# microsoft/M3P

Measured on AMD Instinct MI355X. Metric: pre-train samples/sec (whole node), 12L/768d seq=128+36, higher is better.
Workload: dtype bf16; 1 GPU; cfg2: 12L/768d/12h, 36 regions + 128 tokens, V=250002, 19 MLM targets/seq + ITM BCE, dropout 0.10, adam_inverse_sqrt + clip 5; per_gpu_batch=256, global_batch=256, seq_len=164, parallelism=dp1, prewarm_steps=36

## Files before the change

### include/m3p_hip.h

```cpp
#ifndef M3P_HIP_H
#define M3P_HIP_H

#include <stddef.h>
#include <stdint.h>

#ifdef __cplusplus
extern "C" {
#endif

#define M3P_API __attribute__((visibility("default")))

#define M3P_OK 0
#define M3P_EINVAL (-1)
#define M3P_ENOTIMPL (-2)
#define M3P_ENOMEM (-3)

M3P_API const char* m3p_version(void);


enum {
  M3P_EPI_NONE = 0,
  M3P_EPI_BIAS = 1,
  M3P_EPI_BIAS_GELU = 2,
  M3P_EPI_BIAS_DROP_RES = 3,
  M3P_EPI_RES = 4,
  M3P_EPI_DGELU = 5,
  M3P_EPI_MUL = 6,
  M3P_EPI_MULQ = 7,
  M3P_EPI_BIAS_GELUQ = 8,
  M3P_EPI_BIAS_LSE = 9
};

typedef struct M3PEpilogue {
  const float* bias;
  const void* aux;
  void* out2;
  float* colsum;
  int32_t ld_aux;
  int32_t ld_out2;
  int32_t scale_cols;
  float scale;
  float alpha;
  uint32_t seed;
  uint32_t thresh24;
  float inv_keep;
  const float* descale_a;
  const float* descale_b;
  void* out8;
  const float* scale8;
  float* amax8;
  int32_t ld_out8;
  int32_t out8_bf8;
  const int32_t* rng_rows;
} M3PEpilogue;

M3P_API int m3p_gemm_nt_bf16(const void* A, int lda, const void* W, int ldw, void* C, int ldc,
                             int M, int N, int K, int epilogue, const M3PEpilogue* ep, void* stream);

M3P_API int m3p_gemm_nt_fp8(const void* A8, int lda, int a_is_bf8, const void* W8, int ldw, void* C, int ldc,
                            int M, int N, int K, int epilogue, const M3PEpilogue* ep, void* stream);

M3P_API int m3p_quant_fp8(const void* src, int ld_src, void* dst, int ld_dst, int rows, int cols, const float* scale,
                          float* amax, int bf8, void* stream);

M3P_API int m3p_quant_fp8_batch(const long long* desc, int n_desc, int blocks_per_matrix, void* stream);

M3P_API int m3p_gemm_nt_streamk_f32(const void* A, int lda, const void* W, int ldw, float* C, int ldc,
                                    int M, int N, int K, float alpha, void* stream);
M3P_API int m3p_gemm_nn_streamk_f32(const void* A, int lda, const void* W, int ldw, int k_valid, float* C,
                                    int ldc, int M, int N, int K, float alpha, void* stream);
M3P_API int m3p_gemm_nn_w4_f32(const void* A, int lda, const void* W, int ldw, float* C, int ldc, int M, int N, int K, float alpha,
                               void* workspace, size_t workspace_bytes, void* stream);

M3P_API size_t m3p_gemm_wgrad_workspace_bytes(void);
M3P_API int m3p_gemm_wgrad_bf16(const void* dY, int lddy, const void* X, int ldx, float* dW, int lddw,
                                int M, int N, int K, float alpha, void* workspace, size_t workspace_bytes,
                                void* stream);
M3P_API int m3p_gemm_wgrad_store_bf16(const void* dY, int lddy, const void* X, int ldx, float* dW, int lddw, int M, int N, int K,
                                      float alpha, void* workspace, size_t workspace_bytes, void* stream);
M3P_API int m3p_gemm_wgrad_pair_bf16(const void* dYa, int lddya, const void* Xa, int ldxa, float* dWa, int lddwa, int Na, int Ka,
                                     const void* dYb, int lddyb, const void* Xb, int ldxb, float* dWb, int lddwb, int Nb, int Kb,
                                     int M, float alpha, void* workspace, size_t workspace_bytes, void* stream);


M3P_API int m3p_layernorm_fwd(const void* x, const float* gamma, const float* beta, const uint8_t* rowmask,
                              void* y, float* mean, float* rstd, int rows, int d, float eps, void* stream);

M3P_API int m3p_layernorm_bwd(const void* dy_a, const void* dy_b, const void* x, const float* gamma,
                              const float* mean, const float* rstd, const uint8_t* rowmask,
                              void* dx, void* dx_drop, float* dgamma, float* dbeta, float* dbias_drop,
                              int rows, int d, uint32_t seed, uint32_t thresh24, float inv_keep, void* stream);
M3P_API int m3p_layernorm_bwd_rows(const void* dy_a, const void* dy_b, const void* x, const float* gamma,
                                   const float* mean, const float* rstd, const uint8_t* rowmask,
                                   void* dx, void* dx_drop, float* dgamma, float* dbeta, float* dbias_drop,
                                   int rows, int d, uint32_t seed, uint32_t thresh24, float inv_keep,
                                   const int32_t* rng_rows, void* stream);


M3P_API int m3p_attn_fwd(const void* qkv, const int32_t* keylen, void* ctx, float* lse, uint64_t* keepmask,
                         int B, int S, int H, int dh, uint32_t seed, uint32_t thresh24, float inv_keep,
                         void* stream);

M3P_API int m3p_attn_bwd(const void* qkv, const int32_t* keylen, const void* ctx, const void* dctx,
                         const float* lse, const uint64_t* keepmask, void* dqkv, float* dbias_qkv, int B, int S,
                         int H, int dh, float qscale, uint32_t seed, uint32_t thresh24, float inv_keep,
                         void* stream);

M3P_API int m3p_attn_query_fwd(const void* q, int ld_q, const void* kv, long long kv_bstride, int ld_kv,
                               const int32_t* klen, void* ctx, int B, int Tq, int H, int dh, int Lk, int causal,
                               int pos0, void* stream);

M3P_API int m3p_attn_rows_fwd(const void* q, int ld_q, const void* kv, long long kv_bstride, int ld_kv, const int32_t* klen,
                              void* ctx, float* lse, int B, int Tq, int H, int dh, int Lk, int causal, int pos0,
                              uint32_t seed, uint32_t thresh24, float inv_keep, void* stream);
M3P_API int m3p_attn_rows_bwd(const void* q, int ld_q, const void* kv, long long kv_bstride, int ld_kv, const int32_t* klen,
                              const void* dctx, const float* lse, void* dq, int ld_dq, float* dkv, int B, int Tq, int H,
                              int dh, int Lk, int causal, int pos0, float qscale, uint32_t seed, uint32_t thresh24,
                              float inv_keep, void* stream);


M3P_API int m3p_cast_f32_bf16(const float* src, void* dst, long long n, void* stream);

M3P_API int m3p_embed_assemble_fwd(const int64_t* tok, const void* emb_bf16, const float* pos,
                                   const void* img_proj, const float* loc, const float* w_loc,
                                   const float* b_loc, const float* g_img, const float* be_img,
                                   const float* g_emb, const float* be_emb, const int32_t* totlen,
                                   void* h, void* z, float* mean_emb, float* rstd_emb, void* e,
                                   float* mean_img, float* rstd_img, int B, int T, int R, int d,
                                   uint32_t seed_img, uint32_t seed_emb, uint32_t thresh24, float inv_keep,
                                   const void* img_rows, void* stream);

M3P_API int m3p_embed_image_rows_fwd(const void* img_proj, const float* loc, const float* w_loc, const float* b_loc,
                                     const float* g_img, const float* be_img, void* e, float* mean_img,
                                     float* rstd_img, void* img_rows, int B, int R, int d, uint32_t seed_img,
                                     uint32_t thresh24, float inv_keep, void* stream);

M3P_API int m3p_embed_assemble_bwd(const void* dh, const void* z, const float* mean_emb, const float* rstd_emb,
                                   const float* g_emb, const void* e, const float* mean_img,
                                   const float* rstd_img, const float* g_img, const int64_t* tok,
                                   const int32_t* totlen, const float* loc, void* dz_scratch, void* de,
                                   float* d_g_emb, float* d_be_emb, float* d_pos, float* d_emb,
                                   void* d_tok_rows, float* d_g_img, float* d_be_img, float* d_b_img, float* d_b_loc,
                                   float* d_w_loc, int B, int T, int R, int d, int pad_index,
                                   uint32_t seed_img, uint32_t seed_emb, uint32_t thresh24, float inv_keep,
                                   int phase, void* stream);


M3P_API int m3p_gather_rows(const void* src, const int32_t* idx, void* dst, int n, int d, void* stream);
M3P_API int m3p_place_rows(const void* src, const int32_t* inv, void* dst, int rows, int d, int n, uint32_t fill_bits,
                           void* stream);
M3P_API int m3p_scatter_add_rows(const void* src, const int32_t* idx, void* dst, int n, int d, void* stream);
M3P_API int m3p_scatter_add_token_rows(const void* rows, int ld_rows, const int64_t* ids, float* dst, int n, int d,
                                       int pad_index, void* stream);

M3P_API int m3p_itm_score_fwd(const void* pre, const float* w2, const float* b2, float* pooled, float* scores, int B,
                              int d, void* stream);
M3P_API int m3p_itm_score_bwd(const float* dscores, const float* pooled, const float* w2, void* dpre16, void* dpreT16,
                              int ldt, float* db1, float* dw2, float* db2, int B, int d, void* stream);

M3P_API int m3p_ce_fwd_bwd(void* logits, int ld, int n_rows, int V, const int64_t* target, float* row_loss,
                           float* loss_sum, float loss_scale, float grad_scale, void* stream);

M3P_API int m3p_ce_lse_from_blocks(const void* stats, int n_blocks, int n_rows, const void* logits, int ld, const int64_t* target,
                                   float* row_loss, float* row_lse, void* scratch, void* stream);
M3P_API int m3p_ce_bwd_colsum(void* logits, int ld, int n_rows, int V, const int64_t* target, const float* row_lse,
                              float grad_scale, float* colsum, void* workspace, size_t workspace_bytes, void* stream);
M3P_API size_t m3p_ce_colsum_workspace_bytes(int ld, int n_rows);
M3P_API int m3p_ce_fwd_bwd_colsum(void* logits, int ld, int n_rows, int V, const int64_t* target, float* row_loss,
                                  float* row_lse, float grad_scale, float* colsum, void* workspace,
                                  size_t workspace_bytes, void* stream);

M3P_API int m3p_ce_eval(const void* logits, int ld, int n_rows, int V, const int64_t* target, float* row_loss,
                        int32_t* row_argmax, void* stream);

M3P_API int m3p_colsum_bf16(const void* x, int ld, int n, int ncols, float* out, const float* scale_ptr,
                            void* stream);


M3P_API int m3p_sumsq_f32(const float* g, long long n, double* out, void* stream);

M3P_API int m3p_sumsq_ranges_f32(const float* base, const long long* starts, const long long* counts, int n_ranges, double* out,
                                 void* stream);

M3P_API int m3p_adam_step(float* p, float* g, float* m, float* v, void* w16, long long n, float lr, float beta1,
                          float beta2, float eps, float weight_decay, float step_size, const double* gnorm_sq,
                          float max_norm, float grad_scale, int zero_grad, void* stream);
M3P_API int m3p_adam_step_ranges(float* p, float* g, float* m, float* v, void* w16, const long long* starts,
                                 const long long* counts, const float* step_sizes, const int* zero_grad, int n_ranges,
                                 float lr, float beta1, float beta2, float eps, float weight_decay, const double* gnorm_sq,
                                 float max_norm, float grad_scale, void* stream);

M3P_API int m3p_gelu_fwd(const void* u, void* h, void* dh, long long n, void* stream);
M3P_API int m3p_gelu_fwd_gq(const void* u, void* h, void* gq, int M, int N, void* stream);
M3P_API int m3p_gelu_fwd_q8(const void* u, void* h, void* h8, long long n, const float* scale, float* amax, void* stream);

M3P_API int m3p_gelu_bwd(const void* dy, const void* u, void* du, long long n, void* stream);

M3P_API int m3p_mse_fwd_bwd(const void* pred, int ld_pred, const float* tgt, int ld_tgt, void* dpred, float* row_sq,
                            int rows, int cols, float grad_scale, void* stream);


M3P_API int m3p_dropout_rows(const void* x, int ldx, const void* res, int ldres, void* y, int ldy, int rows, int cols,
                             uint32_t rng_ld, uint32_t rng_col0, uint32_t seed, uint32_t thresh24, float inv_keep,
                             void* stream);

M3P_API int m3p_glu_fwd(const void* ab, int ld_ab, void* y, int rows, int d, void* stream);
M3P_API int m3p_glu_bwd(const void* ab, int ld_ab, const void* dy, void* dab, int rows, int d, void* stream);

M3P_API int m3p_transpose_batch_bf16(const long long* desc, int n_desc, int max_tiles, void* stream);

M3P_API int m3p_transpose_bf16(const void* src, void* dst, int rows, int cols, int ld_src, int ld_dst,
                               void* stream);

M3P_API int m3p_set_persistent_grid(int workgroups);
M3P_API int m3p_set_tile_queue(int32_t* counters, int n_slots);

enum {
  M3P_KERN_NT_SKINNY = 1,
  M3P_KERN_NT_W8 = 2,
  M3P_KERN_NT_W8_QUEUE = 3,
  M3P_KERN_NT_W4 = 4,
  M3P_KERN_NT_RING = 5,
  M3P_KERN_NT_128 = 6,
  M3P_KERN_WGRAD_W4_CHUNKS = 10,
  M3P_KERN_WGRAD_W4_TILES = 11,
  M3P_KERN_WGRAD_RING = 12,
  M3P_KERN_WGRAD_128 = 13
};
M3P_API int m3p_gemm_nt_plan(int M, int N, int K, int epilogue);
M3P_API int m3p_gemm_wgrad_plan(int M, int N, int K);

M3P_API void m3p_debug_set_variant(int v);
M3P_API void m3p_debug_attn_variant(int v);

M3P_API int m3p_seq_masks(const int64_t* lengths, const int64_t* lengths_b, int B, int S, int32_t* totlen,
                          uint8_t* rowmask, void* stream);
M3P_API int m3p_mask_to_rows(const uint8_t* mask, int n_mask, int inner, long long s0, long long s1, long long soff,
                             int d, int32_t* rows, int n_rows, void* stream);
M3P_API int m3p_cast_rows_f32_bf16(const float* in, long long s0, long long s1, int n0, int n1, int cols, void* out,
                                   void* stream);
M3P_API int m3p_scale_bf16_dev(const void* in, int in_is_f32, const float* g, void* out, long long n, void* stream);
M3P_API int m3p_axpy_dev_f32(float* dst, const float* src, const float* g, long long n, void* stream);
M3P_API int m3p_itm_loss_fwd_bwd(const float* scores, const int64_t* pos, int n_groups, int sample_n, float w_ce,
                                 float w_bce, float* loss, float* dscores, void* stream);

M3P_API int m3p_probe_mfma_16x16x32(const void* a_rowmajor_16x32, const void* b_colmajor_32x16,
                                    float* d_16x16, int* d_rowcol, void* stream);
M3P_API int m3p_probe_mfma_fp8_16x16x128(const void* a_16x128, const void* w_16x128, float* d_16x16, int a_is_bf8,
                                         void* stream);
M3P_API int m3p_probe_tr16(const void* tile_bf16_64x16, void* out_64x4, void* stream);
M3P_API int m3p_probe_permlane16_swap(void* out_2x64_u32, void* stream);

#ifdef __cplusplus
}
#endif
#endif
```

### m3p_amd/csrc/gemm.hip

```cpp
#include <mutex>
#include <type_traits>
#include "common.hpp"
#include "../../include/m3p_hip.h"
#include <hip/amd_detail/amd_hip_unsafe_atomics.h>

static int g_variant = 1;
extern "C" void m3p_debug_set_variant(int v) { g_variant = (v == 2 || v == 6) ? v : 1; }

namespace {

constexpr int BK = 64;
constexpr int ROWB = BK * 2;

template <int EPI>
__device__ __forceinline__ void epilogue_store(const M3PEpilogue& ep, bf16* __restrict__ C, int ldc,
                                               int M, int N, int m, int n, f32x4 acc, f32x4& csum) {
  if (m >= M || n >= N) return;
  const bool full = (n + 3 < N);
  float v[4] = {acc[0], acc[1], acc[2], acc[3]};
  const float alpha = (ep.alpha == 0.f) ? 1.f : ep.alpha;
  if (EPI == M3P_EPI_NONE || EPI == M3P_EPI_BIAS || EPI == M3P_EPI_RES) {
#pragma unroll
    for (int r = 0; r < 4; ++r) v[r] *= alpha;
  }
// ... 440 lines not shown
        {
          typedef unsigned int u32x2 __attribute__((ext_vector_type(2)));
          const u32x2 raw = __builtin_bit_cast(u32x2, a);
#pragma unroll
          for (int r = 0; r < 4; ++r) {
            const uint32_t sign = (raw[r >> 1] << (16 * (1 - (r & 1)))) & 0x80000000u;
            const uint32_t tb = __builtin_bit_cast(uint32_t, tv[j][r]);
            v[r] *= 0.5f + __builtin_bit_cast(float, (tb & 0x7FFFFFFFu) | sign);
          }
        }
      } else {
#pragma unroll
        for (int r = 0; r < 4; ++r) v[r] *= gelu_erf_grad_f((float)a[r]);
      }
    } else {
      v *= f32x4{(float)a[0], (float)a[1], (float)a[2], (float)a[3]};
    }
    const bf16x4 ob = bf16x4{(bf16)v[0], (bf16)v[1], (bf16)v[2], (bf16)v[3]};
    *reinterpret_cast<bf16x4*>(r1 + ep_off8<true>(fr, (j * 16 + fg * 4) * 2)) = ob;
    csum[j] += f32x4{(float)ob[0], (float)ob[1], (float)ob[2], (float)ob[3]};
  }
  bf16* Cp = C + (size_t)mrow0 * ldc + nw + sch * 8;
#pragma unroll
  for (int it = 0; it < 2; ++it) {
    const int row = it * 8 + srow;
    st16(Cp + (size_t)row * ldc, flip_halves(*reinterpret_cast<const u32x4*>(r1 + ep_off<true>(row, sch * 16)), it & 1));
  }
}


template <bool BF8>
__device__ __forceinline__ uint32_t pack8(const f32x4& v, float scale, float& amax) {
  constexpr float kMax = BF8 ? 57344.f : 448.f;
  float f[4];
#pragma unroll
  for (int r = 0; r < 4; ++r) {
    amax = fmaxf(amax, fabsf(v[r]));
    f[r] = __builtin_amdgcn_fmed3f(v[r] * scale, -kMax, kMax);
  }
  int w = 0;
  if (BF8) { w = __builtin_amdgcn_cvt_pk_bf8_f32(f[0], f[1], w, false); w = __builtin_amdgcn_cvt_pk_bf8_f32(f[2], f[3], w, true); }
  else { w = __builtin_amdgcn_cvt_pk_fp8_f32(f[0], f[1], w, false); w = __builtin_amdgcn_cvt_pk_fp8_f32(f[2], f[3], w, true); }
  return (uint32_t)w;
}
__device__ __forceinline__ void lds_w32(uint32_t a, uint32_t v) { asm volatile("ds_write_b32 %0, %1" :: "v"(a), "v"(v)); }
__device__ __forceinline__ void piece8_write(char* r8, const uint32_t (&w8)[4], int lane) {
  const int fr = lane & 15, fg = lane >> 4;
  const uint32_t la = lds_addr(r8);
  asm volatile("" ::: "memory");
#pragma unroll
  for (int j = 0; j < 4; ++j) lds_w32(la + fr * 64 + ((j ^ ((fr >> 1) & 3)) << 4) + fg * 4, w8[j]);
}
__device__ __forceinline__ void piece8_store(uint8_t* __restrict__ o8, int ld8, int mrow0, int nw, char* r8, int lane) {
  const uint32_t la = lds_addr(r8);
  const int row = lane >> 2, c = lane & 3;
  u32x4_lds R;
  lds_r128(la + row * 64 + (c << 4), R);
  asm volatile("s_waitcnt lgkmcnt(0)" : "+v"(R) :: "memory");
  st16p<true>(o8 + (size_t)(mrow0 + row) * ld8 + nw + ((c ^ ((row >> 1) & 3)) << 4), u32x4{R[0], R[1], R[2], R[3]});
}
__device__ __forceinline__ void piece8_flush(uint8_t* __restrict__ o8, int ld8, int mrow0, int nw, char* r1, const uint32_t (&w8)[4], int lane) {
  piece8_write(r1, w8, lane);
  piece8_store(o8, ld8, mrow0, nw, r1, lane);
}
template <int O8 = 0>
__device__ __forceinline__ void epilogue_pieceq(bf16* __restrict__ C, int ldc, int mrow0, int nw, char* r1, const f32x4 (&rows)[4],
                                                const u32x4& q, int lane, f32x4 (&csum)[4], uint8_t* __restrict__ o8 = nullptr, int ld8 = 0,
                                                float scale8 = 1.f, float* amax = nullptr, char* r8 = nullptr) {
  const int fr = lane & 15, fg = lane >> 4;
  const int srow = lane >> 3, sch = lane & 7;
  uint32_t w8[4];
#pragma unroll
  for (int j = 0; j < 4; ++j) {
    const uint32_t w = q[j];
    f32x4 g = f32x4{(float)(w & 0xFFu), (float)((w >> 8) & 0xFFu), (float)((w >> 16) & 0xFFu), (float)(w >> 24)};
    g = g * GQ_STEP - GQ_OFF;
    const f32x4 v = rows[j] * g;
    const bf16x4 ob = bf16x4{(bf16)v[0], (bf16)v[1], (bf16)v[2], (bf16)v[3]};
    if (O8) lds_w64(lds_addr(r1) + ep_off8<true>(fr, (j * 16 + fg * 4) * 2), ob);
    else *reinterpret_cast<bf16x4*>(r1 + ep_off8<true>(fr, (j * 16 + fg * 4) * 2)) = ob;
    csum[j] += v;
    if (O8) w8[j] = (O8 == 2) ? pack8<true>(v, scale8, *amax) : pack8<false>(v, scale8, *amax);
  }
  if (O8) piece8_write(r8, w8, lane);
  bf16* Cp = C + (size_t)mrow0 * ldc + nw + sch * 8;
  if (O8) {
    const uint32_t la = lds_addr(r1), l8 = lds_addr(r8);
    const int row8 = lane >> 2, c8 = lane & 3;
    u32x4_lds Ra, Rb, R8;
    lds_r128(la + ep_off<true>(srow, sch * 16), Ra);
    lds_r128(la + ep_off<true>(8 + srow, sch * 16), Rb);
    lds_r128(l8 + row8 * 64 + (c8 << 4), R8);
    asm volatile("s_waitcnt lgkmcnt(0)" : "+v"(Ra), "+v"(Rb), "+v"(R8));
    st16p<true>(Cp + (size_t)srow * ldc, u32x4{Ra[0], Ra[1], Ra[2], Ra[3]});
    st16p<true>(Cp + (size_t)(8 + srow) * ldc, u32x4{Rb[2], Rb[3], Rb[0], Rb[1]});
    st16p<true>(o8 + (size_t)(mrow0 + row8) * ld8 + nw + ((c8 ^ ((row8 >> 1) & 3)) << 4), u32x4{R8[0], R8[1], R8[2], R8[3]});
    return;
  }
  u32x4 R2[2];
#pragma unroll
  for (int it = 0; it < 2; ++it) {
    const int row = it * 8 + srow;
    R2[it] = flip_halves(*reinterpret_cast<const u32x4*>(r1 + ep_off<true>(row, sch * 16)), it & 1);
  }
#pragma unroll
  for (int it = 0; it < 2; ++it) st16p<true>(Cp + (size_t)(it * 8 + srow) * ldc, R2[it]);
  if (O8) piece8_store(o8, ld8, mrow0, nw, r8, lane);
}

__device__ __forceinline__ void epilogue_half_lse(bf16* __restrict__ C, int ldc, float2* __restrict__ stats, int V, int mrow0, int nw,
                                                  char* r1, const f32x4 (&rows0)[4], const f32x4 (&rows1)[4],
                                                  const f32x4 (&biasv)[4], int lane, bool edge) {
  constexpr float kLog2e = 1.4426950408889634f;
  const int fr = lane & 15, fg = lane >> 4;
  const int srow = lane >> 3, sch = lane & 7;
#pragma unroll
  for (int ii = 0; ii < 2; ++ii) {
    f32x4 x[4];
#pragma unroll
    for (int j = 0; j < 4; ++j) {
      x[j] = (ii ? rows1[j] : rows0[j]) + biasv[j];
      const bf16x4 xb = bf16x4{(bf16)x[j][0], (bf16)x[j][1], (bf16)x[j][2], (bf16)x[j][3]};
      *reinterpret_cast<bf16x4*>(r1 + ep_off8<true>(ii * 16 + fr, (j * 16 + fg * 4) * 2)) = xb;
#pragma unroll
      for (int r = 0; r < 4; ++r) x[j][r] = (float)xb[r];
    }
    if (edge) {
#pragma unroll
      for (int j = 0; j < 4; ++j)
#pragma unroll
        for (int r = 0; r < 4; ++r)
          if (nw + j * 16 + fg * 4 + r >= V) x[j][r] = -INFINITY;
    }
    f32x4 m4 = x[0];
#pragma unroll
    for (int j = 1; j < 4; ++j)
#pragma unroll
      for (int r = 0; r < 4; ++r) m4[r] = fmaxf(m4[r], x[j][r]);
    float m = fmaxf(fmaxf(m4[0], m4[1]), fmaxf(m4[2], m4[3]));
    m = fmaxf(m, __shfl_xor(m, 16, 64));
    m = fmaxf(m, __shfl_xor(m, 32, 64));
    const float mb = (m == -INFINITY) ? 0.f : m * kLog2e;
    f32x4 s4 = f32x4{0.f, 0.f, 0.f, 0.f};
#pragma unroll
    for (int j = 0; j < 4; ++j) {
      const f32x4 a = x[j] * kLog2e - mb;
#pragma unroll
      for (int r = 0; r < 4; ++r) s4[r] += __builtin_amdgcn_exp2f(a[r]);
    }
    float sm = (s4[0] + s4[1]) + (s4[2] + s4[3]);
    sm += __shfl_xor(sm, 16, 64);
    sm += __shfl_xor(sm, 32, 64);
    if (fg == 0) stats[mrow0 + ii * 16 + fr] = float2{m, sm};
  }
  bf16* Cp = C + (size_t)mrow0 * ldc + nw + sch * 8;
#pragma unroll
  for (int it = 0; it < 4; ++it) {
    const int row = it * 8 + srow;
    st16p<true>(Cp + (size_t)row * ldc, flip_halves(*reinterpret_cast<const u32x4*>(r1 + ep_off<true>(row, sch * 16)), it & 1));
  }
}

constexpr int GQ_TAB_LO = 0x3A00, GQ_TAB_HI = 0x4100, GQ_TAB_N = GQ_TAB_HI - GQ_TAB_LO;
constexpr int GQ_TAB_BYTES = GQ_TAB_N * 4;
__device__ __forceinline__ void geluq_table_fill(uint32_t* tab, int tid, int nthreads) {
  for (int i = tid; i < GQ_TAB_N; i += nthreads) {
    const float xm = __builtin_bit_cast(float, ((uint32_t)(GQ_TAB_LO + i) << 16) | 0x8000u);
    const float tail = 0.5f * erfcf(xm * 0.70710678118654752440f);
    const float gd = (1.0f - tail) + xm * 0.39894228040143267794f * __expf(-0.5f * xm * xm);
    tab[i] = (__builtin_bit_cast(uint32_t, tail) & 0xFFFFFF00u) | gelu_grad_code(gd);
  }
}
__device__ __forceinline__ void lds_r32(uint32_t a, uint32_t& v) { asm volatile("ds_read_b32 %0, %1" : "=v"(v) : "v"(a)); }
template <int O8 = 0>
__device__ __forceinline__ void epilogue_piece_geluq_lut(bf16* __restrict__ C, int ldc, uint8_t* __restrict__ qout, int mrow0, int nw,
                                                         char* r1, const f32x4 (&rows)[4], int lane, uint32_t tab_off,
                                                         uint8_t* __restrict__ o8 = nullptr, int ld8 = 0, float scale8 = 1.f, float* amax = nullptr,
                                                         char* r8 = nullptr) {
  const int fr = lane & 15, fg = lane >> 4;
  const int srow = lane >> 3, sch = lane & 7;
  uint32_t w8[4];
  uint32_t w[4][4];
#pragma unroll
  for (int j = 0; j < 4; ++j)
#pragma unroll
    for (int r = 0; r < 4; ++r) {
      const float xf = rows[j][r];
      const uint32_t xb = __builtin_bit_cast(uint32_t, xf);
      const uint32_t mag = __builtin_amdgcn_ubfe(xb, 16, 15);
      const uint32_t idx = min(max(mag, (uint32_t)GQ_TAB_LO), (uint32_t)(GQ_TAB_HI - 1));
      lds_r32((idx << 2) + tab_off, w[j][r]);
    }
  asm volatile("s_waitcnt lgkmcnt(0)" : "+v"(w[0][0]), "+v"(w[0][1]), "+v"(w[0][2]), "+v"(w[0][3]), "+v"(w[1][0]), "+v"(w[1][1]), "+v"(w[1][2]), "+v"(w[1][3]),
                                        "+v"(w[2][0]), "+v"(w[2][1]), "+v"(w[2][2]), "+v"(w[2][3]), "+v"(w[3][0]), "+v"(w[3][1]), "+v"(w[3][2]), "+v"(w[3][3]));
  const uint32_t la = lds_addr(r1);
  u32x4 code;
#pragma unroll
  for (int j = 0; j < 4; ++j) {
    f32x4 hv;
    float xs[4];
#pragma unroll
    for (int r = 0; r < 4; ++r) {
      xs[r] = rows[j][r];
      float mx;
      asm("v_max_f32 %0, 0, %1" : "=v"(mx) : "v"(xs[r]));
      asm("v_fma_f32 %0, -|%1|, %2, %3" : "=v"(hv[r]) : "v"(xs[r]), "v"(w[j][r]), "v"(mx));
    }
    const uint32_t x0 = __builtin_bit_cast(uint32_t, xs[0]), x1 = __builtin_bit_cast(uint32_t, xs[1]);
    const uint32_t x2 = __builtin_bit_cast(uint32_t, xs[2]), x3 = __builtin_bit_cast(uint32_t, xs[3]);
    const uint32_t blo = __builtin_amdgcn_perm(w[j][1], w[j][0], 0x0c0c0400u), bhi = __builtin_amdgcn_perm(w[j][3], w[j][2], 0x04000c0cu);
    const uint32_t slo = __builtin_amdgcn_perm(x1, x0, 0x0c0c0b09u), shi = __builtin_amdgcn_perm(x3, x2, 0x0b090c0cu);
    code[j] = (blo | bhi) ^ (slo | shi);
    lds_w64(la + ep_off8<true>(fr, (j * 16 + fg * 4) * 2), bf16x4{(bf16)hv[0], (bf16)hv[1], (bf16)hv[2], (bf16)hv[3]});
    if (O8) w8[j] = pack8<false>(hv, scale8, *amax);
  }
  st16p<true>(qout + lane * 16, code);
  if (O8) piece8_write(r8, w8, lane);
  u32x4 R[2];
  u32x4_lds R8;
  lds_r128(la + ep_off<true>(srow, sch * 16), R[0]);
  lds_r128(la + ep_off<true>(8 + srow, sch * 16), R[1]);
  const int row8 = lane >> 2, c8 = lane & 3;
  if (O8) {
    lds_r128(lds_addr(r8) + row8 * 64 + (c8 << 4), R8);
    asm volatile("s_waitcnt lgkmcnt(0)" : "+v"(R[0]), "+v"(R[1]), "+v"(R8));
  } else {
    asm volatile("s_waitcnt lgkmcnt(0)" : "+v"(R[0]), "+v"(R[1]));
  }
  bf16* Cp = C + (size_t)mrow0 * ldc + nw + sch * 8;
  st16p<true>(Cp + (size_t)srow * ldc, R[0]);
  st16p<true>(Cp + (size_t)(8 + srow) * ldc, flip_halves(R[1], true));
  if (O8) st16p<true>(o8 + (size_t)(mrow0 + row8) * ld8 + nw + ((c8 ^ ((row8 >> 1) & 3)) << 4), u32x4{R8[0], R8[1], R8[2], R8[3]});
}


template <int EPI>
__global__ __launch_bounds__(512)
void gemm_nt_ring_kernel(const bf16* __restrict__ A, int lda, const bf16* __restrict__ W, int ldw,
                         bf16* __restrict__ C, int ldc, int M, int N, int K, M3PEpilogue ep,
                         int tiles_m, int tiles_n) {
  constexpr int BM = 256, BN = 128, NWAVES = 8;
  constexpr int A_BYTES = BM * ROWB, B_BYTES = BN * ROWB, STAGE = A_BYTES + B_BYTES;
  extern __shared__ __attribute__((aligned(16))) char smem[];

  const int tid = threadIdx.x, lane = tid & 63;
  const int wid = __builtin_amdgcn_readfirstlane(tid >> 6);
  const int ntiles = tiles_m * tiles_n;
  const int n_strips = (tiles_n >= 24) ? (tiles_n + 7) / 8 : 1;
  const int strip_w = (tiles_n + n_strips - 1) / n_strips;
  auto split_tile = [&](int t, int& tm, int& tn) {
    const int strip = t / (tiles_m * strip_w);
    const int rem = t - strip * tiles_m * strip_w;
    const int bn = min(strip_w, tiles_n - strip * strip_w);
    tm = rem / bn;
    tn = strip * strip_w + (rem - tm * bn);
  };
  const int nwg = gridDim.x;
  const int per_xcd = nwg >> 3;
  const int slot = (blockIdx.x & 7) * per_xcd + (blockIdx.x >> 3);
  auto tile_of = [&](int q) { return q * nwg + slot; };
  const int my_tiles = (ntiles > slot) ? (ntiles - slot + nwg - 1) / nwg : 0;
  if (my_tiles == 0) return;
  float* gtab = (EPI == M3P_EPI_DGELU) ? reinterpret_cast<float*>(smem + 3 * STAGE) : nullptr;
  if (EPI == M3P_EPI_DGELU) gelu_grad_table_fill(gtab, tid, 512);
  const int nk = K / BK;
  const int total = my_tiles * nk;

  const int sr = lane >> 3, sc = (lane & 7) ^ sr;
  const bf16* a_src[4];
  const bf16* w_src[2];
  int l_q = 0, l_kt = 0;
  auto set_load_tile = [&](int q) {
    const int t = tile_of(q);
    int tm, tn;
    split_tile(t, tm, tn);
#pragma unroll
    for (int i = 0; i < 4; ++i) a_src[i] = A + (size_t)min(tm * BM + (wid + i * NWAVES) * 8 + sr, M - 1) * lda + sc * 8;
#pragma unroll
    for (int i = 0; i < 2; ++i) w_src[i] = W + (size_t)min(tn * BN + (wid + i * NWAVES) * 8 + sr, N - 1) * ldw + sc * 8;
  };
  auto issue_load = [&](int s, int piece) {
    char* sa = smem + s * STAGE;
    const int k0 = l_kt * BK;
    if (piece < 4)
      __builtin_amdgcn_global_load_lds(GLB_PTR(a_src[piece] + k0), LDS_PTR(sa + (wid + piece * NWAVES) * 1024), 16, 0, 0);
    else
      __builtin_amdgcn_global_load_lds(GLB_PTR(w_src[piece - 4] + k0), LDS_PTR(sa + A_BYTES + (wid + (piece - 4) * NWAVES) * 1024), 16, 0, 0);
  };
  auto load_done = [&]() {
    if (++l_kt == nk) { l_kt = 0; ++l_q; if (l_q < my_tiles) set_load_tile(l_q); }
  };
  auto stage_next = [&](int s) {
#pragma unroll
    for (int pc = 0; pc < 6; ++pc) issue_load(s, pc);
    load_done();
  };

  const int wm = wid >> 1, wn = wid & 1;
  const int fr = lane & 15, fg = lane >> 4;
  const uint32_t lds0 = (uint32_t)(uintptr_t)(__attribute__((address_space(3))) char*)smem;
  uint32_t a_addr[2], b_addr[2];
#pragma unroll
  for (int ks = 0; ks < 2; ++ks) {
    const int ch = ((fg + 4 * ks) ^ (fr & 7)) * 16;
    a_addr[ks] = lds0 + (wm * 64 + fr) * ROWB + ch;
    b_addr[ks] = lds0 + A_BYTES + (wn * 64 + fr) * ROWB + ch;
// ... 243 lines not shown
    a_addr[ks] = lds0 + (wm * 128 + fr) * ROWB + ch;
    b_addr[ks] = lds0 + A_BYTES + (wn * 64 + fr) * ROWB + ch;
  }
#define W8_DSR(dst, addr, off) asm volatile("ds_read_b128 %0, %1 offset:" #off : "=v"(dst) : "v"(addr))
  auto read_w = [&](uint32_t ba, bf16x8 (&wf)[4]) {
    W8_DSR(wf[0], ba, 0); W8_DSR(wf[1], ba, 2048); W8_DSR(wf[2], ba, 4096); W8_DSR(wf[3], ba, 6144);
  };
  auto read_a_lo = [&](uint32_t aa, bf16x8 (&af)[4]) {
    W8_DSR(af[0], aa, 0); W8_DSR(af[1], aa, 2048); W8_DSR(af[2], aa, 4096); W8_DSR(af[3], aa, 6144);
  };
  auto read_a_hi = [&](uint32_t aa, bf16x8 (&af)[4]) {
    W8_DSR(af[0], aa, 8192); W8_DSR(af[1], aa, 10240); W8_DSR(af[2], aa, 12288); W8_DSR(af[3], aa, 14336);
  };
#define W8_LGKM0() do { __builtin_amdgcn_sched_barrier(0); asm volatile("s_waitcnt lgkmcnt(0)" ::: "memory"); __builtin_amdgcn_sched_barrier(0); } while (0)

  f32x4 acc[8][4];
#pragma unroll
  for (int i = 0; i < 8; ++i)
#pragma unroll
    for (int j = 0; j < 4; ++j) acc[i][j] = f32x4{0.f, 0.f, 0.f, 0.f};
  if constexpr (kGqLut) {
    int tm0, tn0;
    split_tile(slot, tm0, tn0);
    const float* bp = ep.bias + tn0 * BN + wn * 64 + fg * 4;
#pragma unroll
    for (int j = 0; j < 4; ++j) {
      const f32x4 b = *reinterpret_cast<const f32x4*>(bp + j * 16);
#pragma unroll
      for (int i = 0; i < 8; ++i) acc[i][j] = b;
    }
  }
  auto mfma_q = [&](auto half_c, const bf16x8 (&af)[4], const bf16x8 (&wf)[4]) {
    constexpr int I0 = 4 * decltype(half_c)::value;
    __builtin_amdgcn_s_setprio(1);
#pragma unroll
    for (int i = 0; i < 4; ++i)
#pragma unroll
      for (int j = 0; j < 4; ++j)
        acc[I0 + i][j] = __builtin_amdgcn_mfma_f32_16x16x32_bf16(wf[j], af[i], acc[I0 + i][j], 0, 0, 0);
    __builtin_amdgcn_s_setprio(0);
  };
  using H0 = std::integral_constant<int, 0>;
  using H1 = std::integral_constant<int, 1>;

  set_load_tile(slot);
  stage_next(0);
#define W8_H1 (dyn ? h1d : (step + 1 < total))
#define W8_MORE2 (dyn ? l_alive : more2)
  bool h1d = l_alive;
  if (dyn ? h1d : (total > 1)) {
    stage_next(1);
    asm volatile("s_waitcnt vmcnt(8)" ::: "memory");
  } else {
    asm volatile("s_waitcnt vmcnt(0)" ::: "memory");
  }
  __builtin_amdgcn_s_barrier();
  asm volatile("" ::: "memory");

  bf16x8 fa0[4], fa1[4], fw0[4], fw1[4];
  read_w(b_addr[0], fw0);
  read_a_lo(a_addr[0], fa0);
  W8_LGKM0();
  int c_kt = 0, c_q = 0;
  const bool io_aligned = ((ldc & 7) == 0) && (((uintptr_t)C & 15) == 0) &&
                          (!(EPI == M3P_EPI_BIAS_GELU) || (((ep.ld_out2 & 7) == 0) && (((uintptr_t)ep.out2 & 15) == 0))) &&
                          (!ep.bias || (((uintptr_t)ep.bias & 15) == 0)) &&
                          (!ep.aux || (((ep.ld_aux & 7) == 0) && (((uintptr_t)ep.aux & 15) == 0)));
  f32x4 csum[4];
#pragma unroll
  for (int j = 0; j < 4; ++j) csum[j] = f32x4{0.f, 0.f, 0.f, 0.f};
  int csum_nw = -1;
  auto flush_csum = [&]() {
#pragma unroll
    for (int j = 0; j < 4; ++j)
#pragma unroll
      for (int r = 0; r < 4; ++r) {
        float sfl = csum[j][r];
        sfl += __shfl_xor(sfl, 1, 64); sfl += __shfl_xor(sfl, 2, 64);
        sfl += __shfl_xor(sfl, 4, 64); sfl += __shfl_xor(sfl, 8, 64);
        const int n = csum_nw + j * 16 + fg * 4 + r;
        if (fr == 0 && n < N) unsafeAtomicAdd(ep.colsum + n, sfl);
        csum[j][r] = 0.f;
      }
  };
  float amax_run = 0.f;
  if constexpr (O8 && EPI == M3P_EPI_MULQ) reinterpret_cast<float*>(smem + 2 * STAGE + 8 * 2048)[tid] = 0.f;
  bool spread_pending = false;
  for (int step = 0; dyn || step < total; ++step) {
    const int cur = step & 1, nxt = cur ^ 1;
    const bool last_kt = (c_kt + 1 == nk);
    const bool more2 = dyn ? false : (step + 2 < total);
    const uint32_t so = cur * STAGE;
    const bool pend = spread_pending;
    if (pend) { issue_load(nxt, 3); issue_load(nxt, 4); issue_load(nxt, 5); }
    read_a_hi(a_addr[0] + so, fa1);
    __builtin_amdgcn_sched_barrier(0);
    mfma_q(H0{}, fa0, fw0);
    W8_LGKM0();
    if (pend) { issue_load(nxt, 6); issue_load(nxt, 7); }
    read_w(b_addr[1] + so, fw1);
    read_a_lo(a_addr[1] + so, fa0);
    __builtin_amdgcn_sched_barrier(0);
    mfma_q(H1{}, fa1, fw0);
    if (pend) { load_done(); spread_pending = false; }
    W8_LGKM0();
    read_a_hi(a_addr[1] + so, fa1);
    __builtin_amdgcn_sched_barrier(0);
    mfma_q(H0{}, fa0, fw1);
    W8_LGKM0();
    asm volatile("s_waitcnt vmcnt(0)" ::: "memory");
    __builtin_amdgcn_s_barrier();
    asm volatile("" ::: "memory");
    __builtin_amdgcn_sched_barrier(0);
    if (dyn && pop_state) {
      if (pop_state == 1) {
        if (wid == 0 && lane == 0) {
          const int p = per_xcd + (int)popped, q = p / per_xcd;
          const int t = q * nwg + xcd * per_xcd + (p - q * per_xcd);
          *mbox = (t < ntiles) ? t : -1;
        }
        pop_state = 2;
      } else {
        t_next = __builtin_amdgcn_readfirstlane(*mbox);
        pop_state = 0;
      }
      __builtin_amdgcn_sched_barrier(0);
    }
    const bool req = W8_MORE2 && (!last_kt || !kAuxE);
    if (req) {
      issue_load(cur, 0); issue_load(cur, 1); issue_load(cur, 2);
      spread_pending = true;
    }
    if (W8_H1 && !last_kt) {
      read_w(b_addr[0] + nxt * STAGE, fw0);
      read_a_lo(a_addr[0] + nxt * STAGE, fa0);
    }
    __builtin_amdgcn_sched_barrier(0);
    mfma_q(H1{}, fa1, fw1);
    W8_LGKM0();

    if (++c_kt == nk) {
      c_kt = 0;
      const int t = dyn ? t_cmp : tile_of(c_q);
      if (dyn) t_cmp = t_ld; else ++c_q;
      int tm, tn;
      split_tile(t, tm, tn);
      const int m0 = tm * BM, n0 = tn * BN;
      const int mw = m0 + wm * 128, nw = n0 + wn * 64;
      if (kMulE && ep.colsum && csum_nw != nw) {
        if (csum_nw >= 0) flush_csum();
        csum_nw = nw;
      }
      const bool fast = io_aligned && (m0 + BM <= M) && (n0 + BN <= N);
      if constexpr (EPI == M3P_EPI_BIAS_LSE) {
        if (fast) {
          char* r1 = smem + 2 * STAGE + wid * 4096;
          f32x4 biasv[4];
#pragma unroll
          for (int j = 0; j < 4; ++j) biasv[j] = *reinterpret_cast<const f32x4*>(ep.bias + nw + j * 16 + (lane >> 4) * 4);
          const int V = ep.ld_out2;
          float2* st = reinterpret_cast<float2*>(ep.out2) + (size_t)(tn * 4 + wn) * M;
          const bool edge = (nw + 64 > V);
#pragma unroll
          for (int hf = 0; hf < 4; ++hf) {
            epilogue_half_lse(C, ldc, st, V, mw + 32 * hf, nw, r1, acc[2 * hf], acc[2 * hf + 1], biasv, lane, edge);
            __builtin_amdgcn_sched_barrier(0);
          }
        }
      } else if constexpr (kGqLut) {
        f32x4 bnext[4];
        {
          const bool more_tiles = dyn ? (t_cmp >= 0) : (c_q < my_tiles);
          int tm2 = tm, tn2 = tn;
          if (more_tiles) split_tile(dyn ? t_cmp : tile_of(c_q), tm2, tn2);
          const float* bp = ep.bias + tn2 * BN + wn * 64 + fg * 4;
#pragma unroll
          for (int j = 0; j < 4; ++j) bnext[j] = *reinterpret_cast<const f32x4*>(bp + j * 16);
        }
        {
          char* r1 = smem + 2 * STAGE + kTabBytes + wid * 2048;
          const uint32_t tab_off = lds0 + 2 * STAGE - 4 * GQ_TAB_LO;
          uint8_t* qo = reinterpret_cast<uint8_t*>(ep.out2) + gq_block_offset(tm, tn, tiles_n, wid, 0);
          if constexpr (O8) {
            const float sc8 = ep.scale8 ? *ep.scale8 : 1.f;
#pragma unroll
            for (int hp = 0; hp < 8; ++hp) {
              epilogue_piece_geluq_lut<1>(C, ldc, qo + 1024 * hp, mw + 16 * hp, nw, r1, acc[hp], lane, tab_off,
                                          reinterpret_cast<uint8_t*>(ep.out8), ep.ld_out8, sc8, &amax_run,
                                          smem + 2 * STAGE + kTabBytes + 8 * 2048 + wid * 1024);
              __builtin_amdgcn_sched_barrier(0);
            }
          } else {
#pragma unroll
            for (int hp = 0; hp < 8; ++hp) {
              epilogue_piece_geluq_lut(C, ldc, qo + 1024 * hp, mw + 16 * hp, nw, r1, acc[hp], lane, tab_off);
              __builtin_amdgcn_sched_barrier(0);
            }
          }
        }
#pragma unroll
        for (int i = 0; i < 8; ++i)
#pragma unroll
          for (int j = 0; j < 4; ++j) acc[i][j] = bnext[j];
      } else if constexpr (EPI == M3P_EPI_MULQ) {
        if (fast) {
          const uint8_t* qp = reinterpret_cast<const uint8_t*>(ep.aux) + gq_block_offset(tm, tn, tiles_n, wid, 0) + lane * 16;
          char* r1 = smem + 2 * STAGE + wid * 2048;
#define MQ_LD(off) (*reinterpret_cast<const u32x4*>(qp + (off)))
          u32x4 qa = MQ_LD(0), qb = MQ_LD(1024);
          __builtin_amdgcn_sched_barrier(0);
          if (W8_MORE2) { issue_load(cur, 0); issue_load(cur, 1); issue_load(cur, 2); spread_pending = true; }
          __builtin_amdgcn_sched_barrier(0);
          if constexpr (O8) {
            const float sc8 = ep.scale8 ? *ep.scale8 : 1.f;
            uint8_t* o8 = reinterpret_cast<uint8_t*>(ep.out8);
            float* amax_slot = reinterpret_cast<float*>(smem + 2 * STAGE + 8 * 2048) + tid;
            float amax_t = *amax_slot;
#pragma unroll
            for (int hp = 0; hp < 8; ++hp) {
              u32x4 qc = qb;
              if (hp + 2 < 8) qc = MQ_LD((hp + 2) * 1024);
              char* r8 = smem + 2 * STAGE + 8 * 2048 + 2048 + wid * 1024;
              epilogue_pieceq<2>(C, ldc, mw + 16 * hp, nw, r1, acc[hp], qa, lane, csum, o8, ep.ld_out8, sc8, &amax_t, r8);
              __builtin_amdgcn_sched_barrier(0);
              qa = qb; qb = qc;
            }
            *amax_slot = amax_t;
          } else {
#pragma unroll
          for (int hp = 0; hp < 8; hp += 2) {
            u32x4 qc = qa, qd = qb;
            if (hp + 2 < 8) qc = MQ_LD((hp + 2) * 1024);
            epilogue_pieceq(C, ldc, mw + 16 * hp, nw, r1, acc[hp], qa, lane, csum);
            __builtin_amdgcn_sched_barrier(0);
            if (hp + 3 < 8) qd = MQ_LD((hp + 3) * 1024);
            epilogue_pieceq(C, ldc, mw + 16 * (hp + 1), nw, r1, acc[hp + 1], qb, lane, csum);
            __builtin_amdgcn_sched_barrier(0);
            qa = qc; qb = qd;
          }
          }
#undef MQ_LD
        }
      } else if (fast && kMulE) {
        char* r1 = smem + 2 * STAGE + kTabBytes + wid * 2048;
        u32x4 ta[2], tb[2];
        aux16_issue(ep, mw, nw, lane, ta);
        __builtin_amdgcn_sched_barrier(0);
        if (W8_MORE2) { issue_load(cur, 0); issue_load(cur, 1); issue_load(cur, 2); spread_pending = true; }
        __builtin_amdgcn_sched_barrier(0);
#pragma unroll
        for (int hp = 0; hp < 8; hp += 2) {
          aux16_issue(ep, mw + 16 * (hp + 1), nw, lane, tb);
          epilogue_piece16<EPI>(ep, C, ldc, mw + 16 * hp, nw, r1, acc[hp], ta, lane, csum, gtab);
          __builtin_amdgcn_sched_barrier(0);
          if (hp + 2 < 8) aux16_issue(ep, mw + 16 * (hp + 2), nw, lane, ta);
          epilogue_piece16<EPI>(ep, C, ldc, mw + 16 * (hp + 1), nw, r1, acc[hp + 1], tb, lane, csum, gtab);
          __builtin_amdgcn_sched_barrier(0);
        }
      } else if (fast) {
        char* r1 = smem + 2 * STAGE + wid * 4096;
        f32x4 biasv[4];
        load_bias4<EPI>(ep, nw, lane, biasv);
        u32x4 aux0[4];
        if (kAuxE) {
          load_aux_rows_issue<EPI>(ep, mw, nw, lane, aux0);
          __builtin_amdgcn_sched_barrier(0);
          if (W8_MORE2) { issue_load(cur, 0); issue_load(cur, 1); issue_load(cur, 2); spread_pending = true; }
          __builtin_amdgcn_sched_barrier(0);
        }
#pragma unroll
        for (int hf = 0; hf < 4; ++hf) {
          f32x4 rows[2][4];
#pragma unroll
          for (int ii = 0; ii < 2; ++ii)
#pragma unroll
            for (int j = 0; j < 4; ++j) rows[ii][j] = acc[2 * hf + ii][j];
          bf16x4 auxv[2][4];
          if (kAuxE && hf == 0) load_aux_rows_finish<EPI, true>(lane, r1, aux0, auxv);
          else load_aux_rows<EPI, true>(ep, mw + 32 * hf, nw, lane, r1, auxv);
          epilogue_half<EPI, true>(ep, C, ldc, N, mw + 32 * hf, nw, r1, rows, biasv, auxv, lane, csum, gtab);
          __builtin_amdgcn_sched_barrier(0);
        }
      } else {
        if (kAuxE && W8_MORE2) { issue_load(cur, 0); issue_load(cur, 1); issue_load(cur, 2); spread_pending = true; }
#pragma unroll
        for (int i = 0; i < 8; ++i)
#pragma unroll
          for (int j = 0; j < 4; ++j)
            epilogue_store<EPI>(ep, C, ldc, M, N, mw + i * 16 + fr, nw + j * 16 + fg * 4, acc[i][j], csum[j]);
      }
      if constexpr (!kGqLut) {
#pragma unroll
        for (int i = 0; i < 8; ++i)
#pragma unroll
          for (int j = 0; j < 4; ++j) acc[i][j] = f32x4{0.f, 0.f, 0.f, 0.f};
      }
      if (W8_H1) {
        read_w(b_addr[0] + nxt * STAGE, fw0);
        read_a_lo(a_addr[0] + nxt * STAGE, fa0);
        W8_LGKM0();
      }
    }
    if (dyn) {
      if (!h1d) break;
      h1d = l_alive;
    }
  }
  if (kMulE && ep.colsum && csum_nw >= 0) flush_csum();
  if constexpr (O8 && (EPI == M3P_EPI_BIAS_GELUQ || EPI == M3P_EPI_MULQ)) {
    if (ep.amax8) {
      float* wmax = reinterpret_cast<float*>(smem + 2 * STAGE + kTabBytes);
      if constexpr (EPI == M3P_EPI_MULQ) amax_run = reinterpret_cast<float*>(smem + 2 * STAGE + 8 * 2048)[tid];
      const float mxw = wave_max(amax_run);
      __syncthreads();
      if (lane == 0) wmax[wid] = mxw;
      __syncthreads();
      if (tid == 0) {
        float mx = wmax[0];
#pragma unroll
// ... 951 lines not shown
  *err = hipSuccess;
  std::lock_guard<std::mutex> lk(g_tq_mu);
  if (!g_tq_pool) return nullptr;
  if (!g_tq_bound) { g_tq_stream = st; g_tq_bound = true; }
  if (st != g_tq_stream) return nullptr;
  if (g_tq_next == g_tq_slots) {
    *err = hipMemsetAsync(g_tq_pool, 0, (size_t)g_tq_slots * 8 * sizeof(int), st);
    if (*err != hipSuccess) return nullptr;
    g_tq_next = 0;
  }
  return g_tq_pool + 8 * g_tq_next++;
}

constexpr int W4_MIN_K = 2048;
static bool tq_enabled() {
  std::lock_guard<std::mutex> lk(g_tq_mu);
  return g_tq_pool != nullptr;
}

static int nt_plan(int epi, int M, int N, int K, int* queue) {
  if (queue) *queue = 0;
  const bool whole = M >= 1024 && (M % 256) == 0 && (N % 256) == 0 && N >= 512 && (K % 64) == 0;
  if (epi == M3P_EPI_MULQ || epi == M3P_EPI_BIAS_GELUQ || epi == M3P_EPI_BIAS_LSE) return whole ? M3P_KERN_NT_W8 : M3P_EINVAL;
  const bool mul_epi = epi == M3P_EPI_DGELU || epi == M3P_EPI_MUL;
  if (M <= 128 && (K % 128) == 0 && !mul_epi) return M3P_KERN_NT_SKINNY;
  const bool deep = N >= 512 && 2LL * N * K <= (64LL << 20) && epi != M3P_EPI_DGELU;
  const bool armed = tq_enabled();
  const bool w4_first = g_variant == 1 && deep && K >= W4_MIN_K && epi != M3P_EPI_MUL && !armed;
  if (whole && g_variant != 2 && !w4_first) {
    int grid = num_cus();
    const int ntiles = (M / 256) * (N / 256);
    if (ntiles < grid) grid = (ntiles + 7) / 8 * 8;
    if (queue) *queue = (!mul_epi && armed && ntiles > grid && K >= 8 * BK) ? 1 : 0;
    return M3P_KERN_NT_W8;
  }
  if (M >= 1024 && (M % 256) == 0 && (N % 256) == 0 && (g_variant == 2 || (g_variant == 1 && deep)))
    return M3P_KERN_NT_W4;
  if (M >= 1024) return M3P_KERN_NT_RING;
  return M3P_KERN_NT_128;
}

template <int EPI>
int launch_nt(const bf16* A, int lda, const bf16* W, int ldw, bf16* C, int ldc, int M, int N, int K,
              const M3PEpilogue& ep, hipStream_t st) {
  int want_queue = 0;
  const int plan = nt_plan(EPI, M, N, K, &want_queue);
  if (plan == M3P_KERN_NT_SKINNY) {
    if constexpr (EPI != M3P_EPI_DGELU && EPI != M3P_EPI_MUL) {
      if (M <= 16) return launch_nt_skinny<EPI, 1>(A, lda, W, ldw, C, ldc, M, N, K, ep, st);
      if (M <= 32) return launch_nt_skinny<EPI, 2>(A, lda, W, ldw, C, ldc, M, N, K, ep, st);
      if (M <= 64) return launch_nt_skinny<EPI, 4>(A, lda, W, ldw, C, ldc, M, N, K, ep, st);
      return launch_nt_skinny<EPI, 8>(A, lda, W, ldw, C, ldc, M, N, K, ep, st);
    }
  }
  if (plan == M3P_KERN_NT_W8) {
    const int tiles_m = M / 256, tiles_n = N / 256;
    const size_t lds = 2 * 512 * ROWB + (EPI == M3P_EPI_DGELU ? GELU_TAB_N * sizeof(float) : 0) +
                       ((EPI == M3P_EPI_DGELU || EPI == M3P_EPI_MUL) ? 8 * 2048 : 8 * 4096);
    auto kern = gemm_nt_w8_kernel<EPI>;
    static bool attr_set8 = false;
    if (!attr_set8) {
      hipError_t e = hipFuncSetAttribute((const void*)kern, hipFuncAttributeMaxDynamicSharedMemorySize, (int)lds);
      if (e != hipSuccess) return (int)e;
      attr_set8 = true;
    }
    int grid = num_cus();
    const int ntiles = tiles_m * tiles_n;
    if (ntiles < grid) grid = (ntiles + 7) / 8 * 8;
    constexpr bool kQueueOk = !(EPI == M3P_EPI_DGELU || EPI == M3P_EPI_MUL);
    int* ctr = nullptr;
    if (kQueueOk && want_queue) {
      hipError_t e;
      ctr = tq_acquire(st, &e);
      if (e != hipSuccess) return (int)e;
    }
    if constexpr (kQueueOk) if (ctr) {
      auto kern_d = gemm_nt_w8_kernel<EPI, true>;
      static bool attr_set8d = false;
      if (!attr_set8d) {
        hipError_t e = hipFuncSetAttribute((const void*)kern_d, hipFuncAttributeMaxDynamicSharedMemorySize, (int)lds);
        if (e != hipSuccess) return (int)e;
        attr_set8d = true;
      }
      hipLaunchKernelGGL(kern_d, dim3(grid), dim3(512), lds, st, A, lda, W, ldw, C, ldc, M, N, K, ep, tiles_m, tiles_n, ctr);
      M3P_CHECK_LAUNCH();
      return M3P_OK;
    }
    hipLaunchKernelGGL(kern, dim3(grid), dim3(512), lds, st, A, lda, W, ldw, C, ldc, M, N, K, ep, tiles_m, tiles_n, ctr);
    M3P_CHECK_LAUNCH();
    return M3P_OK;
  }
  if (plan == M3P_KERN_NT_W4) {
    constexpr int BM = 256, BN = 256;
    const int tiles_m = (M + BM - 1) / BM, tiles_n = (N + BN - 1) / BN;
    const size_t lds = 2 * (BM + BN) * 128 + 4 * EP_HALF;
    const bool rows = (EPI == M3P_EPI_BIAS_DROP_RES && ep.rng_rows != nullptr);
    auto kern = rows ? gemm_nt_w4_kernel<(EPI == M3P_EPI_BIAS_DROP_RES ? M3P_EPI_DROP_RES_ROWS : EPI)> : gemm_nt_w4_kernel<EPI>;
    static bool attr_set_both[2] = {false, false};
    bool& attr_set = attr_set_both[rows ? 1 : 0];
    if (!attr_set) {
      hipError_t e = hipFuncSetAttribute((const void*)kern, hipFuncAttributeMaxDynamicSharedMemorySize, (int)lds);
      if (e != hipSuccess) return (int)e;
      attr_set = true;
    }
    int grid = num_cus();
    const int ntiles = tiles_m * tiles_n;
    if (ntiles < grid) grid = (ntiles + 7) / 8 * 8;
    const long long wbytes = 2LL * N * K, abytes = 2LL * M * K;
    const int m_fast = (wbytes > (64LL << 20) && abytes < wbytes) ? 1 : 0;
    hipLaunchKernelGGL(kern, dim3(grid), dim3(256), lds, st, A, lda, W, ldw, C, ldc, M, N, K, ep, tiles_m, tiles_n, m_fast);
    M3P_CHECK_LAUNCH();
    return M3P_OK;
  }
  if (plan == M3P_KERN_NT_RING) {
    constexpr int BM = 256, BN = 128;
    const int tiles_m = (M + BM - 1) / BM, tiles_n = (N + BN - 1) / BN;
    const size_t lds = 3 * (BM + BN) * ROWB + (EPI == M3P_EPI_DGELU ? GELU_TAB_N * sizeof(float) : 0);
    auto kern = gemm_nt_ring_kernel<EPI>;
    static bool attr_set = false;
    if (!attr_set) {
      hipError_t e = hipFuncSetAttribute((const void*)kern, hipFuncAttributeMaxDynamicSharedMemorySize, (int)lds);
      if (e != hipSuccess) return (int)e;
      attr_set = true;
    }
    int grid = num_cus();
    const int ntiles = tiles_m * tiles_n;
    if (ntiles < grid) grid = (ntiles + 7) / 8 * 8;
    hipLaunchKernelGGL(kern, dim3(grid), dim3(512), lds, st, A, lda, W, ldw, C, ldc, M, N, K, ep, tiles_m, tiles_n);
    M3P_CHECK_LAUNCH();
    return M3P_OK;
  }
  constexpr int BM = 128, BN = 128;
  const int tiles_m = (M + BM - 1) / BM, tiles_n = (N + BN - 1) / BN;
  const size_t lds = 2 * (BM + BN) * ROWB;
  auto kern = gemm_nt_kernel<BM, BN, EPI>;
  static bool attr_set = false;
  if (!attr_set) {
    hipError_t e = hipFuncSetAttribute((const void*)kern, hipFuncAttributeMaxDynamicSharedMemorySize, (int)lds);
    if (e != hipSuccess) return (int)e;
    attr_set = true;
  }
  hipLaunchKernelGGL(kern, dim3(tiles_m * tiles_n), dim3(256), lds, st, A, lda, W, ldw, C, ldc, M, N, K, ep,
                     tiles_m, tiles_n);
  M3P_CHECK_LAUNCH();
  return M3P_OK;
}

template <int EPI>
static int launch_nt_gq(const bf16* A, int lda, const bf16* W, int ldw, bf16* C, int ldc, int M, int N, int K,
                        const M3PEpilogue& ep, hipStream_t st) {
  if (M < 1024 || (M % 256) || (N % 256) || N < 512 || (K % 64) || (lda % 8) || (ldw % 8) || (ldc % 8) || ((uintptr_t)C & 15))
    return M3P_EINVAL;
  if (EPI == M3P_EPI_MULQ && (!ep.aux || ((uintptr_t)ep.aux & 15))) return M3P_EINVAL;
  if ((EPI == M3P_EPI_BIAS_GELUQ || EPI == M3P_EPI_BIAS_LSE) && (!ep.out2 || ((uintptr_t)ep.out2 & 15) || !ep.bias || ((uintptr_t)ep.bias & 15)))
    return M3P_EINVAL;
  if (EPI == M3P_EPI_BIAS_LSE && (ep.ld_out2 <= 0 || ep.ld_out2 > N)) return M3P_EINVAL;
  const int tiles_m = M / 256, tiles_n = N / 256;
  const size_t lds = 2 * 512 * ROWB + ((EPI == M3P_EPI_BIAS_GELUQ) ? GQ_TAB_BYTES + 8 * 2048 + 8 * 1024 : 8 * (EPI != M3P_EPI_MULQ ? 4096 : 2048)) +
                     (EPI == M3P_EPI_MULQ ? 2048 + 8 * 1024 : 0);
  int grid = num_cus();
  const int ntiles = tiles_m * tiles_n;
  if (ntiles < grid) grid = (ntiles + 7) / 8 * 8;
  if constexpr (EPI == M3P_EPI_BIAS_GELUQ || EPI == M3P_EPI_MULQ) {
    if (ep.out8) {
      if (((uintptr_t)ep.out8 & 15) || (ep.ld_out8 & 15) || ep.ld_out8 < N || !ep.scale8 || !ep.amax8) return M3P_EINVAL;
      if ((EPI == M3P_EPI_MULQ) != (ep.out8_bf8 != 0)) return M3P_EINVAL;
      auto kern8 = gemm_nt_w8_kernel<EPI, false, true>;
      static bool attr_set8 = false;
      if (!attr_set8) {
        hipError_t e = hipFuncSetAttribute((const void*)kern8, hipFuncAttributeMaxDynamicSharedMemorySize, (int)lds);
        if (e != hipSuccess) return (int)e;
        attr_set8 = true;
      }
      hipLaunchKernelGGL(kern8, dim3(grid), dim3(512), lds, st, A, lda, W, ldw, C, ldc, M, N, K, ep, tiles_m, tiles_n, (int*)nullptr);
      M3P_CHECK_LAUNCH();
      return M3P_OK;
    }
  }
  auto kern = gemm_nt_w8_kernel<EPI>;
  static bool attr_set = false;
  if (!attr_set) {
    hipError_t e = hipFuncSetAttribute((const void*)kern, hipFuncAttributeMaxDynamicSharedMemorySize, (int)lds);
    if (e != hipSuccess) return (int)e;
    attr_set = true;
  }
  hipLaunchKernelGGL(kern, dim3(grid), dim3(512), lds, st, A, lda, W, ldw, C, ldc, M, N, K, ep, tiles_m, tiles_n, (int*)nullptr);
  M3P_CHECK_LAUNCH();
  return M3P_OK;
}

constexpr int WG_T = 128;
constexpr int WG_ROWB = WG_T * 2;
constexpr int WG_TILE_BYTES = BK * WG_ROWB;

__device__ __forceinline__ bf16x4 lds_tr16(const char* p) {
  s16x4 v = __builtin_amdgcn_ds_read_tr16_b64_v4i16((__attribute__((address_space(3))) s16x4*)(p));
  return __builtin_bit_cast(bf16x4, v);
}

__global__ __launch_bounds__(256)
void gemm_wgrad_kernel(const bf16* __restrict__ dY, int lddy, const bf16* __restrict__ X, int ldx,
                       float* __restrict__ dW, int lddw, int M, int N, int K, float alpha,
                       int tiles_i, int tiles_j, int m_chunk) {
  extern __shared__ __attribute__((aligned(16))) char smem[];
  const int tid = threadIdx.x, lane = tid & 63;
  const int wid = __builtin_amdgcn_readfirstlane(tid >> 6);
  const int ntile = tiles_i * tiles_j;
  const int id = xcd_remap(blockIdx.x, gridDim.x);
  const int split = id / ntile, tile = id - split * ntile;
  const int ti = tile / tiles_j, tj = tile - ti * tiles_j;
  const int i0 = ti * WG_T, j0 = tj * WG_T;
  const int m_begin = split * m_chunk;
  const int m_end = min(M, m_begin + m_chunk);
  if (m_begin >= m_end) return;

  const int sr = lane >> 4, sc = lane & 15;
  const int n_chunks = (N + 7) / 8, k_chunks = (K + 7) / 8;
  int ycol[4], xcol[4];
#pragma unroll
  for (int i = 0; i < 4; ++i) {
    const int rb = wid + i * 4;
    const int f = sr | (((rb >> 1) & 1) << 2);
    const int gc = sc ^ (f << 1);
    ycol[i] = min(i0 / 8 + gc, n_chunks - 1) * 8;
    xcol[i] = min(j0 / 8 + gc, k_chunks - 1) * 8;
  }

  auto stage = [&](int mt, int s) {
    char* sy = smem + s * 2 * WG_TILE_BYTES;
    char* sx = sy + WG_TILE_BYTES;
    const int mbase = m_begin + mt * BK;
    const bool fullt = (mbase + BK <= m_end);
#pragma unroll
    for (int i = 0; i < 4; ++i) {
      const int rb = wid + i * 4;
      const int m = mbase + rb * 4 + sr;
      if (fullt) {
        __builtin_amdgcn_global_load_lds(GLB_PTR(dY + (size_t)m * lddy + ycol[i]), LDS_PTR(sy + rb * 1024), 16, 0, 0);
        __builtin_amdgcn_global_load_lds(GLB_PTR(X + (size_t)m * ldx + xcol[i]), LDS_PTR(sx + rb * 1024), 16, 0, 0);
      } else {
        uint4 vy = make_uint4(0, 0, 0, 0), vx = make_uint4(0, 0, 0, 0);
        if (m < m_end) {
          vy = *reinterpret_cast<const uint4*>(dY + (size_t)m * lddy + ycol[i]);
          vx = *reinterpret_cast<const uint4*>(X + (size_t)m * ldx + xcol[i]);
        }
        *reinterpret_cast<uint4*>(sy + rb * 1024 + lane * 16) = vy;
        *reinterpret_cast<uint4*>(sx + rb * 1024 + lane * 16) = vx;
      }
    }
  };

  const int wi = wid >> 1, wj = wid & 1;
  const int ft = lane & 15, fg = lane >> 4;
  const int frow = (fg * 8 + (ft >> 2)) * WG_ROWB;
  const int fsw = ((ft >> 2) | ((fg & 1) << 2)) << 1;
  int y_off[4], x_off[4];
#pragma unroll
  for (int c = 0; c < 4; ++c) {
    const int qy = wi * 8 + 2 * c + ((ft & 3) >> 1), qx = wj * 8 + 2 * c + ((ft & 3) >> 1);
    y_off[c] = frow + ((qy ^ fsw) << 4) + ((ft & 1) << 3);
    x_off[c] = WG_TILE_BYTES + frow + ((qx ^ fsw) << 4) + ((ft & 1) << 3);
  }

  f32x4 acc[4][4];
#pragma unroll
  for (int a = 0; a < 4; ++a)
#pragma unroll
    for (int b = 0; b < 4; ++b) acc[a][b] = f32x4{0.f, 0.f, 0.f, 0.f};

  const int nmt = (m_end - m_begin + BK - 1) / BK;
  stage(0, 0);
  __syncthreads();
  for (int mt = 0; mt < nmt; ++mt) {
    const int cur = mt & 1;
    if (mt + 1 < nmt) stage(mt + 1, cur ^ 1);
    const char* sbase = smem + cur * 2 * WG_TILE_BYTES;
#pragma unroll
    for (int ks = 0; ks < 2; ++ks) {
      bf16x8 yf[4], xf[4];
#pragma unroll
      for (int c = 0; c < 4; ++c) {
        const char* py = sbase + y_off[c] + ks * 32 * WG_ROWB;
        const char* px = sbase + x_off[c] + ks * 32 * WG_ROWB;
        bf16x4 y0 = lds_tr16(py), y1 = lds_tr16(py + 4 * WG_ROWB);
        bf16x4 x0 = lds_tr16(px), x1 = lds_tr16(px + 4 * WG_ROWB);
        yf[c] = bf16x8{y0[0], y0[1], y0[2], y0[3], y1[0], y1[1], y1[2], y1[3]};
        xf[c] = bf16x8{x0[0], x0[1], x0[2], x0[3], x1[0], x1[1], x1[2], x1[3]};
      }
#pragma unroll
      for (int a = 0; a < 4; ++a)
#pragma unroll
        for (int b = 0; b < 4; ++b)
          acc[a][b] = __builtin_amdgcn_mfma_f32_16x16x32_bf16(yf[a], xf[b], acc[a][b], 0, 0, 0);
    }
    __syncthreads();
  }

#pragma unroll
  for (int a = 0; a < 4; ++a)
#pragma unroll
    for (int b = 0; b < 4; ++b) {
      const int j = j0 + wj * 64 + b * 16 + ft;
#pragma unroll
      for (int r = 0; r < 4; ++r) {
        const int i = i0 + wi * 64 + a * 16 + fg * 4 + r;
        if (i < N && j < K) unsafeAtomicAdd(dW + (size_t)i * lddw + j, alpha * acc[a][b][r]);
      }
    }
}
// ... 532 lines not shown
  const int frow = fg * 8 + (ft >> 2);
  const int fsw = ((ft >> 2) | ((fg & 1) << 2)) << 1;
  uint32_t y_addr[4], x_addr[4];
#pragma unroll
  for (int c = 0; c < 4; ++c) {
    const int qy = wi * 8 + 2 * c + ((ft & 3) >> 1), qx = wj * 8 + 2 * c + ((ft & 3) >> 1);
    y_addr[c] = lds0 + frow * WR_YROW + ((qy ^ fsw) << 4) + ((ft & 1) << 3);
    x_addr[c] = lds0 + WR_YB + frow * WR_XROW + ((qx ^ fsw) << 4) + ((ft & 1) << 3);
  }
#define M3P_TR(dst, addr, off) asm volatile("ds_read_b64_tr_b16 %0, %1 offset:" #off : "=v"(dst) : "v"(addr))
  auto read_set0 = [&](uint32_t so, s16x4 (&y)[4][2], s16x4 (&x)[4][2]) {
#pragma unroll
    for (int c = 0; c < 4; ++c) {
      M3P_TR(y[c][0], y_addr[c] + so, 0); M3P_TR(y[c][1], y_addr[c] + so, 2048);
      M3P_TR(x[c][0], x_addr[c] + so, 0); M3P_TR(x[c][1], x_addr[c] + so, 1024);
    }
  };
  auto read_set1 = [&](uint32_t so, s16x4 (&y)[4][2], s16x4 (&x)[4][2]) {
#pragma unroll
    for (int c = 0; c < 4; ++c) {
      M3P_TR(y[c][0], y_addr[c] + so, 16384); M3P_TR(y[c][1], y_addr[c] + so, 18432);
      M3P_TR(x[c][0], x_addr[c] + so, 8192); M3P_TR(x[c][1], x_addr[c] + so, 9216);
    }
  };
#define M3P_LGKM0() do { __builtin_amdgcn_sched_barrier(0); asm volatile("s_waitcnt lgkmcnt(0)" ::: "memory"); __builtin_amdgcn_sched_barrier(0); } while (0)

  f32x4 acc[4][4];
#pragma unroll
  for (int a = 0; a < 4; ++a)
#pragma unroll
    for (int b = 0; b < 4; ++b) acc[a][b] = f32x4{0.f, 0.f, 0.f, 0.f};
  auto frag = [](const s16x4 (&h)[2]) {
    return __builtin_bit_cast(bf16x8, __builtin_shufflevector(h[0], h[1], 0, 1, 2, 3, 4, 5, 6, 7));
  };
  auto mfma_batch = [&](const s16x4 (&y)[4][2], const s16x4 (&x)[4][2]) {
    bf16x8 yf[4], xf[4];
#pragma unroll
    for (int c = 0; c < 4; ++c) { yf[c] = frag(y[c]); xf[c] = frag(x[c]); }
#pragma unroll
    for (int a = 0; a < 4; ++a)
#pragma unroll
      for (int b = 0; b < 4; ++b)
        acc[a][b] = __builtin_amdgcn_mfma_f32_16x16x32_bf16(yf[a], xf[b], acc[a][b], 0, 0, 0);
  };

  stage_next(0);
  if (total > 1) {
    stage_next(1);
    asm volatile("s_waitcnt vmcnt(6)" ::: "memory");
  } else {
    asm volatile("s_waitcnt vmcnt(0)" ::: "memory");
  }
  __builtin_amdgcn_s_barrier();
  asm volatile("" ::: "memory");

  s16x4 y0[4][2], x0[4][2], y1[4][2], x1[4][2];
  read_set0(0, y0, x0);
  M3P_LGKM0();
  WgCursor cc = locate(g0);
  int cur = 0;
  for (int step = 0; step < total; ++step) {
    const int nxt = (cur == 2) ? 0 : cur + 1;
    const int nx2 = (nxt == 2) ? 0 : nxt + 1;
    const bool more2 = (step + 2 < total);
    if (more2) stage_next(nx2);
    read_set1(cur * WR_STAGE, y1, x1);
    __builtin_amdgcn_sched_barrier(0);
    mfma_batch(y0, x0);
    M3P_LGKM0();
    if (more2) asm volatile("s_waitcnt vmcnt(6)" ::: "memory");
    else asm volatile("s_waitcnt vmcnt(0)" ::: "memory");
    __builtin_amdgcn_s_barrier();
    asm volatile("" ::: "memory");
    __builtin_amdgcn_sched_barrier(0);
    read_set0(nxt * WR_STAGE, y0, x0);
    __builtin_amdgcn_sched_barrier(0);
    mfma_batch(y1, x1);
    M3P_LGKM0();

    const bool last_of_tile = (cc.mt + 1 == cc.len) || (step + 1 == total);
    if (last_of_tile) {
      const int ti = cc.t / tiles_j, tj = cc.t - ti * tiles_j;
#pragma unroll
      for (int a = 0; a < 4; ++a)
#pragma unroll
        for (int b = 0; b < 4; ++b) {
          const int j = tj * WR_J + wj * 64 + b * 16 + ft;
#pragma unroll
          for (int r = 0; r < 4; ++r) {
            const int i = ti * WR_I + wi * 64 + a * 16 + fg * 4 + r;
            if (i < N && j < K) unsafeAtomicAdd(dW + (size_t)i * lddw + j, alpha * acc[a][b][r]);
            acc[a][b][r] = 0.f;
          }
        }
    }
    advance(cc);
    cur = nxt;
  }
#undef M3P_TR
#undef M3P_LGKM0
}

}

namespace {
template <int EPI, bool A_BF8>
int launch_nt_fp8(const uint8_t* A, int lda, const uint8_t* W, int ldw, bf16* C, int ldc, int M, int N, int K,
                         const M3PEpilogue& ep, hipStream_t st) {
  const int tiles_m = M / 256, tiles_n = N / 256;
  const size_t lds = 2 * 512 * ROWB + (EPI == M3P_EPI_DGELU ? GELU_TAB_N * sizeof(float) : 0) +
                     ((EPI == M3P_EPI_DGELU || EPI == M3P_EPI_MUL) ? 8 * 2048 : 8 * 4096);
  auto kern = gemm_nt_w8f8_kernel<EPI, A_BF8>;
  static bool attr_set = false;
  if (!attr_set) {
    hipError_t e = hipFuncSetAttribute((const void*)kern, hipFuncAttributeMaxDynamicSharedMemorySize, (int)lds);
    if (e != hipSuccess) return (int)e;
    attr_set = true;
  }
  int grid = num_cus();
  const int ntiles = tiles_m * tiles_n;
  if (ntiles < grid) grid = (ntiles + 7) / 8 * 8;
  hipLaunchKernelGGL(kern, dim3(grid), dim3(512), lds, st, A, lda, W, ldw, C, ldc, M, N, K, ep, tiles_m, tiles_n);
  M3P_CHECK_LAUNCH();
  return M3P_OK;
}

}

extern "C" {

int m3p_gemm_nt_bf16(const void* A, int lda, const void* W, int ldw, void* C, int ldc, int M, int N, int K,
                     int epilogue, const M3PEpilogue* ep_in, void* stream) {
  if (M <= 0 || N <= 0 || K <= 0 || (K % BK) != 0 || (lda % 8) != 0 || (ldw % 8) != 0 || (ldc % 4) != 0)
    return M3P_EINVAL;
  if (((uintptr_t)A & 15) || ((uintptr_t)W & 15) || ((uintptr_t)C & 7)) return M3P_EINVAL;
  M3PEpilogue ep = {};
  if (ep_in) ep = *ep_in;
  if ((epilogue == M3P_EPI_BIAS_DROP_RES || epilogue == M3P_EPI_RES || epilogue == M3P_EPI_DGELU || epilogue == M3P_EPI_MUL) &&
      (!ep.aux || (ep.ld_aux % 4) != 0))
    return M3P_EINVAL;
  if (epilogue == M3P_EPI_BIAS_GELU && (!ep.out2 || (ep.ld_out2 % 4) != 0)) return M3P_EINVAL;
  hipStream_t st = (hipStream_t)stream;
  const bf16* a = (const bf16*)A; const bf16* w = (const bf16*)W; bf16* c = (bf16*)C;
  switch (epilogue) {
    case M3P_EPI_NONE: return launch_nt<M3P_EPI_NONE>(a, lda, w, ldw, c, ldc, M, N, K, ep, st);
    case M3P_EPI_BIAS: return launch_nt<M3P_EPI_BIAS>(a, lda, w, ldw, c, ldc, M, N, K, ep, st);
    case M3P_EPI_BIAS_GELU: return launch_nt<M3P_EPI_BIAS_GELU>(a, lda, w, ldw, c, ldc, M, N, K, ep, st);
    case M3P_EPI_BIAS_DROP_RES: return launch_nt<M3P_EPI_BIAS_DROP_RES>(a, lda, w, ldw, c, ldc, M, N, K, ep, st);
    case M3P_EPI_RES: return launch_nt<M3P_EPI_RES>(a, lda, w, ldw, c, ldc, M, N, K, ep, st);
    case M3P_EPI_DGELU: return launch_nt<M3P_EPI_DGELU>(a, lda, w, ldw, c, ldc, M, N, K, ep, st);
    case M3P_EPI_MUL: return launch_nt<M3P_EPI_MUL>(a, lda, w, ldw, c, ldc, M, N, K, ep, st);
    case M3P_EPI_MULQ: return launch_nt_gq<M3P_EPI_MULQ>(a, lda, w, ldw, c, ldc, M, N, K, ep, st);
    case M3P_EPI_BIAS_GELUQ: return launch_nt_gq<M3P_EPI_BIAS_GELUQ>(a, lda, w, ldw, c, ldc, M, N, K, ep, st);
    case M3P_EPI_BIAS_LSE: return launch_nt_gq<M3P_EPI_BIAS_LSE>(a, lda, w, ldw, c, ldc, M, N, K, ep, st);
    default: return M3P_EINVAL;
  }
}

int m3p_gemm_nt_fp8(const void* A, int lda, int a_is_bf8, const void* W, int ldw, void* C, int ldc, int M, int N, int K,
                    int epilogue, const M3PEpilogue* ep_in, void* stream) {
  if (M <= 0 || N <= 0 || K <= 0 || (K % 128) != 0 || (lda % 16) != 0 || (ldw % 16) != 0 || (ldc % 8) != 0) return M3P_EINVAL;
  if ((M % 256) != 0 || (N % 256) != 0) return M3P_EINVAL;
  if (((uintptr_t)A & 15) || ((uintptr_t)W & 15) || ((uintptr_t)C & 15)) return M3P_EINVAL;
  M3PEpilogue ep = {};
  if (ep_in) ep = *ep_in;
  if ((epilogue == M3P_EPI_BIAS_DROP_RES || epilogue == M3P_EPI_RES || epilogue == M3P_EPI_DGELU || epilogue == M3P_EPI_MUL) &&
      (!ep.aux || (ep.ld_aux % 8) != 0))
    return M3P_EINVAL;
  hipStream_t st = (hipStream_t)stream;
  const uint8_t* a = (const uint8_t*)A; const uint8_t* w = (const uint8_t*)W; bf16* c = (bf16*)C;
#define M3P_F8_CASE(E)                                                                                        \
  case E: return a_is_bf8 ? launch_nt_fp8<E, true>(a, lda, w, ldw, c, ldc, M, N, K, ep, st)                    \
                          : launch_nt_fp8<E, false>(a, lda, w, ldw, c, ldc, M, N, K, ep, st)
  switch (epilogue) {
    M3P_F8_CASE(M3P_EPI_NONE);
    M3P_F8_CASE(M3P_EPI_BIAS);
    M3P_F8_CASE(M3P_EPI_BIAS_DROP_RES);
    M3P_F8_CASE(M3P_EPI_RES);
    M3P_F8_CASE(M3P_EPI_DGELU);
    M3P_F8_CASE(M3P_EPI_MUL);
    default: return M3P_ENOTIMPL;
  }
#undef M3P_F8_CASE
}

static int launch_streamk(const void* A, int lda, const void* W, int ldw, float* C, int ldc, int M, int N, int K, float alpha,
                          bool w_kn, int k_valid, void* stream) {
  if (M <= 0 || N <= 0 || K <= 0 || (K % BK) != 0 || (lda % 8) != 0 || (ldw % 8) != 0) return M3P_EINVAL;
  if (((uintptr_t)A & 15) || ((uintptr_t)W & 15)) return M3P_EINVAL;
  if (w_kn && (k_valid <= 0 || k_valid > K)) return M3P_EINVAL;
  const int tiles_m_all = (M + 255) / 256, tiles_n = (N + 127) / 128;
  const size_t lds = 3 * (256 + 128) * ROWB;
  auto kern = w_kn ? gemm_nt_streamk_kernel<true> : gemm_nt_streamk_kernel<false>;
  hipError_t e = hipFuncSetAttribute((const void*)kern, hipFuncAttributeMaxDynamicSharedMemorySize, (int)lds);
  if (e != hipSuccess) return (int)e;
  const int grid = num_cus();
  const int nk = K / BK;
  const int n_launch = (tiles_m_all * tiles_n + grid - 1) / grid;
  const int rows_per = ((tiles_m_all + n_launch - 1) / n_launch) * 256;
  for (int m0 = 0; m0 < M; m0 += rows_per) {
    const int m = (M - m0 < rows_per) ? M - m0 : rows_per;
    const int tiles_m = (m + 255) / 256;
    long long share = ((long long)tiles_m * tiles_n * nk + grid - 1) / grid;
    const int chunk = (int)(share < nk ? (share < 1 ? 1 : share) : nk);
    hipLaunchKernelGGL(kern, dim3(grid), dim3(512), lds, (hipStream_t)stream, (const bf16*)A + (size_t)m0 * lda, lda,
                       (const bf16*)W, ldw, C + (size_t)m0 * ldc, ldc, m, N, K, alpha, tiles_m, tiles_n, chunk, k_valid);
    M3P_CHECK_LAUNCH();
  }
  return M3P_OK;
}

int m3p_gemm_nt_streamk_f32(const void* A, int lda, const void* W, int ldw, float* C, int ldc, int M, int N, int K,
                            float alpha, void* stream) {
  return launch_streamk(A, lda, W, ldw, C, ldc, M, N, K, alpha, false, K, stream);
}

int m3p_gemm_nn_streamk_f32(const void* A, int lda, const void* W, int ldw, int k_valid, float* C, int ldc, int M, int N,
                            int K, float alpha, void* stream) {
  return launch_streamk(A, lda, W, ldw, C, ldc, M, N, K, alpha, true, k_valid, stream);
}

int m3p_set_persistent_grid(int workgroups) {
  if (workgroups < 0 || (workgroups % 8) != 0) return M3P_EINVAL;
  g_persistent_grid = workgroups;
  return M3P_OK;
}

int m3p_set_tile_queue(int32_t* counters, int n_slots) {
  if (counters && (n_slots <= 0 || ((uintptr_t)counters & 3))) return M3P_EINVAL;
  std::lock_guard<std::mutex> lk(g_tq_mu);
  g_tq_pool = counters;
  g_tq_slots = counters ? n_slots : 0;
  g_tq_next = 0;
  g_tq_bound = false;
  return M3P_OK;
}

size_t m3p_gemm_wgrad_workspace_bytes(void) {
  const size_t grid = (size_t)hw_cus();
  return grid * (65536 + 272) * sizeof(float) + grid * sizeof(int);
}

static bool wgrad_w4_ok(int M, int N, int K, int lddy, int ldx, const void* dY, const void* X) {
  return (M % 64) == 0 && M >= 4096 && (N % 256) == 0 && (K % 256) == 0 &&
         (lddy % 8) == 0 && (ldx % 8) == 0 && !((uintptr_t)dY & 15) && !((uintptr_t)X & 15);
}
extern "C++" {
template <bool YROWS = false>
static int launch_wgrad_w4(const void* dY, int lddy, const void* X, int ldx, float* dW, int lddw, int M, int N, int K,
                           float alpha, void* workspace, size_t workspace_bytes, void* stream, const WgradProblem* pb_in,
                           bool store = false) {
  const int ti = N / 256, tj = K / 256;
  WgradProblem pb = {};
  if (pb_in) pb = *pb_in;
  const int ntile = ti * tj + pb.tiles_i * pb.tiles_j;
  const size_t lds = 2 * 65536;
  static bool attr_set_w = false;
  if (!attr_set_w) {
    hipError_t e = hipFuncSetAttribute((const void*)gemm_wgrad_w4_kernel<YROWS>, hipFuncAttributeMaxDynamicSharedMemorySize, (int)lds);
    if (e != hipSuccess) return (int)e;
    attr_set_w = true;
  }
  const int grid = num_cus();
  const int nmt = M / 64;
  long long share = ((long long)ntile * nmt + grid - 1) / grid;
  int chunk = (int)(share < nmt ? (share < 1 ? 1 : share) : nmt);
  if ((long long)ntile >= 4LL * grid) chunk = 0;
  if (pb_in && chunk == 0) return M3P_EINVAL;
  if (store && chunk != 0) return M3P_ENOTIMPL;
  float* ws = nullptr;
  if (workspace && workspace_bytes >= m3p_gemm_wgrad_workspace_bytes() && (((uintptr_t)workspace & 15) == 0) && chunk != 0 &&
      (lddw % 4) == 0 && (((uintptr_t)dW & 15) == 0) && (!pb_in || ((pb.lddw % 4) == 0 && (((uintptr_t)pb.dW & 15) == 0))))
    ws = (float*)workspace;
  int* ws_tile = ws ? (int*)(ws + (size_t)grid * (65536 + 272)) : nullptr;
  hipLaunchKernelGGL(gemm_wgrad_w4_kernel<YROWS>, dim3(grid), dim3(256), lds, (hipStream_t)stream, (const bf16*)dY, lddy,
                     (const bf16*)X, ldx, dW, lddw, M, N, K, alpha, ti, tj, chunk, ws, ws_tile, store ? 1 : 0, pb);
  M3P_CHECK_LAUNCH();
  if (ws) {
    hipLaunchKernelGGL(wgrad_reduce_kernel, dim3(16, ntile), dim3(256), 0, (hipStream_t)stream, (const float*)ws,
                       (const int*)ws_tile, grid, dW, lddw, tj, alpha, ti * tj, pb);
    M3P_CHECK_LAUNCH();
  }
  return M3P_OK;
}
}

static int wgrad_plan(int M, int N, int K, bool aligned) {
  if (aligned && (M % 64) == 0 && M >= 4096 && (N % 256) == 0 && (K % 256) == 0 && (N / 256) * (K / 256) >= 9)
    return ((long long)(N / 256) * (K / 256) >= 4LL * num_cus()) ? M3P_KERN_WGRAD_W4_TILES : M3P_KERN_WGRAD_W4_CHUNKS;
  if ((M % BK) == 0 && M >= 4096) return M3P_KERN_WGRAD_RING;
  return M3P_KERN_WGRAD_128;
}

int m3p_gemm_nt_plan(int M, int N, int K, int epilogue) {
  if (M <= 0 || N <= 0 || K <= 0 || (K % BK) != 0 || epilogue < 0 || epilogue > M3P_EPI_BIAS_LSE) return M3P_EINVAL;
  int queue = 0;
  const int plan = nt_plan(epilogue, M, N, K, &queue);
  return (plan == M3P_KERN_NT_W8 && queue) ? M3P_KERN_NT_W8_QUEUE : plan;
}

int m3p_gemm_wgrad_plan(int M, int N, int K) {
  if (M <= 0 || N <= 0 || K <= 0) return M3P_EINVAL;
  return wgrad_plan(M, N, K, true);
}

int m3p_gemm_nn_w4_f32(const void* A, int lda, const void* W, int ldw, float* C, int ldc, int M, int N, int K, float alpha,
                       void* workspace, size_t workspace_bytes, void* stream) {
// ... 85 lines not shown
```

### m3p_amd/csrc/heads.hip

```cpp
#include "common.hpp"
#include <hip/amd_detail/amd_hip_unsafe_atomics.h>

namespace {

__global__ __launch_bounds__(256) void gather_rows_kernel(const bf16* __restrict__ src, const int32_t* __restrict__ idx,
                                                          bf16* __restrict__ dst, int n, int d) {
  const int nchunk = d >> 2;
  const size_t total = (size_t)n * nchunk;
  for (size_t i = (size_t)blockIdx.x * blockDim.x + threadIdx.x; i < total; i += (size_t)gridDim.x * blockDim.x) {
    const int r = (int)(i / nchunk), c = (int)(i - (size_t)r * nchunk);
    *reinterpret_cast<bf16x4*>(dst + (size_t)r * d + 4 * c) =
        *reinterpret_cast<const bf16x4*>(src + (size_t)idx[r] * d + 4 * c);
  }
}
__global__ __launch_bounds__(256) void place_rows_kernel(const bf16* __restrict__ src, const int32_t* __restrict__ inv,
                                                         bf16* __restrict__ dst, int rows, int d, int n, uint32_t fill2) {
  typedef unsigned int u32x4 __attribute__((ext_vector_type(4)));
  const int nchunk = d >> 3;
  const size_t total = (size_t)rows * nchunk;
  const u32x4 fv = u32x4{fill2, fill2, fill2, fill2};
  for (size_t i = (size_t)blockIdx.x * blockDim.x + threadIdx.x; i < total; i += (size_t)gridDim.x * blockDim.x) {
    const int r = (int)(i / nchunk), c = (int)(i - (size_t)r * nchunk);
    const int j = inv[r];
    u32x4 v = fv;
// ... 160 lines not shown
  const int nchunk = ld >> 3;
  float m = -INFINITY, s = 0.f;
  int bi = CE_NO_COL;
  for (int c = tid; c < nchunk; c += 1024) {
    const bf16x8 v = *reinterpret_cast<const bf16x8*>(lr + 8 * c);
    float x[8];
    float gm = -INFINITY;
#pragma unroll
    for (int j = 0; j < 8; ++j) {
      x[j] = (8 * c + j < V) ? (float)v[j] : -INFINITY;
      gm = fmaxf(gm, x[j]);
    }
    if (gm > m) {
      int jj = 7;
#pragma unroll
      for (int j = 6; j >= 0; --j) jj = (x[j] == gm) ? j : jj;
      bi = 8 * c + jj;
      s *= __builtin_amdgcn_exp2f((m - gm) * kLog2e);
      m = gm;
    }
    const float mb = m * kLog2e;
#pragma unroll
    for (int j = 0; j < 8; ++j) s += __builtin_amdgcn_exp2f(__builtin_fmaf(x[j], kLog2e, -mb));
  }
#pragma unroll
  for (int o = 32; o > 0; o >>= 1) {
    const float m2 = __shfl_xor(m, o, 64), s2 = __shfl_xor(s, o, 64);
    const int i2 = __shfl_xor(bi, o, 64);
    argmax_fold(m, bi, m2, i2);
    lse_fold(m, s, m2, s2);
  }
  if (lane == 0) { s_m[wib] = m; s_s[wib] = s; s_i[wib] = bi; }
  __syncthreads();
  if (tid == 0) {
    float M = s_m[0], Ssum = s_s[0];
    int I = s_i[0];
    for (int w = 1; w < 16; ++w) {
      argmax_fold(M, I, s_m[w], s_i[w]);
      lse_fold(M, Ssum, s_m[w], s_s[w]);
    }
    row_loss[row] = M + __logf(Ssum) - (float)lr[target[row]];
    row_argmax[row] = (I == CE_NO_COL) ? 0 : I;
  }
}

__global__ __launch_bounds__(256) void ce_lse_partial_kernel(const float2* __restrict__ stats, int n_blocks, int n_rows,
                                                             float2* __restrict__ part) {
  __shared__ float2 sh[4][64];
  const int r = threadIdx.x & 63, q = threadIdx.x >> 6;
  const int row = blockIdx.x * 64 + r;
  const int per = (n_blocks + CE_LSE_SPLIT - 1) / CE_LSE_SPLIT;
  const int b0 = blockIdx.y * per, b1 = min(n_blocks, b0 + per);
  float m = -INFINITY, s = 0.f;
  int b = b0 + q;
  for (; b + 12 < b1; b += 16) {
    float2 v[4];
#pragma unroll
    for (int k = 0; k < 4; ++k) v[k] = stats[(size_t)(b + 4 * k) * n_rows + row];
#pragma unroll
    for (int k = 0; k < 4; ++k) lse_fold(m, s, v[k].x, v[k].y);
  }
  for (; b < b1; b += 4) {
    const float2 v = stats[(size_t)b * n_rows + row];
    lse_fold(m, s, v.x, v.y);
  }
  sh[q][r] = float2{m, s};
  __syncthreads();
  if (q == 0) {
#pragma unroll
    for (int k = 1; k < 4; ++k) lse_fold(m, s, sh[k][r].x, sh[k][r].y);
    part[(size_t)blockIdx.y * n_rows + row] = float2{m, s};
  }
}
__global__ __launch_bounds__(256) void ce_lse_final_kernel(const float2* __restrict__ part, int n_rows, const bf16* __restrict__ logits,
                                                           int ld, const int64_t* __restrict__ target, float* __restrict__ row_loss,
                                                           float* __restrict__ row_lse) {
  const int row = blockIdx.x * 256 + threadIdx.x;
  if (row >= n_rows) return;
  float m = -INFINITY, s = 0.f;
  for (int k = 0; k < CE_LSE_SPLIT; ++k) {
    const float2 v = part[(size_t)k * n_rows + row];
    lse_fold(m, s, v.x, v.y);
  }
  const float lse = m + __logf(s);
  row_lse[row] = lse;
  row_loss[row] = lse - (float)logits[(size_t)row * ld + target[row]];
}

__global__ __launch_bounds__(256) void ce_grad_tile_kernel(bf16* __restrict__ logits, int ld, int n_rows, int V,
                                                           const int64_t* __restrict__ target, const float* __restrict__ row_lse,
                                                           float gscale, float* __restrict__ part) {
  constexpr float kLog2e = 1.4426950408889634f;
  const int col0 = blockIdx.x * CE_CB + threadIdx.x * 8;
  if (col0 >= ld) return;
  const int r0 = blockIdx.y * CE_RB, r1 = min(n_rows, r0 + CE_RB);
  float cs[8] = {0.f, 0.f, 0.f, 0.f, 0.f, 0.f, 0.f, 0.f};
  constexpr int U = 4;
  for (int rb = r0; rb < r1; rb += U) {
    bf16x8 v[U];
    float lb[U];
    int tc[U];
#pragma unroll
    for (int u = 0; u < U; ++u) {
      const int r = min(rb + u, r1 - 1);
      v[u] = __builtin_nontemporal_load(reinterpret_cast<const bf16x8*>(logits + (size_t)r * ld + col0));
      lb[u] = row_lse[r] * kLog2e;
      tc[u] = (int)(target[r] - col0);
    }
#pragma unroll
    for (int u = 0; u < U; ++u) {
      if (rb + u < r1) {
        bf16x8 g;
#pragma unroll
        for (int j = 0; j < 8; ++j) {
          float q = (col0 + j < V) ? __builtin_amdgcn_exp2f(__builtin_fmaf((float)v[u][j], kLog2e, -lb[u])) : 0.f;
          if (j == tc[u]) q -= 1.f;
          g[j] = (bf16)(q * gscale);
          cs[j] += (float)g[j];
        }
        *reinterpret_cast<bf16x8*>(logits + (size_t)(rb + u) * ld + col0) = g;
      }
    }
  }
  float* out = part + (size_t)blockIdx.y * ld + col0;
  *reinterpret_cast<f32x4*>(out) = f32x4{cs[0], cs[1], cs[2], cs[3]};
  *reinterpret_cast<f32x4*>(out + 4) = f32x4{cs[4], cs[5], cs[6], cs[7]};
}

__global__ __launch_bounds__(256) void ce_colsum_reduce_kernel(const float* __restrict__ part, int ld, int n_groups, float* __restrict__ out) {
  const int c = (blockIdx.x * 256 + threadIdx.x) * 4;
  if (c >= ld) return;
  const int per = (n_groups + gridDim.y - 1) / gridDim.y;
  const int g0 = blockIdx.y * per, g1 = min(n_groups, g0 + per);
  f32x4 acc = {0.f, 0.f, 0.f, 0.f};
  for (int g = g0; g < g1; ++g) acc += *reinterpret_cast<const f32x4*>(part + (size_t)g * ld + c);
#pragma unroll
  for (int j = 0; j < 4; ++j) unsafeAtomicAdd(out + c + j, acc[j]);
}

__global__ __launch_bounds__(256) void colsum_kernel(const bf16* __restrict__ x, int ld, int n, int ncols,
                                                     float* __restrict__ out, const float* __restrict__ scale_ptr) {
  const int c4 = blockIdx.x * blockDim.x + threadIdx.x;
  if (4 * c4 >= ncols) return;
  const int rows_per = (n + gridDim.y - 1) / gridDim.y;
  const int r0 = blockIdx.y * rows_per, r1 = min(n, r0 + rows_per);
  f32x4 acc = {0.f, 0.f, 0.f, 0.f};
  for (int r = r0; r < r1; ++r) acc += Vec4<bf16>::load(x + (size_t)r * ld + 4 * c4);
  const float sc = scale_ptr ? *scale_ptr : 1.f;
#pragma unroll
  for (int j = 0; j < 4; ++j)
    if (4 * c4 + j < ncols) unsafeAtomicAdd(out + 4 * c4 + j, acc[j] * sc);
}

}

extern "C" {

size_t m3p_ce_colsum_workspace_bytes(int ld, int n_rows) {
  return (size_t)((n_rows + CE_RB - 1) / CE_RB) * (size_t)ld * sizeof(float);
}

int m3p_ce_fwd_bwd_colsum(void* logits, int ld, int n_rows, int V, const int64_t* target, float* row_loss, float* row_lse,
                          float grad_scale, float* colsum, void* workspace, size_t workspace_bytes, void* stream) {
  if (n_rows <= 0 || V <= 0 || ld < V || (ld % 8) != 0 || ((uintptr_t)logits & 15) || ((uintptr_t)colsum & 15) ||
      ((uintptr_t)workspace & 15))
    return M3P_EINVAL;
  if (workspace_bytes < m3p_ce_colsum_workspace_bytes(ld, n_rows)) return M3P_EINVAL;
  hipLaunchKernelGGL(ce_stats_kernel, dim3(n_rows), dim3(1024), 0, (hipStream_t)stream, (const bf16*)logits, ld, V, target, row_loss, row_lse);
  return m3p_ce_bwd_colsum(logits, ld, n_rows, V, target, row_lse, grad_scale, colsum, workspace, workspace_bytes, stream);
}

int m3p_ce_lse_from_blocks(const void* stats, int n_blocks, int n_rows, const void* logits, int ld, const int64_t* target,
                           float* row_loss, float* row_lse, void* scratch, void* stream) {
  if (n_blocks <= 0 || n_rows <= 0 || (n_rows % 64) != 0 || !stats || !logits || !target || !row_loss || !row_lse || !scratch ||
      ((uintptr_t)stats & 7) || ((uintptr_t)scratch & 7))
    return M3P_EINVAL;
  hipStream_t st = (hipStream_t)stream;
  hipLaunchKernelGGL(ce_lse_partial_kernel, dim3(n_rows / 64, CE_LSE_SPLIT), dim3(256), 0, st, (const float2*)stats, n_blocks, n_rows,
                     (float2*)scratch);
  hipLaunchKernelGGL(ce_lse_final_kernel, dim3((n_rows + 255) / 256), dim3(256), 0, st, (const float2*)scratch, n_rows,
                     (const bf16*)logits, ld, target, row_loss, row_lse);
  M3P_CHECK_LAUNCH();
  return M3P_OK;
}

int m3p_ce_bwd_colsum(void* logits, int ld, int n_rows, int V, const int64_t* target, const float* row_lse,
                      float grad_scale, float* colsum, void* workspace, size_t workspace_bytes, void* stream) {
  if (n_rows <= 0 || V <= 0 || ld < V || (ld % 8) != 0 || ((uintptr_t)logits & 15) || ((uintptr_t)colsum & 15) ||
      ((uintptr_t)workspace & 15) || !row_lse)
    return M3P_EINVAL;
  if (workspace_bytes < m3p_ce_colsum_workspace_bytes(ld, n_rows)) return M3P_EINVAL;
  hipStream_t st = (hipStream_t)stream;
  const int groups = (n_rows + CE_RB - 1) / CE_RB;
  hipLaunchKernelGGL(ce_grad_tile_kernel, dim3((ld + CE_CB - 1) / CE_CB, groups), dim3(256), 0, st, (bf16*)logits, ld, n_rows, V,
                     target, (const float*)row_lse, grad_scale, (float*)workspace);
  if (hipMemsetAsync(colsum, 0, (size_t)ld * sizeof(float), st) != hipSuccess) return M3P_EINVAL;
  hipLaunchKernelGGL(ce_colsum_reduce_kernel, dim3((ld / 4 + 255) / 256, groups >= 16 ? 8 : 1), dim3(256), 0, st,
                     (const float*)workspace, ld, groups, colsum);
  M3P_CHECK_LAUNCH();
  return M3P_OK;
}

int m3p_colsum_bf16(const void* x, int ld, int n, int ncols, float* out, const float* scale_ptr, void* stream) {
  if (n <= 0 || ncols <= 0 || (ld % 4) != 0 || ld < ((ncols + 3) / 4) * 4) return M3P_EINVAL;
  const int c4 = (ncols + 3) / 4;
  int ysplit = 1;
  while (ysplit < 64 && ((c4 + 255) / 256) * ysplit < 1024 && n / (ysplit * 2) >= 16) ysplit *= 2;
  hipLaunchKernelGGL(colsum_kernel, dim3((c4 + 255) / 256, ysplit), dim3(256), 0, (hipStream_t)stream, (const bf16*)x, ld,
                     n, ncols, out, scale_ptr);
  M3P_CHECK_LAUNCH();
  return M3P_OK;
}

int m3p_gather_rows(const void* src, const int32_t* idx, void* dst, int n, int d, void* stream) {
  if (n <= 0) return M3P_OK;
  if ((d % 4) != 0) return M3P_EINVAL;
  const size_t total = (size_t)n * (d / 4);
  const int blocks = (int)((total + 255) / 256 < 2048 ? (total + 255) / 256 : 2048);
  hipLaunchKernelGGL(gather_rows_kernel, dim3(blocks), dim3(256), 0, (hipStream_t)stream, (const bf16*)src, idx, (bf16*)dst, n, d);
  M3P_CHECK_LAUNCH();
  return M3P_OK;
}

int m3p_place_rows(const void* src, const int32_t* inv, void* dst, int rows, int d, int n, uint32_t fill_bits, void* stream) {
  if (rows <= 0) return M3P_OK;
  if (d <= 0 || (d % 8) != 0 || n < 0 || !inv || !dst || (n > 0 && !src) || ((uintptr_t)src & 15) || ((uintptr_t)dst & 15))
    return M3P_EINVAL;
  const size_t total = (size_t)rows * (d / 8);
  const int blocks = (int)((total + 255) / 256 < 8192 ? (total + 255) / 256 : 8192);
  const uint32_t f = fill_bits & 0xFFFFu;
  hipLaunchKernelGGL(place_rows_kernel, dim3(blocks), dim3(256), 0, (hipStream_t)stream, (const bf16*)src, inv, (bf16*)dst, rows, d, n,
                     f | (f << 16));
  M3P_CHECK_LAUNCH();
  return M3P_OK;
}

int m3p_scatter_add_rows(const void* src, const int32_t* idx, void* dst, int n, int d, void* stream) {
  if (n <= 0) return M3P_OK;
  if ((d % 4) != 0) return M3P_EINVAL;
  const size_t total = (size_t)n * (d / 4);
  const int blocks = (int)((total + 255) / 256 < 2048 ? (total + 255) / 256 : 2048);
  hipLaunchKernelGGL(scatter_add_rows_kernel, dim3(blocks), dim3(256), 0, (hipStream_t)stream, (const bf16*)src, idx, (bf16*)dst, n, d);
  M3P_CHECK_LAUNCH();
  return M3P_OK;
}

int m3p_scatter_add_token_rows(const void* rows, int ld_rows, const int64_t* ids, float* dst, int n, int d, int pad_index, void* stream) {
  if (n <= 0) return M3P_OK;
  if (d <= 0 || ld_rows < d) return M3P_EINVAL;
  const int blocks = (n + 3) / 4 < 4096 ? (n + 3) / 4 : 4096;
  hipLaunchKernelGGL(scatter_add_token_rows_kernel, dim3(blocks), dim3(256), 0, (hipStream_t)stream, (const bf16*)rows, ld_rows, ids,
                     dst, n, d, pad_index);
  M3P_CHECK_LAUNCH();
  return M3P_OK;
}

int m3p_ce_fwd_bwd(void* logits, int ld, int n_rows, int V, const int64_t* target, float* row_loss, float* loss_sum,
                   float loss_scale, float grad_scale, void* stream) {
  if (n_rows <= 0 || V <= 0 || ld < V || (ld % 8) != 0 || ((uintptr_t)logits & 15)) return M3P_EINVAL;
  hipLaunchKernelGGL(ce_fwd_bwd_kernel, dim3(n_rows), dim3(1024), 0, (hipStream_t)stream, (bf16*)logits, ld, V, target,
                     row_loss, loss_sum, loss_scale, grad_scale);
  M3P_CHECK_LAUNCH();
  return M3P_OK;
}

int m3p_ce_eval(const void* logits, int ld, int n_rows, int V, const int64_t* target, float* row_loss, int32_t* row_argmax, void* stream) {
  if (n_rows <= 0 || V <= 0 || ld < V || (ld % 8) != 0 || !logits || ((uintptr_t)logits & 15) || !target || !row_loss || !row_argmax)
    return M3P_EINVAL;
  hipLaunchKernelGGL(ce_eval_kernel, dim3(n_rows), dim3(1024), 0, (hipStream_t)stream, (const bf16*)logits, ld, V, target, row_loss,
                     row_argmax);
  M3P_CHECK_LAUNCH();
  return M3P_OK;
}

}
```

### m3p_amd/functional.py

```python
import math
import os
from collections import OrderedDict

import torch

from . import lib as L
from . import fp8 as fp8mod
from . import ops
from . import rng

BF16 = torch.bfloat16
ALIGN = 64
BUCKET_ALIGN = 64 * 8


def _round_up(n, a):
    return (n + a - 1) // a * a


_VOCAB_FULL_TILES = os.environ.get('M3P_VOCAB_FULL_TILES', '1') != '0'
_GELU_GRAD_IN_FWD = os.environ.get('M3P_GELU_GRAD_IN_FWD', '0') != '0'
_GELU_BYTE_GRAD = int(os.environ.get('M3P_GELU_BYTE_GRAD', '2'))
_CE_FUSED_LSE = os.environ.get('M3P_CE_FUSED_LSE', '1') != '0'
_VOCAB_DGRAD_W4 = os.environ.get('M3P_VOCAB_DGRAD_W4', '1') != '0'
# ... 919 lines not shown
                xf, mean15, rstd15 = ops.layernorm_fwd(pre15, ar.p('layer_norm15.%d.weight' % i), ar.p('layer_norm15.%d.bias' % i))
                cross = (q2, kvc, ctx2, lse2, pre15, mean15, rstd15)
            u = torch.empty((M, 4 * d), dtype=BF16, device=dev)
            hact = ops.gemm_nt(xf, ar.w(f + 'lin1.weight'), L.EPI_BIAS_GELU, bias=ar.p(f + 'lin1.bias'), out2=u)
            pre2 = ops.gemm_nt(hact, ar.w(f + 'lin2.weight'), L.EPI_BIAS_DROP_RES, bias=ar.p(f + 'lin2.bias'), aux=xf,
                               seed=dseed(4, i), p_drop=p_drop)
            h_next, mean2, rstd2 = ops.layernorm_fwd(pre2, ar.p('layer_norm2.%d.weight' % i), ar.p('layer_norm2.%d.bias' % i),
                                                     rowmask)
            saved.append((h, qkv, ctxt, lse, pre1, mean1, rstd1, x1, cross, xf, u, hact, pre2, mean2, rstd2))
            h = h_next
        ctx.model = model
        ctx.dims = (B, T, S, d, H, dh, nL)
        ctx.drop = (p_drop, p_attn, seed_step)
        ctx.saved = (x, totlen, rowmask, emb_saved, saved, src16, src_klen, langs, positions)
        ctx.text_meta = (text_embed.dtype, text_embed.device, text_embed.requires_grad) if text_embed is not None else None
        ctx.src_meta = (src_enc.dtype, src_enc.requires_grad) if has_src else None
        hook = model.ddp_hook
        ctx.track = hook is not None
        ctx.tok_rows_max = hook.encoder_forward(T * B) if ctx.track else None
        ctx.set_materialize_grads(False)
        return h

    @staticmethod
    def backward(ctx, dout):
        model = ctx.model
        ar = model.arena()
        B, T, S, d, H, dh, nL = ctx.dims
        p_drop, p_attn, seed_step = ctx.drop
        x, totlen, rowmask, emb_saved, saved, src16, src_klen, langs, positions = ctx.saved
        ctx.saved = None
        dseed = lambda k, i=0: rng.stream_seed(model.base_seed, seed_step, _DEC_SITE0 + 8 * i + k)
        hook = model.ddp_hook if ctx.track else None
        if dout is None:
            if hook is not None:
                hook.encoder_backward_end()
            return (None,) * N_DEC_ARGS
        dh_ = dout.contiguous()
        if dh_.dtype != BF16:
            dh_ = dh_.to(BF16)
        last = hook.encoder_backward_begin() if hook is not None else True
        qscale = 1.0 / math.sqrt(dh)
        has_src = src16 is not None
        d_src = None
        for i in reversed(range(nL)):
            a, f, e = 'attentions.%d.' % i, 'ffns.%d.' % i, 'encoder_attn.%d.' % i
            (h_in, qkv, ctxt, lse, pre1, mean1, rstd1, x1, cross, xf, u, hact, pre2, mean2, rstd2) = saved[i]
            saved[i] = None
            dpre2, dY2 = ops.layernorm_bwd(dh_, None, pre2, ar.p('layer_norm2.%d.weight' % i), mean2, rstd2, rowmask,
                                           ar.g('layer_norm2.%d.weight' % i), ar.g('layer_norm2.%d.bias' % i),
                                           dbias_drop=ar.g(f + 'lin2.bias'), want_drop=p_drop > 0, seed=dseed(4, i), p_drop=p_drop)
            if dY2 is None:
                dY2 = dpre2
            ops.gemm_wgrad(dY2, hact, ar.g(f + 'lin2.weight'))
            dU = ops.gemm_nt(dY2, ar.wt[('lin2', i)], L.EPI_DGELU, aux=u, colsum=ar.g(f + 'lin1.bias'))
            ops.gemm_wgrad(dU, xf, ar.g(f + 'lin1.weight'))
            dxf = ops.gemm_nt(dU, ar.wt[('lin1', i)], L.EPI_RES, aux=dpre2)
            if has_src:
                q2, kvc, ctx2, lse2, pre15, mean15, rstd15 = cross
                dpre15, dAO2 = ops.layernorm_bwd(dxf, None, pre15, ar.p('layer_norm15.%d.weight' % i), mean15, rstd15, None,
                                                 ar.g('layer_norm15.%d.weight' % i), ar.g('layer_norm15.%d.bias' % i),
                                                 dbias_drop=ar.g(e + 'out_lin.bias'), want_drop=p_drop > 0, seed=dseed(3, i),
                                                 p_drop=p_drop)
                if dAO2 is None:
                    dAO2 = dpre15
                ops.gemm_wgrad(dAO2, ctx2, ar.g(e + 'out_lin.weight'))
                dctx2 = ops.gemm_nt(dAO2, ar.wt[('xout', i)], L.EPI_NONE)
                dq2, dkvc = ops.attn_rows_bwd(q2, kvc, src_klen, dctx2, lse2, B, T, H, dh, S, qscale, seed=dseed(2, i), p_drop=p_attn)
                dkvc = dkvc.to(BF16).view(B * S, 2 * d)
                ops.gemm_wgrad(dq2, x1, ar.xattn(i, 'q', grad=True))
                ops.colsum(dq2, d, ar.xattn(i, 'bq', grad=True))
                ops.gemm_wgrad(dkvc, src16, ar.xattn(i, 'kv', grad=True))
                ops.colsum(dkvc, 2 * d, ar.xattn(i, 'bkv', grad=True))
                d_src = ops.gemm_nt(dkvc, ar.wt[('xkv', i)], L.EPI_NONE if d_src is None else L.EPI_RES, aux=d_src)
                dx1 = ops.gemm_nt(dq2, ar.wt[('xq', i)], L.EPI_RES, aux=dpre15)
            else:
                dx1 = dxf
            dpre1, dAO = ops.layernorm_bwd(dx1, None, pre1, ar.p('layer_norm1.%d.weight' % i), mean1, rstd1, None,
                                           ar.g('layer_norm1.%d.weight' % i), ar.g('layer_norm1.%d.bias' % i),
                                           dbias_drop=ar.g(a + 'out_lin.bias'), want_drop=p_drop > 0, seed=dseed(1, i), p_drop=p_drop)
            if dAO is None:
                dAO = dpre1
            ops.gemm_wgrad(dAO, ctxt, ar.g(a + 'out_lin.weight'))
            dctx = ops.gemm_nt(dAO, ar.wt[('out', i)], L.EPI_NONE)
            dqkv = torch.empty_like(qkv)
            _, dkv = ops.attn_rows_bwd(qkv, qkv.view(B, T, 3 * d)[:, :, d:], None, dctx, lse, B, T, H, dh, T, qscale, causal=True,
                                       seed=dseed(0, i), p_drop=p_attn, dq_out=dqkv)
            dqkv.view(B, T, 3 * d)[:, :, d:] = dkv
            ops.colsum(dqkv, 3 * d, ar.qkv_bias(i, grad=True))
            ops.gemm_wgrad(dqkv, h_in, ar.qkv_wgrad(i))
            dh_ = ops.gemm_nt(dqkv, ar.wt[('qkv', i)], L.EPI_RES, aux=dpre1)
            ar.touch_layer(i, cross=has_src)
            if hook is not None:
                hook.layer_done(i, last)
        tok_rows = None
        own_rows = langs is not None or positions is not None or ctx.text_meta is not None
        g_text = None
        if own_rows or (hook is not None and hook.active):
            tok_rows = torch.empty((T * B, d), dtype=BF16, device=dh_.device)
        grads = dict(
            d_g_emb=ar.g('layer_norm_emb.weight'), d_be_emb=ar.g('layer_norm_emb.bias'),
            d_pos=ar.g('position_embeddings.weight'), d_emb=ar.g('embeddings.weight'),
            d_g_img=ar.g('image_embeddings.LayerNorm.weight'), d_be_img=ar.g('image_embeddings.LayerNorm.bias'),
            d_b_img=ar.g('image_embeddings.image_embeddings.bias'),
            d_b_loc=ar.g('image_embeddings.image_location_embeddings.bias'),
            d_w_loc=ar.g('image_embeddings.image_location_embeddings.weight'))
        ops.embed_assemble_bwd(dh_, emb_saved, ar.p('layer_norm_emb.weight'), ar.p('image_embeddings.LayerNorm.weight'), x,
                               totlen, None, grads, B, T, 0, d, model.pad_index, seed_img=0, seed_emb=dseed(7), p_drop=p_drop,
                               tok_rows=tok_rows)
        ar.touch('layer_norm_emb.weight', 'layer_norm_emb.bias', 'position_embeddings.weight', 'embeddings.weight')
        if own_rows:
            if langs is not None:
                npad = (model.n_langs + 7) // 8 * 8
                onehot = torch.zeros((T * B, npad), dtype=BF16, device=tok_rows.device)
                onehot.scatter_(1, langs.view(-1, 1), 1.0)
                dl = torch.zeros((npad, d), dtype=torch.float32, device=tok_rows.device)
                ops.gemm_wgrad(onehot, tok_rows, dl)
                ar.g('cross_lang_embeddings.weight').add_(dl[:model.n_langs])
                ar.touch('cross_lang_embeddings.weight')
            if positions is not None:
                gpos = ar.g('position_embeddings.weight')
                rows32 = tok_rows.float()
                gpos.index_add_(0, positions.reshape(-1), rows32)
                gpos[:T].sub_(rows32.view(T, B, d).sum(dim=1))
            if ctx.text_meta is not None:
                assert hook is None or not hook.active, 'text_embed on the decoder is single-GPU (no token-row exchange for it)'
                if ctx.text_meta[2]:
                    g_text = tok_rows.view(T, B, d).transpose(0, 1).to(device=ctx.text_meta[1], dtype=ctx.text_meta[0])
                tok_rows = None
            elif hook is None or not hook.active:
                ops.scatter_add_token_rows(tok_rows, x.contiguous().view(-1), ar.g('embeddings.weight'), model.pad_index)
                tok_rows = None
        if hook is not None:
            hook.embed_done(last, ids=x if tok_rows is not None else None, rows=tok_rows, n_max=ctx.tok_rows_max)
        g_src = None
        if has_src and ctx.src_meta[1]:
            g_src = d_src.view(B, S, d).to(ctx.src_meta[0])
        return (None, None, None, None, g_src, None, None, None, None, None, None, g_text)


class MLMHeadFn(torch.autograd.Function):

    @staticmethod
    def forward(ctx, tensor, model, base, row_idx, y, scores_out, sink=None):
        ar = model.arena()
        ar.refresh()
        d, V = model.dim, model.n_words
        n = int(y.shape[0])
        ctx.sink = sink
        hsel = ops.gather_rows(base, row_idx, n, d)
        logits = torch.empty((n, ar.V_pad), dtype=BF16, device=hsel.device)
        full_tiles = _VOCAB_FULL_TILES and n >= 1024 and n % 256 == 0
        n_cols = ar.V_pad if full_tiles else V
        fused_lse = _CE_FUSED_LSE and full_tiles
        stats = None
        if fused_lse:
            o = ar.offsets['pred_layer.proj.bias'][0]
            stats = torch.empty((ar.V_pad // 64, n, 2), dtype=torch.float32, device=hsel.device)
            ops.gemm_nt(hsel, ar.w('embeddings.weight'), L.EPI_BIAS_LSE, bias=ar.master[o:o + ar.V_pad], out=logits, n=n_cols,
                        out2=stats, scale_cols=V)
        else:
            ops.gemm_nt(hsel, ar.w('embeddings.weight'), L.EPI_BIAS, bias=ar.p('pred_layer.proj.bias'), out=logits, n=n_cols)
        if scores_out is not None:
            scores_out.append(logits[:, :V].float())
        dbias = None
        if fused_lse:
            loss_sum, _, dbias = ops.ce_from_block_stats(logits, V, y, stats, 1.0 / n, 1.0 / n)
        elif _VOCAB_FULL_TILES and n >= 1024:
            loss_sum, _, dbias = ops.ce_fwd_bwd_colsum(logits, V, y, 1.0 / n, 1.0 / n)
        else:
            loss_sum, _ = ops.ce_fwd_bwd(logits, V, y, 1.0 / n, 1.0 / n)
        ctx.model = model
        ctx.saved = (hsel, logits, row_idx, tuple(tensor.shape), tuple(tensor.stride()), tensor.storage_offset(), base, dbias)
        return loss_sum[0].clone()

    @staticmethod
    def backward(ctx, gloss):
        model = ctx.model
        ar = model.arena()
        fresh = ar.range_untouched(ar.offsets['embeddings.weight'][0], ar.V_pad * model.dim)
        ar.touch('embeddings.weight', 'pred_layer.proj.bias')
        ar.vocab_stored = False
        d, V = model.dim, model.n_words
        hsel, dlogits, row_idx, shape, stride, soff, base, dbias = ctx.saved
        ctx.saved = None
        n = hsel.shape[0]
        g = gloss.reshape(1).float()
        hs = ops.scale_bf16_dev(hsel, g)
        if _VOCAB_FULL_TILES and n >= 4096 and n % 64 == 0:
            o = ar.offsets['embeddings.weight'][0]
            will_store = fresh and L.load().m3p_gemm_wgrad_plan(n, ar.V_pad, d) == L.KERN_WGRAD_W4_TILES
            lazy = will_store and ar.stale == ar.vocab_range()
            if not lazy:
                ar.ensure_zero()
            ar.vocab_stored = ops.gemm_wgrad(dlogits, hs, ar.grad[o:o + ar.V_pad * d].view(ar.V_pad, d), n=ar.V_pad, k=d,
                                             dw_is_zero=fresh, report_store=True, must_store=lazy)
            if lazy:
                ar.stale = None
            if will_store and not ar.vocab_stored:
                raise RuntimeError('the dispatch table promised a stored vocabulary weight gradient, the launcher accumulated')
        else:
            ops.gemm_wgrad(dlogits, hs, ar.g('embeddings.weight'), n=V, k=d)
        if dbias is not None:
            ops.axpy_dev(ar.g('pred_layer.proj.bias'), dbias[:V], g)
        else:
            ops.colsum(dlogits, V, ar.g('pred_layer.proj.bias'), scale=g)
        dH32 = torch.zeros((n, d), dtype=torch.float32, device=dlogits.device)
        ops.gemm_nn(dlogits, ar.w('embeddings.weight'), dH32, k_rows_readable=ar.V_pad if _VOCAB_DGRAD_W4 else None)
        dH = ops.scale_bf16_dev(dH32, g)
        dtensor = _scatter_rows_grad(dH, row_idx, base, shape, stride, soff, ctx.sink)
        if model.ddp_hook is not None:
            model.ddp_hook.mlm_head_done()
        return dtensor, None, None, None, None, None, None


def _as_row_buffer(tensor, d):
    strides, soff = tensor.stride(), tensor.storage_offset()
    with torch.no_grad():
        ok = strides[-1] == 1 and all(st % d == 0 for st in strides[:-1]) and soff % d == 0
        base = torch.as_strided(tensor, (tensor.untyped_storage().nbytes() // 2 // d, d), (d, 1), 0) if ok else None
    if base is None:
        tensor = tensor.contiguous()
        with torch.no_grad():
            base = tensor.view(-1, d)
        strides, soff = tensor.stride(), 0
    return tensor, base, strides, soff


def _scatter_rows_grad(dH, row_idx, base, shape, stride, soff, sink=None):
    if sink is not None:
        ops.scatter_add_rows(dH, row_idx, sink.rows(base), dH.shape[0], dH.shape[1])
        return None
    dbase = torch.zeros_like(base)
    ops.scatter_add_rows(dH, row_idx, dbase, dH.shape[0], dH.shape[1])
    return torch.as_strided(dbase, shape, stride, soff)


class ObjHeadFn(torch.autograd.Function):

    @staticmethod
    def forward(ctx, tensor, model, base, row_idx, y, sink=None):
        ar = model.arena()
        ar.refresh()
        d = model.dim
        n = int(y.shape[0])
        ctx.sink = sink
        hsel = ops.gather_rows(base, row_idx, n, d)
        u = torch.empty((n, d), dtype=BF16, device=hsel.device)
        t = ops.gemm_nt(hsel, ar.w('transformer_obj.dense.weight'), L.EPI_BIAS_GELU, bias=ar.p('transformer_obj.dense.bias'), out2=u)
        x1, mean, rstd = ops.layernorm_fwd(t, ar.p('transformer_obj.LayerNorm.weight'), ar.p('transformer_obj.LayerNorm.bias'))
        logits = ops.gemm_nt(x1, ar.w('pred_obj_layer.proj.weight'), L.EPI_BIAS, bias=ar.p('pred_obj_layer.proj.bias'))
        loss_sum, _ = ops.ce_fwd_bwd(logits, logits.shape[1], y, 1.0 / n, 1.0 / n)
        ctx.model = model
        ctx.saved = (hsel, u, t, mean, rstd, x1, logits, row_idx, tuple(tensor.shape), tuple(tensor.stride()),
                     tensor.storage_offset(), base)
        return loss_sum[0].clone()

    @staticmethod
    def backward(ctx, gloss):
        model = ctx.model
        ar = model.arena()
        hsel, u, t, mean, rstd, x1, dlogits, row_idx, shape, stride, soff, base = ctx.saved
        ctx.saved = None
        n, d = hsel.shape
        g = gloss.reshape(1).float()
        dev = hsel.device
        ar.touch('transformer_obj.dense.weight', 'transformer_obj.dense.bias', 'transformer_obj.LayerNorm.weight',
                 'transformer_obj.LayerNorm.bias', 'pred_obj_layer.proj.weight', 'pred_obj_layer.proj.bias')
        nobj = dlogits.shape[1]
        ops.gemm_wgrad(dlogits, (x1.float() * g).to(BF16), ar.g('pred_obj_layer.proj.weight'))
        ops.colsum(dlogits, nobj, ar.g('pred_obj_layer.proj.bias'), scale=g)
        dx1 = torch.zeros((n, d), dtype=torch.float32, device=dev)
        ops.gemm_nn_streamk(dlogits, ar.w('pred_obj_layer.proj.weight'), dx1)
        dx1 = (dx1 * g).to(BF16)
        dt, _ = ops.layernorm_bwd(dx1, None, t, ar.p('transformer_obj.LayerNorm.weight'), mean, rstd, None,
                                  ar.g('transformer_obj.LayerNorm.weight'), ar.g('transformer_obj.LayerNorm.bias'))
        du = ops.gelu_bwd(dt, u)
        ops.gemm_wgrad(du, hsel, ar.g('transformer_obj.dense.weight'))
        ops.colsum(du, d, ar.g('transformer_obj.dense.bias'))
        dH = torch.zeros((n, d), dtype=torch.float32, device=dev)
        ops.gemm_nn_streamk(du, ar.w('transformer_obj.dense.weight'), dH)
        return _scatter_rows_grad(dH.to(BF16), row_idx, base, shape, stride, soff, ctx.sink), None, None, None, None, None


class MrfrHeadFn(torch.autograd.Function):

    @staticmethod
    def forward(ctx, tensor, model, base, row_idx, target, sink=None):
        ar = model.arena()
        ar.refresh()
        d = model.dim
        n = int(target.shape[0])
        ctx.sink = sink
        hsel = ops.gather_rows(base, row_idx, n, d)
        reg = ops.gemm_nt(hsel, ar.w('mrfr_dense.weight'), L.EPI_BIAS, bias=ar.p('mrfr_dense.bias'))
        sq, dreg = ops.mse_fwd_bwd(reg, target, 1.0 / (n * reg.shape[1]))
        ctx.model = model
        ctx.saved = (hsel, dreg, row_idx, tuple(tensor.shape), tuple(tensor.stride()), tensor.storage_offset(), base)
        return (sq[0] / (n * reg.shape[1])).clone()

    @staticmethod
    def backward(ctx, gloss):
        model = ctx.model
        ar = model.arena()
        hsel, dreg, row_idx, shape, stride, soff, base = ctx.saved
        ctx.saved = None
        n, d = hsel.shape
        g = gloss.reshape(1).float()
        ar.touch('mrfr_dense.weight', 'mrfr_dense.bias')
        ops.gemm_wgrad(dreg, ops.scale_bf16_dev(hsel, g), ar.g('mrfr_dense.weight'))
        ops.colsum(dreg, dreg.shape[1], ar.g('mrfr_dense.bias'), scale=g)
        dH = torch.zeros((n, d), dtype=torch.float32, device=hsel.device)
        ops.gemm_nn_streamk(dreg, ar.w('mrfr_dense.weight'), dH)
        return _scatter_rows_grad(ops.scale_bf16_dev(dH, g), row_idx, base, shape, stride, soff, ctx.sink), None, None, None, None, None


class DenseRowsFn(torch.autograd.Function):

    @staticmethod
    def forward(ctx, x, model, wname, bname):
        ar = model.arena()
        ar.refresh()
        ctx.model, ctx.names = model, (wname, bname)
        ctx.save_for_backward(x)
        return ops.gemm_nt(x, ar.w(wname), L.EPI_BIAS, bias=ar.p(bname))

    @staticmethod
    def backward(ctx, dy):
        model = ctx.model
        ar = model.arena()
        wname, bname = ctx.names
        x, = ctx.saved_tensors
        dy = dy.contiguous()
        if dy.dtype != BF16:
            dy = dy.to(BF16)
        ar.touch(wname, bname)
        ops.colsum(dy, dy.shape[1], ar.g(bname))
        ops.gemm_wgrad(dy, x, ar.g(wname))
        dx = ops.gemm_nt(dy, _transposed(ar.w(wname)), L.EPI_NONE)
        return dx, None, None, None


def mrfr_dense_rows(model, tensor):
    d = model.dim
    assert tensor.shape[-1] == d
    x = tensor.to(BF16).contiguous().view(-1, d)
    return DenseRowsFn.apply(x, model, 'mrfr_dense.weight', 'mrfr_dense.bias').view(*tensor.shape[:-1], -1)


def _masked_region_rows(tensor, labels, d):
    assert tensor.dim() == 3 and tensor.shape[-1] == d and tensor.dtype == BF16
    B, R, _ = tensor.shape
    tensor, base, strides, soff = _as_row_buffer(tensor, d)
    lab = labels.reshape(-1)
    pos = torch.nonzero(lab.cpu() != -1).view(-1)
    b_idx, r_idx = pos // R, pos % R
    row_idx = ((soff + b_idx * strides[0] + r_idx * strides[1]) // d).to(torch.int32).to(tensor.device)
    return tensor, base, row_idx, pos


def mrm_head(model, tensor, y_all):
    tensor, base, row_idx, pos = _masked_region_rows(tensor, y_all, model.dim)
# ... 140 lines not shown
```

### m3p_amd/lib.py

```python
import ctypes as C
import os

import torch

_HERE = os.path.dirname(os.path.abspath(__file__))
LIB_PATH = os.environ.get('M3P_HIP_LIB') or os.path.join(_HERE, 'libm3p_hip.so')

EPI_NONE, EPI_BIAS, EPI_BIAS_GELU, EPI_BIAS_DROP_RES, EPI_RES, EPI_DGELU, EPI_MUL, EPI_MULQ, EPI_BIAS_GELUQ, EPI_BIAS_LSE = range(10)
KERN_NT_SKINNY, KERN_NT_W8, KERN_NT_W8_QUEUE, KERN_NT_W4, KERN_NT_RING, KERN_NT_128 = range(1, 7)
KERN_WGRAD_W4_CHUNKS, KERN_WGRAD_W4_TILES, KERN_WGRAD_RING, KERN_WGRAD_128 = range(10, 14)


class M3PError(RuntimeError):
    pass


class Epilogue(C.Structure):
    _fields_ = [
        ('bias', C.c_void_p), ('aux', C.c_void_p), ('out2', C.c_void_p), ('colsum', C.c_void_p),
        ('ld_aux', C.c_int32), ('ld_out2', C.c_int32), ('scale_cols', C.c_int32), ('scale', C.c_float),
        ('alpha', C.c_float), ('seed', C.c_uint32), ('thresh24', C.c_uint32), ('inv_keep', C.c_float),
        ('descale_a', C.c_void_p), ('descale_b', C.c_void_p),
        ('out8', C.c_void_p), ('scale8', C.c_void_p), ('amax8', C.c_void_p), ('ld_out8', C.c_int32), ('out8_bf8', C.c_int32),
        ('rng_rows', C.c_void_p),
    ]


_p, _i, _f, _u32 = C.c_void_p, C.c_int, C.c_float, C.c_uint32

SIGNATURES = {
    'm3p_version': (C.c_char_p, []),
    'm3p_gemm_nt_bf16': (_i, [_p, _i, _p, _i, _p, _i, _i, _i, _i, _i, C.POINTER(Epilogue), _p]),
    'm3p_gemm_nt_fp8': (_i, [_p, _i, _i, _p, _i, _p, _i, _i, _i, _i, _i, C.POINTER(Epilogue), _p]),
    'm3p_quant_fp8': (_i, [_p, _i, _p, _i, _i, _i, _p, _p, _i, _p]),
    'm3p_quant_fp8_batch': (_i, [_p, _i, _i, _p]),
    'm3p_gemm_nt_streamk_f32': (_i, [_p, _i, _p, _i, _p, _i, _i, _i, _i, _f, _p]),
    'm3p_gemm_nn_streamk_f32': (_i, [_p, _i, _p, _i, _i, _p, _i, _i, _i, _i, _f, _p]),
    'm3p_gemm_nn_w4_f32': (_i, [_p, _i, _p, _i, _p, _i, _i, _i, _i, _f, _p, C.c_size_t, _p]),
    'm3p_gemm_wgrad_workspace_bytes': (C.c_size_t, []),
    'm3p_gemm_wgrad_bf16': (_i, [_p, _i, _p, _i, _p, _i, _i, _i, _i, _f, _p, C.c_size_t, _p]),
    'm3p_gemm_wgrad_store_bf16': (_i, [_p, _i, _p, _i, _p, _i, _i, _i, _i, _f, _p, C.c_size_t, _p]),
    'm3p_gemm_wgrad_pair_bf16': (_i, [_p, _i, _p, _i, _p, _i, _i, _i, _p, _i, _p, _i, _p, _i, _i, _i, _i, _f, _p, C.c_size_t, _p]),
    'm3p_layernorm_fwd': (_i, [_p, _p, _p, _p, _p, _p, _p, _i, _i, _f, _p]),
    'm3p_layernorm_bwd': (_i, [_p, _p, _p, _p, _p, _p, _p, _p, _p, _p, _p, _p, _i, _i, _u32, _u32, _f, _p]),
    'm3p_layernorm_bwd_rows': (_i, [_p, _p, _p, _p, _p, _p, _p, _p, _p, _p, _p, _p, _i, _i, _u32, _u32, _f, _p, _p]),
    'm3p_attn_fwd': (_i, [_p, _p, _p, _p, _p, _i, _i, _i, _i, _u32, _u32, _f, _p]),
    'm3p_attn_bwd': (_i, [_p, _p, _p, _p, _p, _p, _p, _p, _i, _i, _i, _i, _f, _u32, _u32, _f, _p]),
    'm3p_attn_query_fwd': (_i, [_p, _i, _p, C.c_longlong, _i, _p, _p, _i, _i, _i, _i, _i, _i, _i, _p]),
    'm3p_attn_rows_fwd': (_i, [_p, _i, _p, C.c_longlong, _i, _p, _p, _p, _i, _i, _i, _i, _i, _i, _i, _u32, _u32, _f, _p]),
    'm3p_attn_rows_bwd': (_i, [_p, _i, _p, C.c_longlong, _i, _p, _p, _p, _p, _i, _p, _i, _i, _i, _i, _i, _i, _i, _f, _u32, _u32, _f, _p]),
    'm3p_cast_f32_bf16': (_i, [_p, _p, C.c_longlong, _p]),
    'm3p_embed_assemble_fwd': (_i, [_p] * 19 + [_i, _i, _i, _i, _u32, _u32, _u32, _f, _p, _p]),
    'm3p_embed_image_rows_fwd': (_i, [_p] * 10 + [_i, _i, _i, _u32, _u32, _f, _p]),
    'm3p_embed_assemble_bwd': (_i, [_p] * 24 + [_i, _i, _i, _i, _i, _u32, _u32, _u32, _f, _i, _p]),
    'm3p_dropout_rows': (_i, [_p, _i, _p, _i, _p, _i, _i, _i, _u32, _u32, _u32, _u32, _f, _p]),
    'm3p_glu_fwd': (_i, [_p, _i, _p, _i, _i, _p]),
    'm3p_glu_bwd': (_i, [_p, _i, _p, _p, _i, _i, _p]),
    'm3p_gather_rows': (_i, [_p, _p, _p, _i, _i, _p]),
    'm3p_place_rows': (_i, [_p, _p, _p, _i, _i, _i, _u32, _p]),
    'm3p_scatter_add_rows': (_i, [_p, _p, _p, _i, _i, _p]),
    'm3p_scatter_add_token_rows': (_i, [_p, _i, _p, _p, _i, _i, _i, _p]),
    'm3p_ce_fwd_bwd': (_i, [_p, _i, _i, _i, _p, _p, _p, _f, _f, _p]),
    'm3p_ce_colsum_workspace_bytes': (C.c_size_t, [_i, _i]),
    'm3p_ce_fwd_bwd_colsum': (_i, [_p, _i, _i, _i, _p, _p, _p, _f, _p, _p, C.c_size_t, _p]),
    'm3p_ce_lse_from_blocks': (_i, [_p, _i, _i, _p, _i, _p, _p, _p, _p, _p]),
    'm3p_ce_bwd_colsum': (_i, [_p, _i, _i, _i, _p, _p, _f, _p, _p, C.c_size_t, _p]),
    'm3p_ce_eval': (_i, [_p, _i, _i, _i, _p, _p, _p, _p]),
    'm3p_colsum_bf16': (_i, [_p, _i, _i, _i, _p, _p, _p]),
    'm3p_sumsq_f32': (_i, [_p, C.c_longlong, _p, _p]),
    'm3p_sumsq_ranges_f32': (_i, [_p, _p, _p, _i, _p, _p]),
    'm3p_adam_step': (_i, [_p, _p, _p, _p, _p, C.c_longlong, _f, _f, _f, _f, _f, _f, _p, _f, _f, _i, _p]),
    'm3p_adam_step_ranges': (_i, [_p, _p, _p, _p, _p, _p, _p, _p, _p, _i, _f, _f, _f, _f, _f, _p, _f, _f, _p]),
    'm3p_itm_score_fwd': (_i, [_p, _p, _p, _p, _p, _i, _i, _p]),
    'm3p_itm_score_bwd': (_i, [_p, _p, _p, _p, _p, _i, _p, _p, _p, _i, _i, _p]),
    'm3p_gelu_bwd': (_i, [_p, _p, _p, C.c_longlong, _p]),
    'm3p_mse_fwd_bwd': (_i, [_p, _i, _p, _i, _p, _p, _i, _i, _f, _p]),
    'm3p_gelu_fwd': (_i, [_p, _p, _p, C.c_longlong, _p]),
    'm3p_gelu_fwd_gq': (_i, [_p, _p, _p, _i, _i, _p]),
    'm3p_gelu_fwd_q8': (_i, [_p, _p, _p, C.c_longlong, _p, _p, _p]),
    'm3p_transpose_batch_bf16': (_i, [_p, _i, _i, _p]),
    'm3p_transpose_bf16': (_i, [_p, _p, _i, _i, _i, _i, _p]),
    'm3p_set_persistent_grid': (_i, [_i]),
    'm3p_set_tile_queue': (_i, [_p, _i]),
    'm3p_gemm_nt_plan': (_i, [_i, _i, _i, _i]),
    'm3p_gemm_wgrad_plan': (_i, [_i, _i, _i]),
    'm3p_debug_set_variant': (None, [_i]),
    'm3p_debug_attn_variant': (None, [_i]),
    'm3p_seq_masks': (_i, [_p, _p, _i, _i, _p, _p, _p]),
    'm3p_mask_to_rows': (_i, [_p, _i, _i, C.c_longlong, C.c_longlong, C.c_longlong, _i, _p, _i, _p]),
    'm3p_cast_rows_f32_bf16': (_i, [_p, C.c_longlong, C.c_longlong, _i, _i, _i, _p, _p]),
    'm3p_scale_bf16_dev': (_i, [_p, _i, _p, _p, C.c_longlong, _p]),
    'm3p_axpy_dev_f32': (_i, [_p, _p, _p, C.c_longlong, _p]),
    'm3p_itm_loss_fwd_bwd': (_i, [_p, _p, _i, _i, _f, _f, _p, _p, _p]),
    'm3p_probe_mfma_16x16x32': (_i, [_p, _p, _p, _p, _p]),
    'm3p_probe_mfma_fp8_16x16x128': (_i, [_p, _p, _p, _i, _p]),
    'm3p_probe_tr16': (_i, [_p, _p, _p]),
    'm3p_probe_permlane16_swap': (_i, [_p, _p]),
}

_lib = None


def load():
    global _lib
    if _lib is not None:
        return _lib
    if not os.path.exists(LIB_PATH):
        raise M3PError('libm3p_hip.so not found at %s — build it first (make -C m3p_amd/csrc); '
                       'there is no fallback path' % LIB_PATH)
    lib = C.CDLL(LIB_PATH)
    for name, (res, args) in SIGNATURES.items():
        fn = getattr(lib, name)
        fn.restype = res
        fn.argtypes = args
    _lib_tq = os.environ.get('M3P_TILE_QUEUE', '0') != '0'
    _lib = lib
    if _lib_tq and torch.cuda.is_available():
        from . import ops
        ops.set_tile_queue(True)
    return lib


def check(code, what):
    if code != 0:
        kind = {-1: 'M3P_EINVAL (bad shape/alignment)', -2: 'M3P_ENOTIMPL', -3: 'M3P_ENOMEM'}.get(code, 'hipError_t %d' % code)
        raise M3PError('%s failed: %s' % (what, kind))


def ptr(t):
    return None if t is None else t.data_ptr()


def stream():
    return torch.cuda.current_stream().cuda_stream


def num_cus():
    n = torch.cuda.get_device_properties(torch.cuda.current_device()).multi_processor_count
    return max(n - n % 8, 8)


def thresh24(p):
    return int(round(float(p) * (1 << 24)))
```

### m3p_amd/ops.py

```python
import ctypes as C
import os

import torch

from . import lib as L

BF16 = torch.bfloat16
_DEBUG_CHECKS = os.environ.get('M3P_DEBUG_CHECKS') == '1'

PROFILE = None
_EPI_NAMES = ['gemm_nt/none', 'gemm_nt/bias', 'gemm_nt/bias_gelu', 'gemm_nt/bias_drop_res', 'gemm_nt/res',
              'gemm_nt/dgelu', 'gemm_nt/mul', 'gemm_nt/mulq', 'gemm_nt/bias_geluq', 'gemm_nt/bias_lse']


PROFILE_ONLY = None


def _prof_begin(key=None):
    if PROFILE is None or (PROFILE_ONLY is not None and key != PROFILE_ONLY):
        return None
    e = torch.cuda.Event(enable_timing=True)
    e.record()
    return e


def _prof_end(e0, key):
    if e0 is not None:
        e1 = torch.cuda.Event(enable_timing=True)
        e1.record()
        PROFILE.setdefault(key, []).append((e0, e1))


def _chk_bf16(*ts):
    for t in ts:
        if t is not None:
            assert t.dtype == BF16 and t.is_cuda, (t.dtype, t.device)


def gemm_nt(a, w, epilogue=L.EPI_NONE, bias=None, aux=None, out=None, out2=None, colsum=None,
            scale_cols=0, scale=1.0, alpha=1.0, seed=0, p_drop=0.0, n=None, out8=None, scale8=None, amax8=None, out8_bf8=False,
            rng_rows=None):
    M, K = a.shape
    N = w.shape[0] if n is None else n
    if epilogue == L.EPI_MULQ:
        _chk_bf16(a, w, out)
        assert aux is not None and aux.dtype == torch.uint8 and aux.is_contiguous() and aux.numel() == M * N
    elif epilogue == L.EPI_BIAS_LSE:
        _chk_bf16(a, w, out)
        assert out2 is not None and out2.dtype == torch.float32 and out2.is_contiguous() and out2.numel() == (N // 64) * M * 2
        assert bias is not None and 0 < scale_cols <= N
    elif epilogue == L.EPI_BIAS_GELUQ:
        _chk_bf16(a, w, out)
        assert out2 is not None and out2.dtype == torch.uint8 and out2.is_contiguous() and out2.numel() == M * N and bias is not None
    else:
        _chk_bf16(a, w, aux, out, out2)
    assert w.shape[1] == K and a.stride(1) == 1 and w.stride(1) == 1
    if out is None:
        out = torch.empty((M, N), dtype=BF16, device=a.device)
    ep = L.Epilogue()
    ep.bias = L.ptr(bias)
    ep.aux = L.ptr(aux)
    ep.out2 = L.ptr(out2)
    ep.colsum = L.ptr(colsum)
    ep.ld_aux = aux.stride(0) if (aux is not None and epilogue != L.EPI_MULQ) else 0
    ep.ld_out2 = out2.stride(0) if (out2 is not None and epilogue not in (L.EPI_BIAS_GELUQ, L.EPI_BIAS_LSE)) else 0
    ep.scale_cols = scale_cols
    if epilogue == L.EPI_BIAS_LSE:
        ep.ld_out2, ep.scale_cols = scale_cols, 0
    ep.scale = scale
    ep.alpha = alpha
    ep.seed = seed
    ep.thresh24 = L.thresh24(p_drop)
    ep.inv_keep = 1.0 / (1.0 - p_drop) if p_drop > 0 else 1.0
    if bias is not None:
        assert bias.dtype == torch.float32
    if rng_rows is not None:
        assert epilogue == L.EPI_BIAS_DROP_RES and rng_rows.dtype == torch.int32 and rng_rows.is_cuda \
            and rng_rows.is_contiguous() and rng_rows.numel() == M
        ep.rng_rows = rng_rows.data_ptr()
    if out8 is not None:
        assert epilogue in (L.EPI_BIAS_GELUQ, L.EPI_MULQ) and out8.dtype == torch.uint8 and out8.shape == (M, N) and out8.stride(1) == 1
        ep.out8, ep.ld_out8, ep.out8_bf8 = out8.data_ptr(), out8.stride(0), 1 if out8_bf8 else 0
        ep.scale8, ep.amax8 = L.ptr(scale8), L.ptr(amax8)
    e0 = _prof_begin((_EPI_NAMES[epilogue], M, N, K))
    rc = L.load().m3p_gemm_nt_bf16(a.data_ptr(), a.stride(0), w.data_ptr(), w.stride(0), out.data_ptr(),
                                   out.stride(0), M, N, K, epilogue, C.byref(ep), L.stream())
    L.check(rc, 'm3p_gemm_nt_bf16')
    _prof_end(e0, (_EPI_NAMES[epilogue], M, N, K))
    return out


def quant_fp8(x, scale=None, amax=None, bf8=False, out=None):
    _chk_bf16(x)
    rows, cols = x.shape
    assert x.stride(1) == 1
    if out is None:
        out = torch.empty((rows, cols), dtype=torch.uint8, device=x.device)
    rc = L.load().m3p_quant_fp8(x.data_ptr(), x.stride(0), out.data_ptr(), out.stride(0), rows, cols, L.ptr(scale), L.ptr(amax),
                                1 if bf8 else 0, L.stream())
    L.check(rc, 'm3p_quant_fp8')
    return out


def quant_fp8_batch(desc, n_desc, blocks_per_matrix=512):
    L.check(L.load().m3p_quant_fp8_batch(desc.data_ptr(), n_desc, blocks_per_matrix, L.stream()), 'm3p_quant_fp8_batch')


def gemm_nt_fp8(a8, w8, epilogue=L.EPI_NONE, a_is_bf8=False, descale_a=None, descale_b=None, bias=None, aux=None, out=None,
                colsum=None, scale_cols=0, scale=1.0, seed=0, p_drop=0.0):
    assert a8.dtype == torch.uint8 and w8.dtype == torch.uint8 and a8.is_cuda and w8.is_cuda
    M, K = a8.shape
    N = w8.shape[0]
    assert w8.shape[1] == K and a8.stride(1) == 1 and w8.stride(1) == 1
    _chk_bf16(aux, out)
    if out is None:
        out = torch.empty((M, N), dtype=BF16, device=a8.device)
    ep = L.Epilogue()
    ep.bias = L.ptr(bias)
    ep.aux = L.ptr(aux)
    ep.colsum = L.ptr(colsum)
    ep.ld_aux = aux.stride(0) if aux is not None else 0
    ep.scale_cols = scale_cols
    ep.scale = scale
    ep.alpha = 1.0
    ep.seed = seed
    ep.thresh24 = L.thresh24(p_drop)
    ep.inv_keep = 1.0 / (1.0 - p_drop) if p_drop > 0 else 1.0
    ep.descale_a = L.ptr(descale_a)
    ep.descale_b = L.ptr(descale_b)
    e0 = _prof_begin(('gemm_fp8/' + _EPI_NAMES[epilogue].split('/')[1], M, N, K))
    rc = L.load().m3p_gemm_nt_fp8(a8.data_ptr(), a8.stride(0), 1 if a_is_bf8 else 0, w8.data_ptr(), w8.stride(0), out.data_ptr(),
                                  out.stride(0), M, N, K, epilogue, C.byref(ep), L.stream())
    L.check(rc, 'm3p_gemm_nt_fp8')
    _prof_end(e0, ('gemm_fp8/' + _EPI_NAMES[epilogue].split('/')[1], M, N, K))
    return out


def gemm_nt_streamk(a, w, out_f32, alpha=1.0):
    _chk_bf16(a, w)
    M, K = a.shape
    N = w.shape[0]
    assert w.shape[1] == K and out_f32.dtype == torch.float32 and out_f32.shape == (M, N)
    e0 = _prof_begin(('gemm_nt/streamk', M, N, K))
    rc = L.load().m3p_gemm_nt_streamk_f32(a.data_ptr(), a.stride(0), w.data_ptr(), w.stride(0), out_f32.data_ptr(),
                                          out_f32.stride(0), M, N, K, alpha, L.stream())
    L.check(rc, 'm3p_gemm_nt_streamk_f32')
    _prof_end(e0, ('gemm_nt/streamk', M, N, K))
    return out_f32


def gemm_nn_streamk(a, w_kn, out_f32, alpha=1.0):
    _chk_bf16(a, w_kn)
    M, K = a.shape
    k_valid, N = w_kn.shape
    assert k_valid <= K and out_f32.dtype == torch.float32 and out_f32.shape == (M, N) and w_kn.stride(1) == 1
    e0 = _prof_begin(('gemm_nt/streamk', M, N, K))
    rc = L.load().m3p_gemm_nn_streamk_f32(a.data_ptr(), a.stride(0), w_kn.data_ptr(), w_kn.stride(0), k_valid,
                                          out_f32.data_ptr(), out_f32.stride(0), M, N, K, alpha, L.stream())
    L.check(rc, 'm3p_gemm_nn_streamk_f32')
    _prof_end(e0, ('gemm_nt/streamk', M, N, K))
    return out_f32


def gemm_nn(a, w_kn, out_f32, alpha=1.0, k_rows_readable=None):
    _chk_bf16(a, w_kn)
    M, K = a.shape
    k_valid, N = w_kn.shape
    if (k_rows_readable or k_valid) >= K and M % 256 == 0 and N % 256 == 0 and K % 64 == 0 and K >= 4096:
        assert out_f32.dtype == torch.float32 and out_f32.shape == (M, N) and w_kn.stride(1) == 1
        e0 = _prof_begin(('gemm_nn/w4', M, N, K))
        ws = _wgrad_workspace(a.device)
        rc = L.load().m3p_gemm_nn_w4_f32(a.data_ptr(), a.stride(0), w_kn.data_ptr(), w_kn.stride(0), out_f32.data_ptr(),
                                         out_f32.stride(0), M, N, K, alpha, ws.data_ptr(), ws.numel(), L.stream())
        if rc == 0:
            _prof_end(e0, ('gemm_nn/w4', M, N, K))
            return out_f32
        if rc != -2:
            L.check(rc, 'm3p_gemm_nn_w4_f32')
    return gemm_nn_streamk(a, w_kn, out_f32, alpha)


_WGRAD_WS = {}


def _wgrad_workspace(device):
    key = (device.index, torch.cuda.current_stream(device).cuda_stream)
    ws = _WGRAD_WS.get(key)
    if ws is None:
        ws = _WGRAD_WS[key] = torch.empty(int(L.load().m3p_gemm_wgrad_workspace_bytes()), dtype=torch.uint8, device=device)
    return ws


def gemm_wgrad(dy, x, dw, alpha=1.0, n=None, k=None, dw_is_zero=False, report_store=False, must_store=False):
    _chk_bf16(dy, x)
    assert dw.dtype == torch.float32 and dw.stride(-1) == 1
    M = dy.shape[0]
    N = dy.shape[1] if n is None else n
    K = x.shape[1] if k is None else k
    assert x.shape[0] == M and dw.shape[0] >= N and dw.shape[1] >= K
    e0 = _prof_begin(('gemm_wgrad', M, N, K))
    ws = _wgrad_workspace(dy.device)
    if dw_is_zero:
        rc = L.load().m3p_gemm_wgrad_store_bf16(dy.data_ptr(), dy.stride(0), x.data_ptr(), x.stride(0), dw.data_ptr(),
                                                dw.stride(0), M, N, K, alpha, ws.data_ptr(), ws.numel(), L.stream())
        if rc == 0:
            _prof_end(e0, ('gemm_wgrad', M, N, K))
            return True if report_store else dw
        if rc != -2:
            L.check(rc, 'm3p_gemm_wgrad_store_bf16')
        if must_store:
            raise L.M3PError('m3p_gemm_wgrad_store_bf16 declined (M3P_ENOTIMPL) a store the caller depends on: dw is not physically zero')
    rc = L.load().m3p_gemm_wgrad_bf16(dy.data_ptr(), dy.stride(0), x.data_ptr(), x.stride(0), dw.data_ptr(),
                                      dw.stride(0), M, N, K, alpha, ws.data_ptr(), ws.numel(), L.stream())
    L.check(rc, 'm3p_gemm_wgrad_bf16')
    _prof_end(e0, ('gemm_wgrad', M, N, K))
    return False if report_store else dw


def gemm_wgrad_pair(dy_a, x_a, dw_a, dy_b, x_b, dw_b, alpha=1.0):
    _chk_bf16(dy_a, x_a, dy_b, x_b)
    assert dw_a.dtype == torch.float32 and dw_b.dtype == torch.float32 and dw_a.stride(-1) == 1 and dw_b.stride(-1) == 1
    M = dy_a.shape[0]
    assert x_a.shape[0] == M and dy_b.shape[0] == M and x_b.shape[0] == M
    Na, Ka, Nb, Kb = dy_a.shape[1], x_a.shape[1], dy_b.shape[1], x_b.shape[1]
    assert dw_a.shape[0] >= Na and dw_a.shape[1] >= Ka and dw_b.shape[0] >= Nb and dw_b.shape[1] >= Kb
    e0 = _prof_begin(('gemm_wgrad_pair', M, Na + Nb, Ka))
    ws = _wgrad_workspace(dy_a.device)
    rc = L.load().m3p_gemm_wgrad_pair_bf16(dy_a.data_ptr(), dy_a.stride(0), x_a.data_ptr(), x_a.stride(0), dw_a.data_ptr(), dw_a.stride(0),
                                           Na, Ka, dy_b.data_ptr(), dy_b.stride(0), x_b.data_ptr(), x_b.stride(0), dw_b.data_ptr(),
                                           dw_b.stride(0), Nb, Kb, M, alpha, ws.data_ptr(), ws.numel(), L.stream())
    L.check(rc, 'm3p_gemm_wgrad_pair_bf16')
    _prof_end(e0, ('gemm_wgrad_pair', M, Na + Nb, Ka))
# ... 198 lines not shown
        assert img_rows.dtype == BF16 and img_rows.is_contiguous() and img_rows.shape == (B * R, d)
        e, mean_i, rstd_i = img_saved
    else:
        e = torch.empty((max(R * B, 1), d), dtype=BF16, device=dev)
        mean_i = torch.empty(max(R * B, 1), dtype=torch.float32, device=dev)
        rstd_i = torch.empty(max(R * B, 1), dtype=torch.float32, device=dev)
    th, ik = _drop_args(p_drop)
    rc = L.load().m3p_embed_assemble_fwd(
        tok.data_ptr(), emb16.data_ptr(), pos.data_ptr(), L.ptr(img_proj), L.ptr(loc), w_loc.data_ptr(),
        b_loc.data_ptr(), g_img.data_ptr(), be_img.data_ptr(), g_emb.data_ptr(), be_emb.data_ptr(), totlen.data_ptr(),
        h.data_ptr(), z.data_ptr(), mean_e.data_ptr(), rstd_e.data_ptr(), e.data_ptr(), mean_i.data_ptr(),
        rstd_i.data_ptr(), B, T, R, d, seed_img, seed_emb, th, ik, L.ptr(img_rows), L.stream())
    L.check(rc, 'm3p_embed_assemble_fwd')
    return h, (z, mean_e, rstd_e, e, mean_i, rstd_i)


def embed_image_rows_fwd(img_proj, loc, w_loc, b_loc, g_img, be_img, B, R, d, seed_img=0, p_drop=0.0):
    dev = img_proj.device
    e = torch.empty((R * B, d), dtype=BF16, device=dev)
    mean_i = torch.empty(R * B, dtype=torch.float32, device=dev)
    rstd_i = torch.empty(R * B, dtype=torch.float32, device=dev)
    rows = torch.empty((B * R, d), dtype=BF16, device=dev)
    th, ik = _drop_args(p_drop)
    rc = L.load().m3p_embed_image_rows_fwd(img_proj.data_ptr(), loc.data_ptr(), w_loc.data_ptr(), b_loc.data_ptr(),
                                           g_img.data_ptr(), be_img.data_ptr(), e.data_ptr(), mean_i.data_ptr(),
                                           rstd_i.data_ptr(), rows.data_ptr(), B, R, d, seed_img, th, ik, L.stream())
    L.check(rc, 'm3p_embed_image_rows_fwd')
    return rows, (e, mean_i, rstd_i)


def embed_image_rows_bwd(d_rows, img_saved, g_img, loc, totlen, grads, B, R, d, seed_img=0, p_drop=0.0):
    e, mean_i, rstd_i = img_saved
    assert d_rows.dtype == BF16 and d_rows.is_contiguous() and d_rows.shape == (B * R, d)
    de = torch.empty_like(e)
    th, ik = _drop_args(p_drop)
    dummy = d_rows.data_ptr()
    args = (dummy, dummy, mean_i.data_ptr(), rstd_i.data_ptr(), g_img.data_ptr(), e.data_ptr(), mean_i.data_ptr(),
            rstd_i.data_ptr(), g_img.data_ptr(), dummy, totlen.data_ptr(), loc.data_ptr(), d_rows.data_ptr(), de.data_ptr(),
            grads['d_g_img'].data_ptr(), grads['d_be_img'].data_ptr(), grads['d_g_img'].data_ptr(), grads['d_g_img'].data_ptr(),
            None, grads['d_g_img'].data_ptr(), grads['d_be_img'].data_ptr(), grads['d_b_img'].data_ptr(),
            grads['d_b_loc'].data_ptr(), grads['d_w_loc'].data_ptr(), B, 0, R, d, -1, seed_img, 0, th, ik)
    L.check(L.load().m3p_embed_assemble_bwd(*args, 2, L.stream()), 'm3p_embed_assemble_bwd')
    return de


def embed_assemble_bwd(dh, saved, g_emb, g_img, tok, totlen, loc, grads, B, T, R, d, pad_index,
                       seed_img=0, seed_emb=0, p_drop=0.0, img_rows_bwd=None, tok_rows=None):
    z, mean_e, rstd_e, e, mean_i, rstd_i = saved
    dz = torch.empty_like(z)
    de = torch.empty_like(e)
    th, ik = _drop_args(p_drop)
    if tok_rows is not None:
        assert tok_rows.dtype == BF16 and tok_rows.is_contiguous() and tok_rows.shape == (T * B, d)
    args = (dh.data_ptr(), z.data_ptr(), mean_e.data_ptr(), rstd_e.data_ptr(), g_emb.data_ptr(), e.data_ptr(),
            mean_i.data_ptr(), rstd_i.data_ptr(), g_img.data_ptr(), tok.data_ptr(), totlen.data_ptr(), L.ptr(loc),
            dz.data_ptr(), de.data_ptr(), grads['d_g_emb'].data_ptr(), grads['d_be_emb'].data_ptr(),
            grads['d_pos'].data_ptr(), grads['d_emb'].data_ptr(), L.ptr(tok_rows), grads['d_g_img'].data_ptr(),
            grads['d_be_img'].data_ptr(), grads['d_b_img'].data_ptr(), grads['d_b_loc'].data_ptr(),
            grads['d_w_loc'].data_ptr(), B, T, R, d, pad_index, seed_img, seed_emb, th, ik)
    if img_rows_bwd is not None:
        L.check(L.load().m3p_embed_assemble_bwd(*args, 1, L.stream()), 'm3p_embed_assemble_bwd')
        dz_img = dz.view(B, R + T, d)[:, :R, :]
        dz_img.copy_(img_rows_bwd(dz_img.contiguous().view(B * R, d)).view(B, R, d))
        L.check(L.load().m3p_embed_assemble_bwd(*args, 2, L.stream()), 'm3p_embed_assemble_bwd')
        return de
    L.check(L.load().m3p_embed_assemble_bwd(*args, 0, L.stream()), 'm3p_embed_assemble_bwd')
    return de


def scatter_add_token_rows(rows, ids, dst, pad_index):
    _chk_bf16(rows)
    assert ids.dtype == torch.int64 and dst.dtype == torch.float32 and rows.stride(1) == 1 and ids.is_contiguous()
    n, d = rows.shape
    assert ids.numel() == n and dst.shape[1] == d and dst.stride(0) == d
    L.check(L.load().m3p_scatter_add_token_rows(rows.data_ptr(), rows.stride(0), ids.data_ptr(), dst.data_ptr(), n, d, int(pad_index),
                                                L.stream()), 'm3p_scatter_add_token_rows')


def gather_rows(src_base, idx, n, d):
    out = torch.empty((n, d), dtype=BF16, device=idx.device)
    L.check(L.load().m3p_gather_rows(src_base.data_ptr(), idx.data_ptr(), out.data_ptr(), n, d, L.stream()), 'm3p_gather_rows')
    return out


BF16_NAN_BITS = 0x7FC0


def place_rows(src, inv, rows, fill_bits=0):
    _chk_bf16(src)
    n, d = src.shape
    assert src.is_contiguous() and inv.dtype == torch.int32 and inv.is_cuda and inv.is_contiguous() and inv.numel() == rows
    out = torch.empty((rows, d), dtype=BF16, device=src.device)
    L.check(L.load().m3p_place_rows(src.data_ptr(), inv.data_ptr(), out.data_ptr(), rows, d, n, int(fill_bits), L.stream()),
            'm3p_place_rows')
    return out


def scatter_add_rows(src, idx, dst_base, n, d):
    L.check(L.load().m3p_scatter_add_rows(src.data_ptr(), idx.data_ptr(), dst_base.data_ptr(), n, d, L.stream()),
            'm3p_scatter_add_rows')


def ce_fwd_bwd(logits, V, target, loss_scale, grad_scale):
    n, ld = logits.shape[0], logits.stride(0)
    row_loss = torch.empty(n, dtype=torch.float32, device=logits.device)
    assert target.dtype == torch.int64
    rc = L.load().m3p_ce_fwd_bwd(logits.data_ptr(), ld, n, V, target.data_ptr(), row_loss.data_ptr(),
                                 None, loss_scale, grad_scale, L.stream())
    L.check(rc, 'm3p_ce_fwd_bwd')
    loss_sum = (row_loss.sum() * loss_scale).reshape(1)
    return loss_sum, row_loss


_CE_WS = {}


def ce_fwd_bwd_colsum(logits, V, target, loss_scale, grad_scale):
    n, ld = logits.shape[0], logits.stride(0)
    dev = logits.device
    row_loss = torch.empty(n, dtype=torch.float32, device=dev)
    row_lse = torch.empty(n, dtype=torch.float32, device=dev)
    cs = torch.empty(ld, dtype=torch.float32, device=dev)
    need = L.load().m3p_ce_colsum_workspace_bytes(ld, n)
    ws = _CE_WS.get(dev)
    if ws is None or ws.numel() < need:
        ws = _CE_WS[dev] = torch.empty(need, dtype=torch.uint8, device=dev)
    assert target.dtype == torch.int64
    rc = L.load().m3p_ce_fwd_bwd_colsum(logits.data_ptr(), ld, n, V, target.data_ptr(), row_loss.data_ptr(), row_lse.data_ptr(),
                                        grad_scale, cs.data_ptr(), ws.data_ptr(), ws.numel(), L.stream())
    L.check(rc, 'm3p_ce_fwd_bwd_colsum')
    return (row_loss.sum() * loss_scale).reshape(1), row_loss, cs


def ce_from_block_stats(logits, V, target, stats, loss_scale, grad_scale):
    n, ld = logits.shape[0], logits.stride(0)
    dev = logits.device
    row_loss = torch.empty(n, dtype=torch.float32, device=dev)
    row_lse = torch.empty(n, dtype=torch.float32, device=dev)
    cs = torch.empty(ld, dtype=torch.float32, device=dev)
    scratch = torch.empty((32, n, 2), dtype=torch.float32, device=dev)
    assert target.dtype == torch.int64 and stats.dtype == torch.float32 and stats.shape[1] == n
    L.check(L.load().m3p_ce_lse_from_blocks(stats.data_ptr(), stats.shape[0], n, logits.data_ptr(), ld, target.data_ptr(),
                                            row_loss.data_ptr(), row_lse.data_ptr(), scratch.data_ptr(), L.stream()),
            'm3p_ce_lse_from_blocks')
    need = L.load().m3p_ce_colsum_workspace_bytes(ld, n)
    ws = _CE_WS.get(dev)
    if ws is None or ws.numel() < need:
        ws = _CE_WS[dev] = torch.empty(need, dtype=torch.uint8, device=dev)
    L.check(L.load().m3p_ce_bwd_colsum(logits.data_ptr(), ld, n, V, target.data_ptr(), row_lse.data_ptr(), grad_scale, cs.data_ptr(),
                                       ws.data_ptr(), ws.numel(), L.stream()), 'm3p_ce_bwd_colsum')
    return (row_loss.sum() * loss_scale).reshape(1), row_loss, cs


def ce_eval(logits, V, target):
    _chk_bf16(logits)
    assert logits.dim() == 2 and logits.stride(1) == 1 and target.dtype == torch.int64 and target.is_contiguous()
    n, ld = logits.shape[0], logits.stride(0)
    assert target.numel() == n and ld >= V
    row_loss = torch.empty(n, dtype=torch.float32, device=logits.device)
    row_argmax = torch.empty(n, dtype=torch.int32, device=logits.device)
    L.check(L.load().m3p_ce_eval(logits.data_ptr(), ld, n, V, target.data_ptr(), row_loss.data_ptr(), row_argmax.data_ptr(),
                                 L.stream()), 'm3p_ce_eval')
    return row_loss, row_argmax


def colsum(x, ncols, out, scale=None):
    rc = L.load().m3p_colsum_bf16(x.data_ptr(), x.stride(0), x.shape[0], ncols, out.data_ptr(), L.ptr(scale), L.stream())
    L.check(rc, 'm3p_colsum_bf16')


def sumsq(g, out):
    L.check(L.load().m3p_sumsq_f32(g.data_ptr(), g.numel(), out.data_ptr(), L.stream()), 'm3p_sumsq_f32')


def sumsq_ranges(buf, ranges, out):
    ranges = [(int(a), int(b)) for a, b in ranges if b > a]
    if not ranges:
        return
    if len(ranges) == 1:
        return sumsq(buf[ranges[0][0]:ranges[0][1]], out)
    n = len(ranges)
    starts = (C.c_longlong * n)(*[a for a, _ in ranges])
    counts = (C.c_longlong * n)(*[b - a for a, b in ranges])
    L.check(L.load().m3p_sumsq_ranges_f32(buf.data_ptr(), starts, counts, n, out.data_ptr(), L.stream()), 'm3p_sumsq_ranges_f32')


def adam_step(p, g, m, v, w16, lr, beta1, beta2, eps, weight_decay, step_size, gnorm_sq=None, max_norm=0.0,
              grad_scale=1.0, zero_grad=True):
    n = p.numel()
    rc = L.load().m3p_adam_step(p.data_ptr(), g.data_ptr(), m.data_ptr(), v.data_ptr(), L.ptr(w16), n, lr, beta1, beta2,
                                eps, weight_decay, step_size, L.ptr(gnorm_sq), max_norm, grad_scale, int(zero_grad),
                                L.stream())
    L.check(rc, 'm3p_adam_step')


def adam_step_ranges(p, g, m, v, w16, pieces, lr, beta1, beta2, eps, weight_decay, gnorm_sq=None, max_norm=0.0, grad_scale=1.0):
    pieces = [q for q in pieces if q[1] > q[0]]
    if not pieces:
        return
    n = len(pieces)
    starts = (C.c_longlong * n)(*[int(a) for a, _, _, _ in pieces])
    counts = (C.c_longlong * n)(*[int(b - a) for a, b, _, _ in pieces])
    steps = (C.c_float * n)(*[float(st) for _, _, st, _ in pieces])
    zeros = (C.c_int * n)(*[int(bool(z)) for _, _, _, z in pieces])
    rc = L.load().m3p_adam_step_ranges(p.data_ptr(), g.data_ptr(), m.data_ptr(), v.data_ptr(), L.ptr(w16), starts, counts, steps, zeros, n,
                                       lr, beta1, beta2, eps, weight_decay, L.ptr(gnorm_sq), max_norm, grad_scale, L.stream())
    L.check(rc, 'm3p_adam_step_ranges')


def transpose_bf16(src, dst):
    rows, cols = src.shape
    rc = L.load().m3p_transpose_bf16(src.data_ptr(), dst.data_ptr(), rows, cols, src.stride(0), dst.stride(0), L.stream())
    L.check(rc, 'm3p_transpose_bf16')


def gelu_fwd(u, grad_inplace=False):
    h = torch.empty_like(u)
    L.check(L.load().m3p_gelu_fwd(u.data_ptr(), h.data_ptr(), u.data_ptr() if grad_inplace else None, u.numel(), L.stream()),
            'm3p_gelu_fwd')
    return h


GQ_OFF, GQ_STEP = 27.0 / 201.0, 1.0 / 201.0


def gq_eligible(M, N):
    return M >= 1024 and M % 256 == 0 and N % 256 == 0 and N >= 512


def gelu_fwd_gq(u):
    _chk_bf16(u)
    M, N = u.shape
    assert u.is_contiguous() and gq_eligible(M, N), (M, N)
    h = torch.empty_like(u)
    gq = torch.empty((M * N,), dtype=torch.uint8, device=u.device)
    L.check(L.load().m3p_gelu_fwd_gq(u.data_ptr(), h.data_ptr(), gq.data_ptr(), M, N, L.stream()), 'm3p_gelu_fwd_gq')
    return h, gq


def gq_unpack(gq, M, N):
    t = gq.view(M // 256, N // 256, 2, 4, 8, 4, 16, 4, 4)
    t = t.permute(0, 2, 4, 6, 1, 3, 7, 5, 8).reshape(M, N)
    return t.float() * GQ_STEP - GQ_OFF


def gelu_fwd_q8(u, scale, amax=None):
    h = torch.empty_like(u)
    h8 = torch.empty(u.shape, dtype=torch.uint8, device=u.device)
    L.check(L.load().m3p_gelu_fwd_q8(u.data_ptr(), h.data_ptr(), h8.data_ptr(), u.numel(), scale.data_ptr(), L.ptr(amax), L.stream()),
            'm3p_gelu_fwd_q8')
    return h, h8


def transpose_batch(desc, n_desc, max_tiles):
    L.check(L.load().m3p_transpose_batch_bf16(desc.data_ptr(), n_desc, max_tiles, L.stream()), 'm3p_transpose_batch_bf16')


def itm_head_fwd(first, W1_16, b1, w2, b2):
    _chk_bf16(first, W1_16)
    B, d = first.shape
    h16 = first.contiguous()
    pre = gemm_nt(h16, W1_16, L.EPI_BIAS, bias=b1)
    pooled = torch.empty((B, d), dtype=torch.float32, device=first.device)
    scores = torch.empty((B,), dtype=torch.float32, device=first.device)
    rc = L.load().m3p_itm_score_fwd(pre.data_ptr(), w2.data_ptr(), b2.data_ptr(), pooled.data_ptr(), scores.data_ptr(),
                                    B, d, L.stream())
    L.check(rc, 'm3p_itm_score_fwd')
    return h16, pooled, scores


def itm_head_bwd(dscores, h16, pooled, W1_16, w2, dW1, db1, dw2, db2):
    B, d = h16.shape
    dev = h16.device
    ldt = (B + 7) // 8 * 8
    dpre16 = torch.empty((B, d), dtype=BF16, device=dev)
    dpreT16 = torch.zeros((d, ldt), dtype=BF16, device=dev)
    assert dscores.dtype == torch.float32 and dscores.is_contiguous() and dscores.numel() == B
    rc = L.load().m3p_itm_score_bwd(dscores.data_ptr(), pooled.data_ptr(), w2.data_ptr(), dpre16.data_ptr(),
                                    dpreT16.data_ptr(), ldt, db1.data_ptr(), dw2.data_ptr(), db2.data_ptr(), B, d, L.stream())
    L.check(rc, 'm3p_itm_score_bwd')
    gemm_wgrad(dpre16, h16, dW1)
    dh32 = torch.zeros((B, d), dtype=torch.float32, device=dev)
    gemm_wgrad(dpreT16, W1_16, dh32, n=B)
    return dh32.to(BF16)


def gelu_bwd(dy, u):
    _chk_bf16(dy, u)
    assert dy.shape == u.shape and dy.is_contiguous() and u.is_contiguous()
    du = torch.empty_like(dy)
    L.check(L.load().m3p_gelu_bwd(dy.data_ptr(), u.data_ptr(), du.data_ptr(), dy.numel(), L.stream()), 'm3p_gelu_bwd')
    return du


def mse_fwd_bwd(pred, tgt, grad_scale):
    _chk_bf16(pred)
    n, c = pred.shape
    assert tgt.shape == (n, c) and tgt.dtype == torch.float32 and pred.stride(1) == 1 and tgt.stride(1) == 1
    dpred = torch.empty_like(pred)
    row_sq = torch.empty((n,), dtype=torch.float32, device=pred.device)
    rc = L.load().m3p_mse_fwd_bwd(pred.data_ptr(), pred.stride(0), tgt.data_ptr(), tgt.stride(0), dpred.data_ptr(),
                                  row_sq.data_ptr(), n, c, grad_scale, L.stream())
    L.check(rc, 'm3p_mse_fwd_bwd')
    return row_sq.sum().reshape(1), dpred


# ... 33 lines not shown
```

Before: 8107 sequences/s.

## Use target-shifted exponent CE for vocab head instead of max-based LSE

Adds a cross-entropy formulation that first computes each row's target logit, then has the vocab GEMM epilogue emit exp(logit - target - shift) with the target column zeroed and only per-block sums. The running-max pass is dropped and the stats shrink to one float per block. Loss and gradients are rebuilt from these shifted sums with new kernels for row scaling, target-row correction of embedding and bias grads, and dH fixup. This adds several small kernels and atomics and relies on a fixed shift of 40 staying within range.

```diff
diff --git a/include/m3p_hip.h b/include/m3p_hip.h
--- a/include/m3p_hip.h
+++ b/include/m3p_hip.h
@@ -52,6 +52,7 @@
   int32_t ld_out8;
   int32_t out8_bf8;
   const int32_t* rng_rows;
+  const void* row_ref;
 } M3PEpilogue;
 
 M3P_API int m3p_gemm_nt_bf16(const void* A, int lda, const void* W, int ldw, void* C, int ldc,
@@ -169,6 +170,18 @@
 M3P_API int m3p_ce_fwd_bwd_colsum(void* logits, int ld, int n_rows, int V, const int64_t* target, float* row_loss,
                                   float* row_lse, float grad_scale, float* colsum, void* workspace,
                                   size_t workspace_bytes, void* stream);
+
+M3P_API int m3p_ce_shift_target(const void* h, const void* emb, const float* bias, const int64_t* target, float* row_t, void* row_ref,
+                                int n_rows, int d, void* stream);
+M3P_API int m3p_ce_shift_rows(const void* stats, int n_blocks, int n_rows, float grad_scale, float* row_loss, float* row_s,
+                              float* row_q, void* scratch, void* stream);
+M3P_API int m3p_ce_shift_colsum(const void* e, int ld, int n_rows, const float* row_s, float* colsum, void* workspace,
+                                size_t workspace_bytes, void* stream);
+M3P_API int m3p_ce_shift_scale_rows(const void* h, const float* row_s, const float* g, void* out, int n_rows, int d, void* stream);
+M3P_API int m3p_ce_shift_target_rows(const void* h, const int64_t* target, const float* row_q, const float* g, float* demb, float* dbias,
+                                     int n_rows, int d, void* stream);
+M3P_API int m3p_ce_shift_dh(const float* dh32, const void* emb, const int64_t* target, const float* row_s, const float* row_q,
+                            const float* g, void* dh, int n_rows, int d, void* stream);
 
 M3P_API int m3p_ce_eval(const void* logits, int ld, int n_rows, int V, const int64_t* target, float* row_loss,
                         int32_t* row_argmax, void* stream);
diff --git a/m3p_amd/csrc/gemm.hip b/m3p_amd/csrc/gemm.hip
--- a/m3p_amd/csrc/gemm.hip
+++ b/m3p_amd/csrc/gemm.hip
@@ -616,6 +616,61 @@
     sm += __shfl_xor(sm, 16, 64);
     sm += __shfl_xor(sm, 32, 64);
     if (fg == 0) stats[mrow0 + ii * 16 + fr] = float2{m, sm};
+  }
+  bf16* Cp = C + (size_t)mrow0 * ldc + nw + sch * 8;
+#pragma unroll
+  for (int it = 0; it < 4; ++it) {
+    const int row = it * 8 + srow;
+    st16p<true>(Cp + (size_t)row * ldc, flip_halves(*reinterpret_cast<const u32x4*>(r1 + ep_off<true>(row, sch * 16)), it & 1));
+  }
+}
+
+constexpr int M3P_EPI_BIAS_EXP = 11;
+struct CeRowRef { float c; int32_t y; };
+__device__ __forceinline__ void epilogue_half_exp(bf16* __restrict__ C, int ldc, float* __restrict__ stats, const CeRowRef* __restrict__ ref,
+                                                  int V, int mrow0, int nw, char* r1, const f32x4 (&rows0)[4], const f32x4 (&rows1)[4],
+                                                  const f32x4 (&biasv)[4], int lane, bool edge) {
+  constexpr float kLog2e = 1.4426950408889634f;
+  const int fr = lane & 15, fg = lane >> 4;
+  const int srow = lane >> 3, sch = lane & 7;
+  const float2 rf[2] = {*reinterpret_cast<const float2*>(ref + mrow0 + fr), *reinterpret_cast<const float2*>(ref + mrow0 + 16 + fr)};
+#pragma unroll
+  for (int ii = 0; ii < 2; ++ii) {
+    const float cb = rf[ii].x * kLog2e;
+    const int tc = __builtin_bit_cast(int, rf[ii].y) - nw - fg * 4;
+    f32x4 x[4];
+#pragma unroll
+    for (int j = 0; j < 4; ++j) {
+      const f32x4 a = ((ii ? rows1[j] : rows0[j]) + biasv[j]) * kLog2e - cb;
+#pragma unroll
+      for (int r = 0; r < 4; ++r) x[j][r] = __builtin_amdgcn_exp2f(a[r]);
+    }
+    if (edge) {
+#pragma unroll
+      for (int j = 0; j < 4; ++j)
+#pragma unroll
+        for (int r = 0; r < 4; ++r)
+          if (nw + j * 16 + fg * 4 + r >= V) x[j][r] = 0.f;
+    }
+    if (__any((unsigned)(tc + fg * 4) < 64u)) {
+#pragma unroll
+      for (int j = 0; j < 4; ++j)
+#pragma unroll
+        for (int r = 0; r < 4; ++r)
+          if (j * 16 + r == tc) x[j][r] = 0.f;
+    }
+    f32x4 s4 = f32x4{0.f, 0.f, 0.f, 0.f};
+#pragma unroll
+    for (int j = 0; j < 4; ++j) {
+      const bf16x4 xb = bf16x4{(bf16)x[j][0], (bf16)x[j][1], (bf16)x[j][2], (bf16)x[j][3]};
+      *reinterpret_cast<bf16x4*>(r1 + ep_off8<true>(ii * 16 + fr, (j * 16 + fg * 4) * 2)) = xb;
+#pragma unroll
+      for (int r = 0; r < 4; ++r) s4[r] += (float)xb[r];
+    }
+    float sm = (s4[0] + s4[1]) + (s4[2] + s4[3]);
+    sm += __shfl_xor(sm, 16, 64);
+    sm += __shfl_xor(sm, 32, 64);
+    if (fg == 0) stats[mrow0 + ii * 16 + fr] = sm;
   }
   bf16* Cp = C + (size_t)mrow0 * ldc + nw + sch * 8;
 #pragma unroll
@@ -1165,19 +1220,29 @@
         csum_nw = nw;
       }
       const bool fast = io_aligned && (m0 + BM <= M) && (n0 + BN <= N);
-      if constexpr (EPI == M3P_EPI_BIAS_LSE) {
+      if constexpr (EPI == M3P_EPI_BIAS_LSE || EPI == M3P_EPI_BIAS_EXP) {
         if (fast) {
           char* r1 = smem + 2 * STAGE + wid * 4096;
           f32x4 biasv[4];
 #pragma unroll
           for (int j = 0; j < 4; ++j) biasv[j] = *reinterpret_cast<const f32x4*>(ep.bias + nw + j * 16 + (lane >> 4) * 4);
           const int V = ep.ld_out2;
-          float2* st = reinterpret_cast<float2*>(ep.out2) + (size_t)(tn * 4 + wn) * M;
           const bool edge = (nw + 64 > V);
-#pragma unroll
-          for (int hf = 0; hf < 4; ++hf) {
-            epilogue_half_lse(C, ldc, st, V, mw + 32 * hf, nw, r1, acc[2 * hf], acc[2 * hf + 1], biasv, lane, edge);
-            __builtin_amdgcn_sched_barrier(0);
+          if constexpr (EPI == M3P_EPI_BIAS_EXP) {
+            float* st = reinterpret_cast<float*>(ep.out2) + (size_t)(tn * 4 + wn) * M;
+            const CeRowRef* ref = reinterpret_cast<const CeRowRef*>(ep.row_ref);
+#pragma unroll
+            for (int hf = 0; hf < 4; ++hf) {
+              epilogue_half_exp(C, ldc, st, ref, V, mw + 32 * hf, nw, r1, acc[2 * hf], acc[2 * hf + 1], biasv, lane, edge);
+              __builtin_amdgcn_sched_barrier(0);
+            }
+          } else {
+            float2* st = reinterpret_cast<float2*>(ep.out2) + (size_t)(tn * 4 + wn) * M;
+#pragma unroll
+            for (int hf = 0; hf < 4; ++hf) {
+              epilogue_half_lse(C, ldc, st, V, mw + 32 * hf, nw, r1, acc[2 * hf], acc[2 * hf + 1], biasv, lane, edge);
+              __builtin_amdgcn_sched_barrier(0);
+            }
           }
         }
       } else if constexpr (kGqLut) {
@@ -2435,9 +2500,11 @@
   if (M < 1024 || (M % 256) || (N % 256) || N < 512 || (K % 64) || (lda % 8) || (ldw % 8) || (ldc % 8) || ((uintptr_t)C & 15))
     return M3P_EINVAL;
   if (EPI == M3P_EPI_MULQ && (!ep.aux || ((uintptr_t)ep.aux & 15))) return M3P_EINVAL;
-  if ((EPI == M3P_EPI_BIAS_GELUQ || EPI == M3P_EPI_BIAS_LSE) && (!ep.out2 || ((uintptr_t)ep.out2 & 15) || !ep.bias || ((uintptr_t)ep.bias & 15)))
+  constexpr bool kLse = (EPI == M3P_EPI_BIAS_LSE || EPI == M3P_EPI_BIAS_EXP);
+  if ((EPI == M3P_EPI_BIAS_GELUQ || kLse) && (!ep.out2 || ((uintptr_t)ep.out2 & 15) || !ep.bias || ((uintptr_t)ep.bias & 15)))
     return M3P_EINVAL;
-  if (EPI == M3P_EPI_BIAS_LSE && (ep.ld_out2 <= 0 || ep.ld_out2 > N)) return M3P_EINVAL;
+  if (kLse && (ep.ld_out2 <= 0 || ep.ld_out2 > N)) return M3P_EINVAL;
+  if (EPI == M3P_EPI_BIAS_EXP && (!ep.row_ref || ((uintptr_t)ep.row_ref & 7))) return M3P_EINVAL;
   const int tiles_m = M / 256, tiles_n = N / 256;
   const size_t lds = 2 * 512 * ROWB + ((EPI == M3P_EPI_BIAS_GELUQ) ? GQ_TAB_BYTES + 8 * 2048 + 8 * 1024 : 8 * (EPI != M3P_EPI_MULQ ? 4096 : 2048)) +
                      (EPI == M3P_EPI_MULQ ? 2048 + 8 * 1024 : 0);
@@ -3276,7 +3343,9 @@
     case M3P_EPI_MUL: return launch_nt<M3P_EPI_MUL>(a, lda, w, ldw, c, ldc, M, N, K, ep, st);
     case M3P_EPI_MULQ: return launch_nt_gq<M3P_EPI_MULQ>(a, lda, w, ldw, c, ldc, M, N, K, ep, st);
     case M3P_EPI_BIAS_GELUQ: return launch_nt_gq<M3P_EPI_BIAS_GELUQ>(a, lda, w, ldw, c, ldc, M, N, K, ep, st);
-    case M3P_EPI_BIAS_LSE: return launch_nt_gq<M3P_EPI_BIAS_LSE>(a, lda, w, ldw, c, ldc, M, N, K, ep, st);
+    case M3P_EPI_BIAS_LSE:
+      if (ep.row_ref) return launch_nt_gq<M3P_EPI_BIAS_EXP>(a, lda, w, ldw, c, ldc, M, N, K, ep, st);
+      return launch_nt_gq<M3P_EPI_BIAS_LSE>(a, lda, w, ldw, c, ldc, M, N, K, ep, st);
     default: return M3P_EINVAL;
   }
 }
diff --git a/m3p_amd/csrc/heads.hip b/m3p_amd/csrc/heads.hip
--- a/m3p_amd/csrc/heads.hip
+++ b/m3p_amd/csrc/heads.hip
@@ -336,9 +336,215 @@
     if (4 * c4 + j < ncols) unsafeAtomicAdd(out + 4 * c4 + j, acc[j] * sc);
 }
 
+constexpr float CE_SHIFT = 40.f;
+struct CeRowRef { float c; int32_t y; };
+
+__global__ __launch_bounds__(256) void ce_shift_target_kernel(const bf16* __restrict__ h, const bf16* __restrict__ emb, const float* __restrict__ bias,
+                                                              const int64_t* __restrict__ target, float* __restrict__ row_t,
+                                                              CeRowRef* __restrict__ row_ref, int n_rows, int d) {
+  const int lane = threadIdx.x & 63;
+  const int row = (int)((blockIdx.x * blockDim.x + threadIdx.x) >> 6);
+  if (row >= n_rows) return;
+  const int64_t y = target[row];
+  const bf16* hr = h + (size_t)row * d;
+  const bf16* er = emb + (size_t)y * d;
+  float acc = 0.f;
+  for (int c = lane * 4; c < d; c += 256) {
+    const f32x4 a = Vec4<bf16>::load(hr + c), b = Vec4<bf16>::load(er + c);
+    acc += (a[0] * b[0] + a[1] * b[1]) + (a[2] * b[2] + a[3] * b[3]);
+  }
+  acc = wave_sum(acc);
+  if (lane == 0) {
+    const float t = acc + bias[y];
+    row_t[row] = t;
+    row_ref[row] = CeRowRef{t + CE_SHIFT, (int32_t)y};
+  }
+}
+
+__global__ __launch_bounds__(256) void ce_shift_partial_kernel(const float* __restrict__ stats, int n_blocks, int n_rows, float* __restrict__ part) {
+  __shared__ float sh[4][64];
+  const int r = threadIdx.x & 63, q = threadIdx.x >> 6;
+  const int row = blockIdx.x * 64 + r;
+  const int per = (n_blocks + CE_LSE_SPLIT - 1) / CE_LSE_SPLIT;
+  const int b0 = blockIdx.y * per, b1 = min(n_blocks, b0 + per);
+  float s[4] = {0.f, 0.f, 0.f, 0.f};
+  int b = b0 + q;
+  for (; b + 12 < b1; b += 16) {
+#pragma unroll
+    for (int k = 0; k < 4; ++k) s[k] += stats[(size_t)(b + 4 * k) * n_rows + row];
+  }
+  for (; b < b1; b += 4) s[0] += stats[(size_t)b * n_rows + row];
+  sh[q][r] = (s[0] + s[1]) + (s[2] + s[3]);
+  __syncthreads();
+  if (q == 0) part[(size_t)blockIdx.y * n_rows + row] = (sh[0][r] + sh[1][r]) + (sh[2][r] + sh[3][r]);
+}
+__global__ __launch_bounds__(256) void ce_shift_final_kernel(const float* __restrict__ part, int n_rows, float gs, float* __restrict__ row_loss,
+                                                             float* __restrict__ row_s, float* __restrict__ row_q) {
+  const int row = blockIdx.x * 256 + threadIdx.x;
+  if (row >= n_rows) return;
+  float sum = 0.f;
+  for (int k = 0; k < CE_LSE_SPLIT; ++k) sum += part[(size_t)k * n_rows + row];
+  const float e0 = expf(-CE_SHIFT);
+  const float sigma = sum + e0;
+  float loss, q;
+  if (sum < e0) {
+    const float r = sum * expf(CE_SHIFT);
+    loss = log1pf(r);
+    q = -gs * r / (1.f + r);
+  } else {
+    loss = CE_SHIFT + logf(sigma);
+    q = gs * expm1f(-loss);
+  }
+  row_loss[row] = loss;
+  row_s[row] = gs / sigma;
+  row_q[row] = q;
+}
+
+__global__ __launch_bounds__(256) void ce_shift_colsum_tile_kernel(const bf16* __restrict__ e, int ld, int n_rows, const float* __restrict__ row_s,
+                                                                   float* __restrict__ part) {
+  const int col0 = blockIdx.x * CE_CB + threadIdx.x * 8;
+  if (col0 >= ld) return;
+  const int r0 = blockIdx.y * CE_RB, r1 = min(n_rows, r0 + CE_RB);
+  float cs[8] = {0.f, 0.f, 0.f, 0.f, 0.f, 0.f, 0.f, 0.f};
+  constexpr int U = 4;
+  for (int rb = r0; rb < r1; rb += U) {
+    bf16x8 v[U];
+    float w[U];
+#pragma unroll
+    for (int u = 0; u < U; ++u) {
+      const int r = min(rb + u, r1 - 1);
+      v[u] = __builtin_nontemporal_load(reinterpret_cast<const bf16x8*>(e + (size_t)r * ld + col0));
+      w[u] = (rb + u < r1) ? row_s[r] : 0.f;
+    }
+#pragma unroll
+    for (int u = 0; u < U; ++u)
+#pragma unroll
+      for (int j = 0; j < 8; ++j) cs[j] = __builtin_fmaf(w[u], (float)v[u][j], cs[j]);
+  }
+  float* out = part + (size_t)blockIdx.y * ld + col0;
+  *reinterpret_cast<f32x4*>(out) = f32x4{cs[0], cs[1], cs[2], cs[3]};
+  *reinterpret_cast<f32x4*>(out + 4) = f32x4{cs[4], cs[5], cs[6], cs[7]};
+}
+
+__global__ __launch_bounds__(256) void ce_shift_scale_rows_kernel(const bf16* __restrict__ h, const float* __restrict__ row_s, const float* __restrict__ g,
+                                                                  bf16* __restrict__ out, int n, int d) {
+  const int nchunk = d >> 2;
+  const size_t total = (size_t)n * nchunk;
+  const float gv = *g;
+  for (size_t i = (size_t)blockIdx.x * blockDim.x + threadIdx.x; i < total; i += (size_t)gridDim.x * blockDim.x) {
+    const int r = (int)(i / nchunk);
+    Vec4<bf16>::store(out + 4 * i, Vec4<bf16>::load(h + 4 * i) * (gv * row_s[r]));
+  }
+}
+
+__global__ __launch_bounds__(256) void ce_shift_target_rows_kernel(const bf16* __restrict__ h, const int64_t* __restrict__ target,
+                                                                   const float* __restrict__ row_q, const float* __restrict__ g,
+                                                                   float* __restrict__ demb, float* __restrict__ dbias, int n, int d) {
+  const int lane = threadIdx.x & 63;
+  const int wave = (int)((blockIdx.x * blockDim.x + threadIdx.x) >> 6), nwave = (int)((gridDim.x * blockDim.x) >> 6);
+  const float gv = *g;
+  for (int r = wave; r < n; r += nwave) {
+    const int64_t id = target[r];
+    const float c = gv * row_q[r];
+    const bf16* src = h + (size_t)r * d;
+    float* out = demb + (size_t)id * d;
+    for (int k = lane; k < d; k += 64) {
+      const float v = c * (float)src[k];
+      if (v != 0.f) unsafeAtomicAdd(out + k, v);
+    }
+    if (lane == 0) unsafeAtomicAdd(dbias + id, c);
+  }
+}
+
+__global__ __launch_bounds__(256) void ce_shift_dh_kernel(const float* __restrict__ dh32, const bf16* __restrict__ emb, const int64_t* __restrict__ target,
+                                                          const float* __restrict__ row_s, const float* __restrict__ row_q,
+                                                          const float* __restrict__ g, bf16* __restrict__ dh, int n, int d) {
+  const int nchunk = d >> 2;
+  const size_t total = (size_t)n * nchunk;
+  const float gv = *g;
+  for (size_t i = (size_t)blockIdx.x * blockDim.x + threadIdx.x; i < total; i += (size_t)gridDim.x * blockDim.x) {
+    const int r = (int)(i / nchunk), c = (int)(i - (size_t)r * nchunk);
+    const f32x4 a = Vec4<float>::load(dh32 + 4 * i);
+    const f32x4 b = Vec4<bf16>::load(emb + (size_t)target[r] * d + 4 * c);
+    Vec4<bf16>::store(dh + 4 * i, (a * row_s[r] + b * row_q[r]) * gv);
+  }
+}
+
 }
 
 extern "C" {
+
+int m3p_ce_shift_target(const void* h, const void* emb, const float* bias, const int64_t* target, float* row_t, void* row_ref,
+                        int n_rows, int d, void* stream) {
+  if (n_rows <= 0 || d <= 0 || (d % 4) != 0 || !h || !emb || !bias || !target || !row_t || !row_ref || ((uintptr_t)h & 7) ||
+      ((uintptr_t)emb & 7) || ((uintptr_t)row_ref & 7))
+    return M3P_EINVAL;
+  hipLaunchKernelGGL(ce_shift_target_kernel, dim3((n_rows + 3) / 4), dim3(256), 0, (hipStream_t)stream, (const bf16*)h, (const bf16*)emb,
+                     bias, target, row_t, (CeRowRef*)row_ref, n_rows, d);
+  M3P_CHECK_LAUNCH();
+  return M3P_OK;
+}
+
+int m3p_ce_shift_rows(const void* stats, int n_blocks, int n_rows, float grad_scale, float* row_loss, float* row_s, float* row_q,
+                      void* scratch, void* stream) {
+  if (n_blocks <= 0 || n_rows <= 0 || (n_rows % 64) != 0 || !stats || !row_loss || !row_s || !row_q || !scratch)
+    return M3P_EINVAL;
+  hipStream_t st = (hipStream_t)stream;
+  hipLaunchKernelGGL(ce_shift_partial_kernel, dim3(n_rows / 64, CE_LSE_SPLIT), dim3(256), 0, st, (const float*)stats, n_blocks, n_rows,
+                     (float*)scratch);
+  hipLaunchKernelGGL(ce_shift_final_kernel, dim3((n_rows + 255) / 256), dim3(256), 0, st, (const float*)scratch, n_rows, grad_scale,
+                     row_loss, row_s, row_q);
+  M3P_CHECK_LAUNCH();
+  return M3P_OK;
+}
+
+int m3p_ce_shift_colsum(const void* e, int ld, int n_rows, const float* row_s, float* colsum, void* workspace, size_t workspace_bytes,
+                        void* stream) {
+  if (n_rows <= 0 || ld <= 0 || (ld % 8) != 0 || !e || !row_s || !colsum || !workspace || ((uintptr_t)e & 15) ||
+      ((uintptr_t)colsum & 15) || ((uintptr_t)workspace & 15))
+    return M3P_EINVAL;
+  if (workspace_bytes < m3p_ce_colsum_workspace_bytes(ld, n_rows)) return M3P_EINVAL;
+  hipStream_t st = (hipStream_t)stream;
+  const int groups = (n_rows + CE_RB - 1) / CE_RB;
+  hipLaunchKernelGGL(ce_shift_colsum_tile_kernel, dim3((ld + CE_CB - 1) / CE_CB, groups), dim3(256), 0, st, (const bf16*)e, ld, n_rows,
+                     row_s, (float*)workspace);
+  if (hipMemsetAsync(colsum, 0, (size_t)ld * sizeof(float), st) != hipSuccess) return M3P_EINVAL;
+  hipLaunchKernelGGL(ce_colsum_reduce_kernel, dim3((ld / 4 + 255) / 256, groups >= 16 ? 8 : 1), dim3(256), 0, st,
+                     (const float*)workspace, ld, groups, colsum);
+  M3P_CHECK_LAUNCH();
+  return M3P_OK;
+}
+
+static int ce_shift_blocks(size_t total) { return (int)((total + 255) / 256 < 2048 ? (total + 255) / 256 : 2048); }
+
+int m3p_ce_shift_scale_rows(const void* h, const float* row_s, const float* g, void* out, int n_rows, int d, void* stream) {
+  if (n_rows <= 0 || d <= 0 || (d % 4) != 0 || !h || !row_s || !g || !out || ((uintptr_t)h & 7) || ((uintptr_t)out & 7)) return M3P_EINVAL;
+  hipLaunchKernelGGL(ce_shift_scale_rows_kernel, dim3(ce_shift_blocks((size_t)n_rows * (d / 4))), dim3(256), 0, (hipStream_t)stream,
+                     (const bf16*)h, row_s, g, (bf16*)out, n_rows, d);
+  M3P_CHECK_LAUNCH();
+  return M3P_OK;
+}
+
+int m3p_ce_shift_target_rows(const void* h, const int64_t* target, const float* row_q, const float* g, float* demb, float* dbias,
+                             int n_rows, int d, void* stream) {
+  if (n_rows <= 0 || d <= 0 || !h || !target || !row_q || !g || !demb || !dbias) return M3P_EINVAL;
+  const int blocks = (n_rows + 3) / 4 < 4096 ? (n_rows + 3) / 4 : 4096;
+  hipLaunchKernelGGL(ce_shift_target_rows_kernel, dim3(blocks), dim3(256), 0, (hipStream_t)stream, (const bf16*)h, target, row_q, g, demb,
+                     dbias, n_rows, d);
+  M3P_CHECK_LAUNCH();
+  return M3P_OK;
+}
+
+int m3p_ce_shift_dh(const float* dh32, const void* emb, const int64_t* target, const float* row_s, const float* row_q, const float* g,
+                    void* dh, int n_rows, int d, void* stream) {
+  if (n_rows <= 0 || d <= 0 || (d % 4) != 0 || !dh32 || !emb || !target || !row_s || !row_q || !g || !dh || ((uintptr_t)dh32 & 15) ||
+      ((uintptr_t)emb & 7) || ((uintptr_t)dh & 7))
+    return M3P_EINVAL;
+  hipLaunchKernelGGL(ce_shift_dh_kernel, dim3(ce_shift_blocks((size_t)n_rows * (d / 4))), dim3(256), 0, (hipStream_t)stream, dh32,
+                     (const bf16*)emb, target, row_s, row_q, g, (bf16*)dh, n_rows, d);
+  M3P_CHECK_LAUNCH();
+  return M3P_OK;
+}
 
 size_t m3p_ce_colsum_workspace_bytes(int ld, int n_rows) {
   return (size_t)((n_rows + CE_RB - 1) / CE_RB) * (size_t)ld * sizeof(float);
diff --git a/m3p_amd/functional.py b/m3p_amd/functional.py
--- a/m3p_amd/functional.py
+++ b/m3p_amd/functional.py
@@ -1095,8 +1095,15 @@
         full_tiles = _VOCAB_FULL_TILES and n >= 1024 and n % 256 == 0
         n_cols = ar.V_pad if full_tiles else V
         fused_lse = _CE_FUSED_LSE and full_tiles
+        shifted = fused_lse and scores_out is None
         stats = None
-        if fused_lse:
+        if shifted:
+            o = ar.offsets['pred_layer.proj.bias'][0]
+            _, row_ref = ops.ce_shift_target(hsel, ar.w('embeddings.weight'), ar.p('pred_layer.proj.bias'), y)
+            stats = torch.empty((ar.V_pad // 64, n), dtype=torch.float32, device=hsel.device)
+            ops.gemm_nt(hsel, ar.w('embeddings.weight'), L.EPI_BIAS_LSE, bias=ar.master[o:o + ar.V_pad], out=logits, n=n_cols,
+                        out2=stats, scale_cols=V, row_ref=row_ref)
+        elif fused_lse:
             o = ar.offsets['pred_layer.proj.bias'][0]
             stats = torch.empty((ar.V_pad // 64, n, 2), dtype=torch.float32, device=hsel.device)
             ops.gemm_nt(hsel, ar.w('embeddings.weight'), L.EPI_BIAS_LSE, bias=ar.master[o:o + ar.V_pad], out=logits, n=n_cols,
@@ -1106,14 +1113,18 @@
         if scores_out is not None:
             scores_out.append(logits[:, :V].float())
         dbias = None
-        if fused_lse:
+        rows = None
+        if shifted:
+            loss_sum, _, row_s, row_q, dbias = ops.ce_shift_from_block_sums(logits, stats, 1.0 / n, 1.0 / n)
+            rows = (row_s, row_q, y)
+        elif fused_lse:
             loss_sum, _, dbias = ops.ce_from_block_stats(logits, V, y, stats, 1.0 / n, 1.0 / n)
         elif _VOCAB_FULL_TILES and n >= 1024:
             loss_sum, _, dbias = ops.ce_fwd_bwd_colsum(logits, V, y, 1.0 / n, 1.0 / n)
         else:
             loss_sum, _ = ops.ce_fwd_bwd(logits, V, y, 1.0 / n, 1.0 / n)
         ctx.model = model
-        ctx.saved = (hsel, logits, row_idx, tuple(tensor.shape), tuple(tensor.stride()), tensor.storage_offset(), base, dbias)
+        ctx.saved = (hsel, logits, row_idx, tuple(tensor.shape), tuple(tensor.stride()), tensor.storage_offset(), base, dbias, rows)
         return loss_sum[0].clone()
 
     @staticmethod
@@ -1124,11 +1135,11 @@
         ar.touch('embeddings.weight', 'pred_layer.proj.bias')
         ar.vocab_stored = False
         d, V = model.dim, model.n_words
-        hsel, dlogits, row_idx, shape, stride, soff, base, dbias = ctx.saved
+        hsel, dlogits, row_idx, shape, stride, soff, base, dbias, rows = ctx.saved
         ctx.saved = None
         n = hsel.shape[0]
         g = gloss.reshape(1).float()
-        hs = ops.scale_bf16_dev(hsel, g)
+        hs = ops.scale_bf16_dev(hsel, g) if rows is None else ops.ce_shift_scale_rows(hsel, rows[0], g)
         if _VOCAB_FULL_TILES and n >= 4096 and n % 64 == 0:
             o = ar.offsets['embeddings.weight'][0]
             will_store = fresh and L.load().m3p_gemm_wgrad_plan(n, ar.V_pad, d) == L.KERN_WGRAD_W4_TILES
@@ -1147,9 +1158,14 @@
             ops.axpy_dev(ar.g('pred_layer.proj.bias'), dbias[:V], g)
         else:
             ops.colsum(dlogits, V, ar.g('pred_layer.proj.bias'), scale=g)
+        if rows is not None:
+            ops.ce_shift_target_rows(hsel, rows[2], rows[1], g, ar.g('embeddings.weight'), ar.g('pred_layer.proj.bias'))
         dH32 = torch.zeros((n, d), dtype=torch.float32, device=dlogits.device)
         ops.gemm_nn(dlogits, ar.w('embeddings.weight'), dH32, k_rows_readable=ar.V_pad if _VOCAB_DGRAD_W4 else None)
-        dH = ops.scale_bf16_dev(dH32, g)
+        if rows is None:
+            dH = ops.scale_bf16_dev(dH32, g)
+        else:
+            dH = ops.ce_shift_dh(dH32, ar.w('embeddings.weight'), rows[2], rows[0], rows[1], g)
         dtensor = _scatter_rows_grad(dH, row_idx, base, shape, stride, soff, ctx.sink)
         if model.ddp_hook is not None:
             model.ddp_hook.mlm_head_done()
diff --git a/m3p_amd/lib.py b/m3p_amd/lib.py
--- a/m3p_amd/lib.py
+++ b/m3p_amd/lib.py
@@ -23,6 +23,7 @@
         ('descale_a', C.c_void_p), ('descale_b', C.c_void_p),
         ('out8', C.c_void_p), ('scale8', C.c_void_p), ('amax8', C.c_void_p), ('ld_out8', C.c_int32), ('out8_bf8', C.c_int32),
         ('rng_rows', C.c_void_p),
+        ('row_ref', C.c_void_p),
     ]
 
 
@@ -65,6 +66,12 @@
     'm3p_ce_fwd_bwd_colsum': (_i, [_p, _i, _i, _i, _p, _p, _p, _f, _p, _p, C.c_size_t, _p]),
     'm3p_ce_lse_from_blocks': (_i, [_p, _i, _i, _p, _i, _p, _p, _p, _p, _p]),
     'm3p_ce_bwd_colsum': (_i, [_p, _i, _i, _i, _p, _p, _f, _p, _p, C.c_size_t, _p]),
+    'm3p_ce_shift_target': (_i, [_p, _p, _p, _p, _p, _p, _i, _i, _p]),
+    'm3p_ce_shift_rows': (_i, [_p, _i, _i, _f, _p, _p, _p, _p, _p]),
+    'm3p_ce_shift_colsum': (_i, [_p, _i, _i, _p, _p, _p, C.c_size_t, _p]),
+    'm3p_ce_shift_scale_rows': (_i, [_p, _p, _p, _p, _i, _i, _p]),
+    'm3p_ce_shift_target_rows': (_i, [_p, _p, _p, _p, _p, _p, _i, _i, _p]),
+    'm3p_ce_shift_dh': (_i, [_p, _p, _p, _p, _p, _p, _p, _i, _i, _p]),
     'm3p_ce_eval': (_i, [_p, _i, _i, _i, _p, _p, _p, _p]),
     'm3p_colsum_bf16': (_i, [_p, _i, _i, _i, _p, _p, _p]),
     'm3p_sumsq_f32': (_i, [_p, C.c_longlong, _p, _p]),
diff --git a/m3p_amd/ops.py b/m3p_amd/ops.py
--- a/m3p_amd/ops.py
+++ b/m3p_amd/ops.py
@@ -39,7 +39,7 @@
 
 def gemm_nt(a, w, epilogue=L.EPI_NONE, bias=None, aux=None, out=None, out2=None, colsum=None,
             scale_cols=0, scale=1.0, alpha=1.0, seed=0, p_drop=0.0, n=None, out8=None, scale8=None, amax8=None, out8_bf8=False,
-            rng_rows=None):
+            rng_rows=None, row_ref=None):
     M, K = a.shape
     N = w.shape[0] if n is None else n
     if epilogue == L.EPI_MULQ:
@@ -47,8 +47,10 @@
         assert aux is not None and aux.dtype == torch.uint8 and aux.is_contiguous() and aux.numel() == M * N
     elif epilogue == L.EPI_BIAS_LSE:
         _chk_bf16(a, w, out)
-        assert out2 is not None and out2.dtype == torch.float32 and out2.is_contiguous() and out2.numel() == (N // 64) * M * 2
+        assert out2 is not None and out2.dtype == torch.float32 and out2.is_contiguous()
+        assert out2.numel() == (N // 64) * M * (2 if row_ref is None else 1)
         assert bias is not None and 0 < scale_cols <= N
+        assert row_ref is None or (row_ref.dtype == torch.int32 and row_ref.is_cuda and row_ref.is_contiguous() and row_ref.numel() == 2 * M)
     elif epilogue == L.EPI_BIAS_GELUQ:
         _chk_bf16(a, w, out)
         assert out2 is not None and out2.dtype == torch.uint8 and out2.is_contiguous() and out2.numel() == M * N and bias is not None
@@ -78,6 +80,9 @@
         assert epilogue == L.EPI_BIAS_DROP_RES and rng_rows.dtype == torch.int32 and rng_rows.is_cuda \
             and rng_rows.is_contiguous() and rng_rows.numel() == M
         ep.rng_rows = rng_rows.data_ptr()
+    if row_ref is not None:
+        assert epilogue == L.EPI_BIAS_LSE
+        ep.row_ref = row_ref.data_ptr()
     if out8 is not None:
         assert epilogue in (L.EPI_BIAS_GELUQ, L.EPI_MULQ) and out8.dtype == torch.uint8 and out8.shape == (M, N) and out8.stride(1) == 1
         ep.out8, ep.ld_out8, ep.out8_bf8 = out8.data_ptr(), out8.stride(0), 1 if out8_bf8 else 0
@@ -582,6 +587,67 @@
     return (row_loss.sum() * loss_scale).reshape(1), row_loss, cs
 
 
+def ce_shift_target(h, emb, bias, target):
+    _chk_bf16(h, emb)
+    n, d = h.shape
+    assert h.is_contiguous() and emb.stride(0) == d and emb.stride(1) == 1 and bias.dtype == torch.float32 and bias.is_contiguous()
+    assert target.dtype == torch.int64 and target.is_contiguous() and target.numel() == n
+    row_t = torch.empty(n, dtype=torch.float32, device=h.device)
+    row_ref = torch.empty((n, 2), dtype=torch.int32, device=h.device)
+    L.check(L.load().m3p_ce_shift_target(h.data_ptr(), emb.data_ptr(), bias.data_ptr(), target.data_ptr(), row_t.data_ptr(),
+                                         row_ref.data_ptr(), n, d, L.stream()), 'm3p_ce_shift_target')
+    return row_t, row_ref
+
+
+def ce_shift_from_block_sums(e, stats, loss_scale, grad_scale):
+    n, ld = e.shape[0], e.stride(0)
+    dev = e.device
+    assert stats.dtype == torch.float32 and stats.is_contiguous() and stats.shape[1] == n
+    row_loss = torch.empty(n, dtype=torch.float32, device=dev)
+    row_s = torch.empty(n, dtype=torch.float32, device=dev)
+    row_q = torch.empty(n, dtype=torch.float32, device=dev)
+    scratch = torch.empty((32, n), dtype=torch.float32, device=dev)
+    L.check(L.load().m3p_ce_shift_rows(stats.data_ptr(), stats.shape[0], n, grad_scale, row_loss.data_ptr(), row_s.data_ptr(),
+                                       row_q.data_ptr(), scratch.data_ptr(), L.stream()), 'm3p_ce_shift_rows')
+    cs = torch.empty(ld, dtype=torch.float32, device=dev)
+    need = L.load().m3p_ce_colsum_workspace_bytes(ld, n)
+    ws = _CE_WS.get(dev)
+    if ws is None or ws.numel() < need:
+        ws = _CE_WS[dev] = torch.empty(need, dtype=torch.uint8, device=dev)
+    L.check(L.load().m3p_ce_shift_colsum(e.data_ptr(), ld, n, row_s.data_ptr(), cs.data_ptr(), ws.data_ptr(), ws.numel(), L.stream()),
+            'm3p_ce_shift_colsum')
+    return (row_loss.sum() * loss_scale).reshape(1), row_loss, row_s, row_q, cs
+
+
+def ce_shift_scale_rows(h, row_s, g):
+    _chk_bf16(h)
+    assert h.is_contiguous() and row_s.dtype == g.dtype == torch.float32 and row_s.numel() == h.shape[0] and g.numel() == 1
+    out = torch.empty_like(h)
+    L.check(L.load().m3p_ce_shift_scale_rows(h.data_ptr(), row_s.data_ptr(), g.data_ptr(), out.data_ptr(), h.shape[0], h.shape[1],
+                                             L.stream()), 'm3p_ce_shift_scale_rows')
+    return out
+
+
+def ce_shift_target_rows(h, target, row_q, g, demb, dbias):
+    _chk_bf16(h)
+    n, d = h.shape
+    assert h.is_contiguous() and target.dtype == torch.int64 and target.numel() == n and row_q.dtype == g.dtype == torch.float32
+    assert demb.dtype == dbias.dtype == torch.float32 and demb.shape[1] == d and demb.stride(0) == d and dbias.is_contiguous()
+    L.check(L.load().m3p_ce_shift_target_rows(h.data_ptr(), target.data_ptr(), row_q.data_ptr(), g.data_ptr(), demb.data_ptr(),
+                                              dbias.data_ptr(), n, d, L.stream()), 'm3p_ce_shift_target_rows')
+
+
+def ce_shift_dh(dh32, emb, target, row_s, row_q, g):
+    _chk_bf16(emb)
+    n, d = dh32.shape
+    assert dh32.dtype == torch.float32 and dh32.is_contiguous() and emb.stride(0) == d and emb.stride(1) == 1
+    assert target.dtype == torch.int64 and target.numel() == n and row_s.dtype == row_q.dtype == g.dtype == torch.float32
+    out = torch.empty((n, d), dtype=BF16, device=dh32.device)
+    L.check(L.load().m3p_ce_shift_dh(dh32.data_ptr(), emb.data_ptr(), target.data_ptr(), row_s.data_ptr(), row_q.data_ptr(),
+                                     g.data_ptr(), out.data_ptr(), n, d, L.stream()), 'm3p_ce_shift_dh')
+    return out
+
+
 def ce_eval(logits, V, target):
     _chk_bf16(logits)
     assert logits.dim() == 2 and logits.stride(1) == 1 and target.dtype == torch.int64 and target.is_contiguous()
```

Result: faster. 8253 sequences/s (median of 6 runs) (+1.8%).
